# AlfredUg/MiCall-Lite

Measured on AMD Instinct MI355X. Metric: paired 2×251 nt reads/sec mapped+realigned; fraction of HBM roofline, higher is better.
Workload: dtype int32; 1 GPU; C2: synthetic 2x251 nt HIV-1 pol read pairs (10% divergent sample genome, 0.5% errors), prelim_map end-to-end vs 74 seeds + 1 remap iteration(s) (--local vs consensus) + pileups, default projects.json; pairs_per_gpu=1000000, read_len=251, parallelism=dp1 (one GPU, no collective), dist_world=1

## Files before the change

### include/micall_hip.h

```cpp
#ifndef MICALL_HIP_H
#define MICALL_HIP_H

#include <stddef.h>
#include <stdint.h>

#ifdef __cplusplus
extern "C" {
#endif

#define MH_MAXOPS 128

enum { MH_E2E = 0, MH_LOCAL = 1 };
enum { MH_OP_M = 0, MH_OP_I = 1, MH_OP_D = 2, MH_OP_S = 4 };

typedef struct {
    int mode;
    int rdg_open, rdg_ext;
    int rfg_open, rfg_ext;
    int maxins;
} mh_params;

typedef struct {
    int32_t ref, pos, rev, score, secbest, flag, mapq, rnext, pnext, tlen;
    int32_t sam_ref, sam_pos, xm, xo, xg, nm, ys, yt, yf, n_cigar;
// ... 1 lines not shown
} mh_aln;

typedef struct mh_ctx mh_ctx;

int mh_version(void);
int mh_last_error(char *buf, size_t cap);
int mh_device_count(int *n);

int mh_ctx_create(int device, mh_ctx **out);
int mh_ctx_destroy(mh_ctx *ctx);
int mh_ctx_sync(mh_ctx *ctx);
int mh_ctx_stream(mh_ctx *ctx, void **stream);

int mh_index_build(mh_ctx *ctx, int n_refs, const char *const *seqs, int seedlen);

int mh_reads_load(mh_ctx *ctx, int64_t n_reads, int paired, const uint8_t *seq,
                  const uint8_t *qual, const int64_t *offsets, const int32_t *lens);
int mh_reads_load_fastq(mh_ctx *ctx, const char *path1, const char *path2, int64_t *n_reads);
int mh_reads_load_fastq_part(mh_ctx *ctx, const char *path1, const char *path2, int part, int parts,
                             int64_t *n_reads, int64_t *first_unit);
int mh_reads_count(mh_ctx *ctx, int64_t *n_reads, int *paired);

typedef struct mh_fastq mh_fastq;
int mh_fastq_open_part(const char *path, int fd, int part, int parts, mh_fastq **out, int64_t *info);
int mh_fastq_scan_part(const char *path, int fd, int part, int parts, int64_t *info);
int mh_fastq_member_open(const char *path, int fd, int part, int parts, mh_fastq **out, int64_t *info);
int mh_fastq_member_decode(mh_fastq *fq, int64_t end_bit, int64_t *info);
int mh_fastq_member_tail(mh_fastq *fq, const char *window, char *tail);
int mh_fastq_member_finish(mh_fastq *fq, const char *window, int64_t c0, int64_t c1, int64_t *info);
int mh_fastq_frame(mh_fastq *fq, int64_t line0, int starts_line, int64_t *out5);
int mh_fastq_record_offset(mh_fastq *fq, int64_t k, int64_t *off);
int mh_fastq_splice(mh_fastq *fq, int64_t lo, int64_t hi, const char *front, int64_t flen,
                    const char *back, int64_t blen);
int mh_fastq_view(mh_fastq *fq, const char **data, int64_t *len);
int mh_fastq_close(mh_fastq *fq);
int mh_fastq_parse(mh_fastq *fq1, mh_fastq *fq2, char *names, size_t names_cap, uint8_t *seq,
                   uint8_t *qual, size_t bases_cap, int32_t *lens, int64_t reads_cap, int64_t *n_reads,
                   int64_t *n_bases, size_t *names_used);
int mh_reads_load_staged(mh_ctx *ctx, mh_fastq *fq1, mh_fastq *fq2, const int64_t *range4,
                         int64_t fastq_lines1, int64_t *n_reads);
int mh_reads_fastq_lines(mh_ctx *ctx, int64_t *lines1);

int mh_map(mh_ctx *ctx, const mh_params *par);
int mh_alns_fetch(mh_ctx *ctx, int64_t first, int64_t n, mh_aln *out);
int mh_map_counts(mh_ctx *ctx, int64_t *lines, int64_t *filtered, int64_t *mapped,
                  int64_t *first_row, int64_t *first_mapped, int64_t *unmapped,
                  int64_t *star_lines, int64_t *star_first);
int mh_map_stats(mh_ctx *ctx, int64_t *out5);
int mh_test_set_capacities(mh_ctx *ctx, int64_t cigar_pool_words, int64_t pileup_events,
                           int64_t pileup_event_bytes, int64_t token_bytes);
int mh_test_pileup_info(mh_ctx *ctx, int64_t *out16, int n_refs, int32_t *win_len);
int mh_test_force_index_collision(mh_ctx *ctx, int on);
int mh_retry_counts(mh_ctx *ctx, int64_t *out4);
int mh_test_set_gotoh_wait(mh_ctx *ctx, int64_t ticks);
int mh_recs_fetch(mh_ctx *ctx, int64_t first, int64_t n, int32_t *out20);
int mh_recs_fetch_fields(mh_ctx *ctx, int64_t first, int64_t n, int field0, int nfields, int32_t *out);
int mh_reads_set_names(mh_ctx *ctx, int64_t n, const char *const *names);
int mh_format_rows(mh_ctx *ctx, int style, const int64_t *order, int64_t first, int64_t n,
                   const char *const *refnames, char *buf, size_t cap, size_t *used);
int mh_format_segments(mh_ctx *ctx, int style, const int64_t *order, int64_t n,
                       const char *const *refnames, int n_seg, const int64_t *seg_rows,
                       int64_t *seg_bytes);
int mh_write_segments(mh_ctx *ctx, int fd, const int64_t *seg_off, uint32_t *crc);
uint32_t mh_crc32_combine(uint32_t a, uint32_t b, int64_t len_b);
int mh_file_crc32(int fd, int64_t *size, uint32_t *crc);
enum { MH_PHASE_INFLATE = 0, MH_PHASE_PARSE = 1, MH_PHASE_UPLOAD = 2, MH_PHASE_FORMAT = 3,
       MH_PHASE_WRITE = 4, MH_PHASES = 5 };
int mh_phase_times(mh_ctx *ctx, double *ms, int reset);
int mh_write_rows_crc(mh_ctx *ctx, int style, const int64_t *order, int64_t first, int64_t n,
                      const char *const *refnames, int fd, int64_t offset, int64_t *written,
                      uint32_t *crc);

int mh_rows_load(mh_ctx *ctx, int64_t n_rows, const int32_t *flag, const int32_t *ref,
                 const int32_t *pos, const int32_t *cigar_off, const int32_t *n_cigar,
                 const uint32_t *cigar, const uint8_t *seq, const uint8_t *qual,
                 const int64_t *offsets, const int32_t *lens, int64_t n_units,
                 const int64_t *unit_rows);
int mh_rows_load_csv(mh_ctx *ctx, const char *text, int64_t len, int n_refs,
                     const char *const *refnames, int64_t *n_rows, int64_t *n_units,
                     int32_t *n_present);
int mh_rows_info(mh_ctx *ctx, int32_t *out4, int32_t *present, char *unknown, size_t cap);
#define MH_PILEUP_SLACK 2048
int mh_pileup(mh_ctx *ctx, int source, int q_cutoff, int n_refs, const int32_t *ref_lens);
int mh_pileup_only(mh_ctx *ctx, int source, int q_cutoff, int n_refs, const int32_t *ref_lens, int n_sel,
                   const int32_t *sel);
#define MH_WATCH_MAXKEYS 1024
#define MH_WATCH_QBINS 95
int mh_pileup_watch(mh_ctx *ctx, int n_keys, const int32_t *refs, const int32_t *poss);
int mh_pileup_watch_fetch(mh_ctx *ctx, uint32_t *counts, int64_t *first_unit);
int mh_rows_load_sam(mh_ctx *ctx, const char *text, int64_t len, int64_t *n_rows,
                     int64_t *n_units, int32_t *n_refs, size_t *names_bytes);
int mh_sam_info(mh_ctx *ctx, char *names, size_t cap, int32_t *ends);
typedef struct {
    int64_t n_rows, n_units, n_cigar, n_bases;
    int32_t n_refs;
    size_t names_bytes;
} mh_sam_sizes;
int mh_sam_parse(const char *text, int64_t len, mh_sam_sizes *sizes, int32_t *flag, int32_t *ref,
                 int32_t *pos, int32_t *cigar_off, int32_t *n_cigar, uint32_t *cigar,
                 int64_t *seq_off, int32_t *seq_len, uint8_t *seq, uint8_t *qual, int64_t *units,
                 char *names, int32_t *ends);
typedef struct {
    int64_t n_rows, n_units, n_cigar, n_bases;
    int32_t n_present;
    size_t unknown_bytes;
} mh_prelim_sizes;
// ... 147 lines not shown
```

### micall-lite_amd/csrc/mh_api.cpp

```cpp
#include <errno.h>
#include <fcntl.h>
#include <sys/mman.h>
#include <sys/stat.h>
#include <unistd.h>
#include <zlib.h>

#include <algorithm>
#include <atomic>
#include <chrono>
#include <cmath>
#include <cstdarg>
#include <cstdio>
#include <cstring>
#include <memory>
#include <new>
#include <string>
#include <condition_variable>
#include <deque>
#include <exception>
#include <mutex>
#include <functional>
#include <string_view>
#include <thread>
#include <unordered_map>
#include <vector>

#include "mh_fastq.h"
#include "mh_gunzip.h"
#include "mh_internal.h"
#include "mh_prelim.h"
#include "mh_sam.h"
#include "mh_text.h"

#include <map>
#include <tuple>

namespace mh {

static thread_local char g_err[1024];

void set_error(const char *fmt, ...)
{
    va_list ap;
    va_start(ap, fmt);
    vsnprintf(g_err, sizeof(g_err), fmt, ap);
    va_end(ap);
}

static std::string last_error_text() { return std::string(g_err); }

int hip_fail(hipError_t e, const char *what)
{
    set_error("HIP error %d (%s) in %s", (int)e, hipGetErrorString(e), what);
    return -4;
}

hipError_t copy_sync(Ctx &c, void *dst, const void *src, size_t bytes, hipMemcpyKind kind)
{
    hipError_t e = hipMemcpyAsync(dst, src, bytes, kind, c.stream);
    return e == hipSuccess ? hipStreamSynchronize(c.stream) : e;
}

int prof_begin(Ctx &c, const char *name)
{
    if (!c.prof) return -1;
    ProfPending p{name, nullptr, nullptr};
    if (hipEventCreate(&p.a) != hipSuccess || hipEventCreate(&p.b) != hipSuccess) return -1;
    hipEventRecord(p.a, c.stream);
    c.prof_pending.push_back(p);
    return (int)c.prof_pending.size() - 1;
}

void prof_end(Ctx &c, int slot)
{
    if (slot < 0 || slot >= (int)c.prof_pending.size()) return;
    hipEventRecord(c.prof_pending[slot].b, c.stream);
}

void prof_flush(Ctx &c)
{
    for (auto &p : c.prof_pending) {
        float ms = 0.f;
        if (hipEventSynchronize(p.b) == hipSuccess && hipEventElapsedTime(&ms, p.a, p.b) == hipSuccess) {
            ProfEntry &e = c.prof_acc[p.name];
            e.ms += ms;
            e.launches += 1;
        }
        hipEventDestroy(p.a);
        hipEventDestroy(p.b);
    }
    c.prof_pending.clear();
}

static int seed_interval(int mode, int len)
{
    const double f = mode == MH_LOCAL ? 0.75 : 1.15;
    int iv = (int)(1.0 + f * std::sqrt((double)len) + 0.5);
    return iv < 1 ? 1 : iv;
}

static int min_score(int mode, int len)
{
    if (mode == MH_LOCAL) {
        double v = 20.0 + 8.0 * std::log((double)(len > 0 ? len : 1));
        long s = (long)v;
        return (int)(s < 0 ? 0 : s);
    }
    long s = (long)(-0.6 + -0.6 * (double)len);
    return (int)(s > 0 ? 0 : s);
}

static int n_ceil(int len) { return (int)(0.0 + 0.15 * (double)len); }

// ... 27 lines not shown
        c.len_tab = hit->second;
        c.len_tab_key = key;
        return 0;
    }
    std::vector<int32_t> t(4 * (MAXLEN + 1));
    for (int l = 0; l <= MAXLEN; ++l) {
        t[l] = seed_interval(par.mode, l);
        t[(MAXLEN + 1) + l] = min_score(par.mode, l);
        t[2 * (MAXLEN + 1) + l] = n_ceil(l);
        t[3 * (MAXLEN + 1) + l] = band_half(par, l);
    }
    int32_t *d = nullptr;
    MH_HIP(hipMalloc(&d, sizeof(int32_t) * t.size()));
    c.len_tabs[key] = d;
    MH_HIP(copy_sync(c, d, t.data(), sizeof(int32_t) * t.size(), hipMemcpyHostToDevice));
    c.len_tab = d;
    c.len_tab_key = key;
    return 0;
}

struct Bytes {
    std::unique_ptr<char[], BigDeleter> p{nullptr, BigDeleter{}};
    size_t n = 0;
    void alloc(size_t k)
    {
        p = std::unique_ptr<char[], BigDeleter>(big_alloc(k > 0 ? k : 1), BigDeleter{k > 0 ? k : 1});
        n = k;
    }
    void assign(const uint8_t *a, const uint8_t *b) { alloc((size_t)(b - a)); if (b > a) std::memcpy(p.get(), a, n); }
    uint8_t *data() { return (uint8_t *)p.get(); }
    const uint8_t *data() const { return (const uint8_t *)p.get(); }
    size_t size() const { return n; }
};

struct HostReads {
    Bytes seq, qual;
    std::vector<int64_t> off;
    std::vector<int32_t> len;
};

struct CtxEx : Ctx {
    HostReads host;
    std::vector<DevIndex> cache;
    std::vector<std::string> cache_text;
    bool force_index_collision = false;
    std::vector<Rec> rec_cache;
    std::vector<int32_t> csv_rows_info;
    std::vector<int32_t> csv_present;
    std::vector<std::string> csv_unknown;
    std::vector<std::string> sam_names;
    std::vector<int32_t> sam_ends;
    int64_t fastq_lines1 = -1;
    DevIndex small;
    int64_t tok_gen = -1;
    std::vector<int32_t> tok_ref, tok_pos, tok_off, tok_len;
    std::vector<int64_t> tok_count;
    std::string tok_pool;
    void *pin = nullptr;
    size_t pin_cap = 0;
    int64_t map_gen = 0;
    uint64_t fmt_key = 0;
    bool fmt_valid = false;
    std::vector<TextBuf> fmt_chunks;
    double phase_ms[MH_PHASES] = {};
    std::vector<TextBuf> seg_chunks;
    std::vector<int64_t> seg_at;
    std::unordered_map<const void *, size_t> rcap;
    uint8_t *stage_seq = nullptr, *stage_qual = nullptr;
    int64_t *stage_off = nullptr;
};

template <class T>
static hipError_t grow_dev(CtxEx &c, T *&p, size_t need)
{
    if (need == 0) need = 1;
    if (p) {
        auto it = c.rcap.find((const void *)p);
        if (it != c.rcap.end() && it->second >= need) return hipSuccess;
        if (it != c.rcap.end()) c.rcap.erase(it);
        hipFree(p);
        p = nullptr;
    }
    void *q = nullptr;
    const hipError_t e = hipMalloc(&q, need);
    if (e != hipSuccess) return e;
    p = (T *)q;
    c.rcap[(const void *)q] = need;
    return hipSuccess;
}

static void free_index(DevIndex &ix)
{
    hipFree(ix.blob);
    ix = DevIndex{};
}

static void free_reads(DevReads &r)
{
    hipFree(r.seq2); hipFree(r.nmask); hipFree(r.qual); hipFree(r.off); hipFree(r.len);
    r = DevReads{};
}

static uint8_t code_of(char ch)
{
    switch (ch) {
    case 'A': case 'a': return 0;
    case 'C': case 'c': return 1;
    case 'G': case 'g': return 2;
    case 'T': case 't': return 3;
    default: return 4;
    }
}

static inline uint64_t mix64(uint64_t h, uint64_t w)
{
    h = (h ^ w) * 0x9E3779B97F4A7C15ull;
    return h ^ (h >> 29);
}

static uint64_t signature(int n, const char *const *seqs, int seedlen)
{
    uint64_t h = 1469598103934665603ull ^ (uint64_t)seedlen;
    for (int r = 0; r < n; ++r) {
        const size_t len = std::strlen(seqs[r]);
        h = mix64(h, (uint64_t)len);
        uint64_t q[4] = {h, h ^ 1, h ^ 2, h ^ 3};
        size_t i = 0;
        for (; i + 32 <= len; i += 32)
            for (int k = 0; k < 4; ++k) {
                uint64_t w;
                std::memcpy(&w, seqs[r] + i + 8 * k, 8);
                q[k] = mix64(q[k], w);
            }
        h = mix64(mix64(mix64(mix64(h, q[0]), q[1]), q[2]), q[3]);
        for (; i + 8 <= len; i += 8) {
            uint64_t w;
            std::memcpy(&w, seqs[r] + i, 8);
            h = mix64(h, w);
        }
        uint64_t tail = 0;
        std::memcpy(&tail, seqs[r] + i, len - i);
        h = mix64(h, tail ^ 0xffull << 56);
    }
    return mix64(h, (uint64_t)n);
}

static int build_index(DevIndex &ix, int n_refs, const char *const *seqs, int seedlen)
{
    static const bool trace = getenv("MH_INDEX_TRACE") && *getenv("MH_INDEX_TRACE") == '1';
    const auto tb = std::chrono::steady_clock::now();
    auto mark = [&](const char *what) {
        if (trace)
            fprintf(stderr, "index %s %.2f ms\n", what,
                    std::chrono::duration<double, std::milli>(std::chrono::steady_clock::now() - tb).count());
    };
    struct E { uint64_t key; int32_t ref, pos; };
    std::vector<int64_t> ref_off(n_refs);
    std::vector<int32_t> ref_len(n_refs);
    int64_t total_len = 0;
    for (int r = 0; r < n_refs; ++r) {
        ref_len[r] = (int)std::strlen(seqs[r]);
        ref_off[r] = total_len;
        total_len += ref_len[r];
    }
    std::vector<uint8_t> codes((size_t)total_len);
    const int nt = std::max(1, std::min<int>(s2a_threads(), n_refs));
    std::vector<std::vector<E>> per(n_refs);
    mark("pre");
    std::vector<double> t_start((size_t)nt, 0.0);
    {
        std::atomic<int> next(0);
        par_for(nt, [&](int t) {
            t_start[(size_t)t] = std::chrono::duration<double, std::milli>(std::chrono::steady_clock::now() - tb).count();
            for (int r; (r = next.fetch_add(1)) < n_refs;) {
                const int L = ref_len[r];
                uint8_t *cr = codes.data() + ref_off[r];
                std::vector<E> &v = per[r];
                v.reserve(L > seedlen ? (size_t)(L - seedlen + 1) : 0);
                uint64_t key = 0;
                int last_n = -1;
                for (int p = 0; p < L; ++p) {
                    const uint8_t c = code_of(seqs[r][p]);
                    cr[p] = c;
                    if (c > 3) last_n = p;
                    key = (key >> 2) | ((uint64_t)(c & 3) << (2 * (seedlen - 1)));
                    if (p >= seedlen - 1 && last_n <= p - seedlen) v.push_back({key, r, p - seedlen + 1});
                }
            }
        });
    }
    if (trace) {
        double mx = 0;
        for (double x : t_start) mx = std::max(mx, x);
        fprintf(stderr, "index thread starts: last at %.2f ms\n", mx);
    }
    mark("seeds");
    std::vector<E> ent;
    {
        size_t n = 0;
        for (auto &v : per) n += v.size();
        ent.reserve(n);
        for (auto &v : per) { ent.insert(ent.end(), v.begin(), v.end()); std::vector<E>().swap(v); }
    }
    auto less = [](const E &a, const E &b) {
        return a.key != b.key ? a.key < b.key : a.ref != b.ref ? a.ref < b.ref : a.pos < b.pos;
    };
    {
        const int ns = ent.size() < 65536 ? 1 : s2a_threads();
        std::vector<size_t> b((size_t)ns + 1);
        for (int t = 0; t <= ns; ++t) b[(size_t)t] = ent.size() * (size_t)t / (size_t)ns;
        par_for(ns, [&](int t) { std::sort(ent.begin() + b[(size_t)t], ent.begin() + b[(size_t)t + 1], less); });
        for (int w = 1; w < ns; w *= 2) {
            std::vector<std::pair<int, int>> jobs;
            for (int t = 0; t + w < ns; t += 2 * w) jobs.push_back({t, std::min(t + 2 * w, ns)});
            par_for((int)jobs.size(), [&](int j) {
                const int a = jobs[(size_t)j].first, m = a + w, z = jobs[(size_t)j].second;
                std::inplace_merge(ent.begin() + b[(size_t)a], ent.begin() + b[(size_t)m], ent.begin() + b[(size_t)z], less);
            });
        }
    }
    mark("sort");
    size_t nkeys = 0;
    for (size_t i = 0; i < ent.size(); ++i) if (i == 0 || ent[i].key != ent[i - 1].key) ++nkeys;
    uint64_t cap = 1024;
    while (cap < 2 * nkeys) cap <<= 1;
    std::vector<uint4> hent(cap, make_uint4(~0u, ~0u, 0u, 0u));
    std::vector<int2> hits(ent.size() ? ent.size() : 1);
    for (size_t i = 0; i < ent.size();) {
        size_t j = i + 1;
        while (j < ent.size() && ent[j].key == ent[i].key) ++j;
        uint64_t h = hash_key(ent[i].key) & (cap - 1);
        while (((uint64_t)hent[h].x | ((uint64_t)hent[h].y << 32)) != HEMPTY) h = (h + 1) & (cap - 1);
        hent[h] = make_uint4((uint32_t)ent[i].key, (uint32_t)(ent[i].key >> 32), (uint32_t)i, (uint32_t)(j - i));
        i = j;
    }
    for (size_t i = 0; i < ent.size(); ++i) hits[i] = make_int2(ent[i].ref, ent[i].pos);
    mark("hash");
    ix.n_refs = n_refs;
    ix.seedlen = seedlen;
    ix.total = (int64_t)codes.size();
    ix.hmask = cap - 1;
    codes.resize(codes.size() + 64, 4);
    std::vector<uint32_t> code2((codes.size() + 15) / 16 + 2, 0), ncode((codes.size() + 31) / 32 + 2, 0);
    for (size_t j = 0; j < codes.size(); ++j) {
        if (codes[j] > 3) ncode[j >> 5] |= 1u << (j & 31);
        else code2[j >> 4] |= (uint32_t)codes[j] << (2 * (j & 15));
    }
    std::vector<uint32_t> cplane(2 * ((codes.size() + 31) / 32 + 2), 0);
    for (size_t j = 0; j < codes.size(); ++j) {
        const uint32_t c = codes[j] > 3 ? 0u : codes[j];
        cplane[2 * (j >> 5)] |= (c & 1u) << (j & 31);
        cplane[2 * (j >> 5) + 1] |= (c >> 1) << (j & 31);
    }
    auto al = [](size_t x) { return (x + 255) & ~(size_t)255; };
    constexpr int NP = 8;
    const size_t sz[NP] = {codes.size(), sizeof(int64_t) * (size_t)n_refs, sizeof(int32_t) * (size_t)n_refs,
                           sizeof(uint4) * cap, sizeof(int2) * hits.size(), sizeof(uint32_t) * code2.size(),
                           sizeof(uint32_t) * ncode.size(), sizeof(uint32_t) * cplane.size()};
    const void *src[NP] = {codes.data(), ref_off.data(), ref_len.data(), hent.data(), hits.data(),
                           code2.data(), ncode.data(), cplane.data()};
    size_t at[NP], total = 0;
    for (int x = 0; x < NP; ++x) { at[x] = total; total += al(sz[x]); }
    if ((int64_t)total > ix.cap_blob) {
        hipFree(ix.blob);
        ix.blob = nullptr;
        ix.cap_blob = 0;
        MH_HIP(hipMalloc(&ix.blob, total));
        ix.cap_blob = (int64_t)total;
    }
    mark("planes+alloc");
    std::vector<uint8_t> stage(total);
    for (int x = 0; x < NP; ++x) if (sz[x]) std::memcpy(stage.data() + at[x], src[x], sz[x]);
    mark("stage");
    uint8_t *d = (uint8_t *)ix.blob;
    ix.codes = d + at[0];
    ix.ref_off = (int64_t *)(d + at[1]);
    ix.ref_len = (int32_t *)(d + at[2]);
    ix.hent = (uint4 *)(d + at[3]);
    ix.hits = (int2 *)(d + at[4]);
    ix.code2 = (uint32_t *)(d + at[5]);
    ix.ncode = (uint32_t *)(d + at[6]);
    ix.cplane = (uint32_t *)(d + at[7]);
    MH_HIP(hipMemcpy(ix.blob, stage.data(), total, hipMemcpyHostToDevice));
    mark("upload");
    return 0;
}

static int load_reads(CtxEx &c, DevReads &dst, HostReads &host, int64_t n, int paired,
                      const uint8_t *seq, const uint8_t *qual, const int64_t *offsets,
                      const int32_t *lens, bool keep_host, HostReads *adopt = nullptr)
{
    if (n < 0 || (paired && (n & 1))) { set_error("reads: bad count"); return -3; }
    int max_len = 0;
    int64_t src_total = 0;
    for (int64_t r = 0; r < n; ++r) {
        if (lens[r] < 0 || lens[r] > MAXLEN) {
            set_error("reads: read %lld has length %d (max %d)", (long long)r, lens[r], MAXLEN);
            return -3;
        }
        max_len = std::max(max_len, (int)lens[r]);
        src_total = std::max(src_total, offsets[r] + lens[r]);
    }
    std::vector<int64_t> off(n > 0 ? n : 1);
    int64_t total = 0;
    for (int64_t r = 0; r < n; ++r) {
        off[r] = total;
        total += ((int64_t)lens[r] + 31) / 32 * 32;
    }
    MH_HIP(hipStreamSynchronize(c.stream));
    dst.n = n;
    dst.paired = paired;
    dst.max_len = max_len;
    dst.total_bases = total;
    MH_HIP(grow_dev(c, dst.seq2, sizeof(uint32_t) * (total / 16 + 8)));
    MH_HIP(grow_dev(c, dst.nmask, sizeof(uint32_t) * (total / 32 + 8)));
    MH_HIP(grow_dev(c, dst.qual, (size_t)total + 64));
    MH_HIP(grow_dev(c, dst.off, sizeof(int64_t) * (n > 0 ? n : 1)));
    MH_HIP(grow_dev(c, dst.len, sizeof(int32_t) * (n > 0 ? n : 1)));
    MH_HIP(hipMemsetAsync(dst.seq2, 0, sizeof(uint32_t) * (total / 16 + 8), c.stream));
    MH_HIP(hipMemsetAsync(dst.nmask, 0, sizeof(uint32_t) * (total / 32 + 8), c.stream));
    if (n > 0) {
        MH_HIP(hipMemcpyAsync(dst.off, off.data(), sizeof(int64_t) * n, hipMemcpyHostToDevice, c.stream));
        MH_HIP(hipMemcpyAsync(dst.len, lens, sizeof(int32_t) * n, hipMemcpyHostToDevice, c.stream));
        MH_HIP(grow_dev(c, c.stage_seq, (size_t)src_total + 1));
        MH_HIP(grow_dev(c, c.stage_qual, (size_t)src_total + 1));
        MH_HIP(grow_dev(c, c.stage_off, sizeof(int64_t) * (size_t)n));
        MH_HIP(hipMemcpyAsync(c.stage_seq, seq, src_total, hipMemcpyHostToDevice, c.stream));
        MH_HIP(hipMemcpyAsync(c.stage_qual, qual, src_total, hipMemcpyHostToDevice, c.stream));
        MH_HIP(hipMemcpyAsync(c.stage_off, offsets, sizeof(int64_t) * n, hipMemcpyHostToDevice, c.stream));
        MH_HIP(launch_pack_reads(dst, c.stage_seq, c.stage_qual, c.stage_off, c.stream));
        MH_HIP(hipStreamSynchronize(c.stream));
    }
    if (adopt) {
        host = std::move(*adopt);
    } else if (keep_host) {
        host.seq.assign(seq, seq + src_total);
        host.qual.assign(qual, qual + src_total);
// ... 175 lines not shown
    if (!buf || cap == 0) return -3;
    snprintf(buf, cap, "%s", g_err);
    return 0;
}

int mh_device_count(int *n)
{
    int k = 0;
    hipError_t e = hipGetDeviceCount(&k);
    if (e != hipSuccess) { *n = 0; return hip_fail(e, "hipGetDeviceCount") == -4 ? -5 : -5; }
    *n = k;
    return 0;
}

int mh_ctx_create(int device, mh_ctx **out)
{
    if (!out) return -3;
    *out = nullptr;
    int n = 0;
    if (hipGetDeviceCount(&n) != hipSuccess || n == 0) {
        set_error("no HIP device available (the MI355X path has no CPU fallback)");
        return -5;
    }
    if (device < 0 || device >= n) { set_error("bad device %d", device); return -3; }
    MH_HIP(hipSetDevice(device));
    hipDeviceProp_t prop;
    MH_HIP(hipGetDeviceProperties(&prop, device));
    if (std::strncmp(prop.gcnArchName, "gfx950", 6) != 0) {
        set_error("device %d is %s, libmicall_hip is built for gfx950 only", device, prop.gcnArchName);
        return -5;
    }
    CtxEx *c = new (std::nothrow) CtxEx();
    if (!c) return -2;
    c->device = device;
    hipError_t e = hipStreamCreateWithFlags(&c->stream, hipStreamNonBlocking);
    if (e != hipSuccess) { delete c; return hip_fail(e, "hipStreamCreate"); }
    *out = reinterpret_cast<mh_ctx *>(c);
    return 0;
}

int mh_ctx_destroy(mh_ctx *ctx)
{
    if (!ctx) return 0;
    CtxEx *c = X(ctx);
    hipSetDevice(c->device);
    hipStreamSynchronize(c->stream);
    free_reads(c->reads);
    free_reads(c->rows.reads);
    hipFree(c->stage_seq); hipFree(c->stage_qual); hipFree(c->stage_off);
    for (auto &ix : c->cache) free_index(ix);
    free_index(c->small);
    MapState &M = c->map;
    hipFree(M.cand); hipFree(M.n_cand); hipFree(M.yf); hipFree(M.work); hipFree(M.rwork); hipFree(M.skey); hipFree(M.sinfo);
    hipFree(M.pool); hipFree(M.pool_used); hipFree(M.rec); hipFree(M.counters); hipFree(M.ref_stats);
    if (M.stats_pin) hipHostFree(M.stats_pin);
    M.stats_pin = nullptr;
    M.stats_pin_cap = 0;
    RowState &R = c->rows;
    hipFree(R.flag); hipFree(R.ref); hipFree(R.pos); hipFree(R.cig_off); hipFree(R.n_cigar);
    hipFree(R.cigar); hipFree(R.units);
    PileState &P = c->pile;
    hipFree(c->gotoh_buf);
    hipFree(P.dense); hipFree(P.nflag); hipFree(P.dflag); hipFree(P.read_counts);
    hipFree(P.first_unit); hipFree(P.max_pos); hipFree(P.ev); hipFree(P.ev_pool);
    hipFree(P.tok_slot); hipFree(P.tok_cnt); hipFree(P.tok_used); hipFree(P.tok_meta);
    hipFree(P.tok_bytes);
    hipFree(P.ev_counters);
    if (P.land) hipHostFree(P.land);
    P.land = nullptr;
    if (P.tok_pin) hipHostFree(P.tok_pin);
    P.tok_pin = nullptr;
    P.tok_pin_cap = 0;
    P.land_cap = 0;
    P.land_ok = false;
    hipFree(P.ins_scratch);
    hipFree(P.watch_dpos); hipFree(P.watch_range); hipFree(P.watch_count); hipFree(P.watch_first);
    hipFree(P.sel);
    hipFree(P.win_map);
    for (auto &kv : c->len_tabs) hipFree(kv.second);
    if (c->pin) hipHostFree(c->pin);
    s2a_free(*c);
    censor_free(*c);
    a2c_free(*c);
    hipStreamDestroy(c->stream);
    delete c;
    return 0;
}

int mh_ctx_sync(mh_ctx *ctx)
{
    if (!ctx) return -3;
    MH_HIP(hipSetDevice(X(ctx)->device));
    MH_HIP(hipStreamSynchronize(X(ctx)->stream));
    return 0;
}

int mh_ctx_stream(mh_ctx *ctx, void **stream)
{
    if (!ctx || !stream) return -3;
    *stream = (void *)X(ctx)->stream;
    return 0;
}

int mh_index_build(mh_ctx *ctx, int n_refs, const char *const *seqs, int seedlen)
{
    if (!ctx || n_refs < 0 || (n_refs > 0 && !seqs) || seedlen < 8 || seedlen > 32) {
        set_error("mh_index_build: bad arguments");
        return -3;
    }
    CtxEx *c = X(ctx);
    MH_HIP(hipSetDevice(c->device));
    MH_HIP(hipStreamSynchronize(c->stream));
    int64_t total = 0;
    for (int r = 0; r < n_refs; ++r) total += (int64_t)std::strlen(seqs[r]);
    const uint64_t sig = c->force_index_collision ? 0x5eedull : signature(n_refs, seqs, seedlen);
    const bool cacheable = total > 65536;
    c->index = DevIndex{};
    for (size_t e = 0; e < c->cache.size(); ++e) {
        const DevIndex &ix = c->cache[e];
        if (ix.sig != sig || ix.n_refs != n_refs || ix.seedlen != seedlen) continue;
        const std::string &t = c->cache_text[e];
        bool same = t.size() == (size_t)(total + n_refs);
        size_t at = 0;
        for (int r = 0; same && r < n_refs; ++r) {
            const size_t len = std::strlen(seqs[r]);
            same = std::memcmp(t.data() + at, seqs[r], len + 1) == 0;
            at += len + 1;
        }
        if (same) {
            c->index = ix;
            return 0;
        }
    }
    if (!cacheable) {
        if (int st = build_index(c->small, n_refs, seqs, seedlen)) return st;
        c->small.sig = sig;
        c->index = c->small;
        return 0;
    }
    DevIndex ix;
    if (int st = build_index(ix, n_refs, seqs, seedlen)) { free_index(ix); return st; }
    ix.sig = sig;
    if (c->cache.size() >= 2) {
        free_index(c->cache.front());
        c->cache.erase(c->cache.begin());
        c->cache_text.erase(c->cache_text.begin());
    }
    std::string text;
    text.reserve((size_t)(total + n_refs));
    for (int r = 0; r < n_refs; ++r) text.append(seqs[r], std::strlen(seqs[r]) + 1);
    c->cache.push_back(ix);
    c->cache_text.push_back(std::move(text));
    c->index = ix;
    return 0;
}

int mh_reads_load(mh_ctx *ctx, int64_t n_reads, int paired, const uint8_t *seq,
                  const uint8_t *qual, const int64_t *offsets, const int32_t *lens)
{
    if (!ctx || (n_reads > 0 && (!seq || !qual || !offsets || !lens))) return -3;
    CtxEx *c = X(ctx);
    MH_HIP(hipSetDevice(c->device));
    c->names.clear();
    c->map.valid = false;
    return load_reads(*c, c->reads, c->host, n_reads, paired, seq, qual, offsets, lens, true);
}

int mh_reads_load_fastq(mh_ctx *ctx, const char *path1, const char *path2, int64_t *n_reads)
{
    return mh_reads_load_fastq_part(ctx, path1, path2, 0, 1, n_reads, nullptr);
}

static int host_reads_from(Fastq &a, Fastq *b, int64_t a0, int64_t a1, int64_t b0, int64_t b1,
                           HostReads &h, NameTable &names, double *names_ms, double *copy_ms)
{
    const bool paired = b != nullptr;
    if (a0 < 0 || a1 < a0 || a1 > (int64_t)a.size() ||
        (paired && (b0 < 0 || b1 < b0 || b1 > (int64_t)b->size() || b1 - b0 != a1 - a0))) {
        set_error("paired FASTQ blocks hold %lld and %lld reads", (long long)(a1 - a0),
                  (long long)(paired ? b1 - b0 : a1 - a0));
        return -3;
    }
    const int per = paired ? 2 : 1;
    const int64_t n = per * (a1 - a0);
    h.off.resize((size_t)n);
    h.len.resize((size_t)n);
    int64_t total = 0;
    for (int64_t i = 0; i < n; ++i) {
        const bool mate2 = paired && (i & 1);
        const Fastq &f = mate2 ? *b : a;
        h.off[i] = total;
        h.len[i] = f.len[(mate2 ? b0 : a0) + i / per];
        total += h.len[i];
    }
// ... 209 lines not shown
            return st;
        const int64_t n = (int64_t)h.len.size();
        const int64_t bases = n ? h.off[n - 1] + h.len[n - 1] : 0;
        *n_reads = n;
        *n_bases = bases;
        *names_used = nt.pool.size() + (size_t)n;
        if (!names || !seq || !qual || !lens) return 0;
        if (reads_cap < n || bases_cap < (size_t)bases || names_cap < *names_used) {
            set_error("mh_fastq_parse: buffers too small");
            return -2;
        }
        size_t at = 0;
        for (int64_t r = 0; r < n; ++r) {
            const std::string_view v = nt[(size_t)r];
            memcpy(names + at, v.data(), v.size());
            at += v.size();
            names[at++] = '\n';
            lens[r] = h.len[r];
        }
        if (bases) {
            memcpy(seq, h.seq.data(), (size_t)bases);
            memcpy(qual, h.qual.data(), (size_t)bases);
        }
        return 0;
    } catch (const std::bad_alloc &) {
        set_error("mh_fastq_parse: out of memory");
        return -2;
    }
}

int mh_reads_count(mh_ctx *ctx, int64_t *n_reads, int *paired)
{
    if (!ctx) return -3;
    if (n_reads) *n_reads = X(ctx)->reads.n;
    if (paired) *paired = X(ctx)->reads.paired;
    return 0;
}

int mh_reads_set_names(mh_ctx *ctx, int64_t n, const char *const *names)
{
    if (!ctx || n != X(ctx)->reads.n) { set_error("mh_reads_set_names: count mismatch"); return -3; }
    CtxEx *c = X(ctx);
    c->names.assign(names, n);
    return 0;
}

int mh_map(mh_ctx *ctx, const mh_params *par)
{
    if (!ctx || !par) return -3;
    CtxEx *c = X(ctx);
    MH_HIP(hipSetDevice(c->device));
    if (int st = prepare_len_tab(*c, *par)) return st;
    int st = run_map(*c, *par);
    if (st == 0) MH_HIP(hipStreamSynchronize(c->stream));
    prof_flush(*c);
    c->rec_cache.clear();
    ++c->map_gen;
    c->fmt_valid = false;
    c->fmt_chunks.clear();
    return st;
}

int mh_probe_extend(mh_ctx *ctx, const mh_params *par, int n, const int32_t *items, int32_t *out)
{
    if (!ctx || !par || n < 0 || (n > 0 && (!items || !out))) return -3;
    CtxEx *c = X(ctx);
    MH_HIP(hipSetDevice(c->device));
    if (int st = prepare_len_tab(*c, *par)) return st;
    return run_probe_ext(*c, *par, n, items, out);
}

int mh_profile(mh_ctx *ctx, int enable)
{
    if (!ctx) return -3;
    CtxEx *c = X(ctx);
    c->prof = enable != 0;
    c->prof_acc.clear();
    return 0;
}

int mh_profile_get(mh_ctx *ctx, const char *kernel, double *total_ms, int64_t *launches)
{
    if (!ctx || !kernel) return -3;
    CtxEx *c = X(ctx);
    prof_flush(*c);
    auto it = c->prof_acc.find(kernel);
    if (total_ms) *total_ms = it == c->prof_acc.end() ? 0.0 : it->second.ms;
    if (launches) *launches = it == c->prof_acc.end() ? 0 : it->second.launches;
    return 0;
}

static int fetch_recs(CtxEx *c, int64_t first, int64_t n, std::vector<Rec> &rec,
                      std::vector<uint32_t> &pool)
{
    MapState &M = c->map;
    if (!M.valid) { set_error("no mapping results (call mh_map)"); return -3; }
    if (first < 0 || n < 0 || first + n > M.n_reads) { set_error("record range out of bounds"); return -3; }
    rec.resize(n > 0 ? n : 1);
    if (n > 0)
        MH_HIP(copy_sync(*c, rec.data(), M.rec + first, sizeof(Rec) * n, hipMemcpyDeviceToHost));
    int64_t used = M.last_cigar < M.pool_cap ? M.last_cigar : M.pool_cap;
    pool.resize(used > 0 ? used : 1);
    if (used > 0)
        MH_HIP(copy_sync(*c, pool.data(), M.pool, sizeof(uint32_t) * used, hipMemcpyDeviceToHost));
    return 0;
}

// ... 40 lines not shown

int mh_map_stats(mh_ctx *ctx, int64_t *out5)
{
    if (!ctx || !out5) return -3;
    int64_t *out4 = out5;
    CtxEx *c = X(ctx);
    MapState &M = c->map;
    if (!M.valid) { set_error("no mapping results (call mh_map)"); return -3; }
    out4[0] = M.n_reads;
    out4[1] = M.last_work;
    out4[2] = M.last_cigar;
    out4[3] = M.last_fast;
    out5[4] = M.last_rescue;
    return 0;
}

int mh_test_force_index_collision(mh_ctx *ctx, int on)
{
    if (!ctx) return -3;
    X(ctx)->force_index_collision = on != 0;
    return 0;
}

int mh_test_set_capacities(mh_ctx *ctx, int64_t cigar_pool_words, int64_t pileup_events,
                           int64_t pileup_event_bytes, int64_t token_bytes)
{
    if (!ctx || cigar_pool_words < 0 || pileup_events < 0 || pileup_event_bytes < 0 || token_bytes < 0) {
        set_error("mh_test_set_capacities: bad arguments");
        return -3;
    }
    CtxEx *c = X(ctx);
    MH_HIP(hipSetDevice(c->device));
    MH_HIP(hipStreamSynchronize(c->stream));
    MapState &M = c->map;
    PileState &P = c->pile;
    hipFree(M.pool); M.pool = nullptr; M.pool_cap = 0;
    hipFree(P.ev); P.ev = nullptr; P.ev_cap = 0;
    hipFree(P.ev_pool); P.ev_pool = nullptr; P.pool_cap = 0;
    hipFree(P.tok_bytes); P.tok_bytes = nullptr; P.tok_bytes_cap = 0;
    M.valid = false;
    TestCaps &t = c->test_caps;
    t.cigar_pool_words = cigar_pool_words;
    t.pile_events = pileup_events;
    t.pile_event_bytes = pileup_event_bytes;
    t.token_bytes = token_bytes;
    return 0;
}

int mh_retry_counts(mh_ctx *ctx, int64_t *out4)
{
    if (!ctx || !out4) return -3;
    for (int k = 0; k < RETRY_KINDS; ++k) out4[k] = X(ctx)->retries[k];
    return 0;
}

int mh_test_set_gotoh_wait(mh_ctx *ctx, int64_t ticks)
{
    if (!ctx || ticks < 0) { set_error("mh_test_set_gotoh_wait: bad arguments"); return -3; }
    X(ctx)->test_caps.gotoh_wait_ticks = ticks;
    return 0;
}

int mh_recs_fetch(mh_ctx *ctx, int64_t first, int64_t n, int32_t *out20)
{
    if (!ctx || (n > 0 && !out20)) return -3;
    CtxEx *c = X(ctx);
    MapState &M = c->map;
    if (!M.valid) { set_error("no mapping results (call mh_map)"); return -3; }
    if (first < 0 || n < 0 || first + n > M.n_reads) { set_error("record range out of bounds"); return -3; }
    MH_HIP(hipSetDevice(c->device));
    if (n == 0) return 0;
    MH_HIP(hipMemcpy2DAsync(out20, sizeof(int32_t) * 20, M.rec + first, sizeof(Rec), sizeof(int32_t) * 20,
                            (size_t)n, hipMemcpyDeviceToHost, c->stream));
    MH_HIP(hipStreamSynchronize(c->stream));
    return 0;
}

int mh_recs_fetch_fields(mh_ctx *ctx, int64_t first, int64_t n, int field0, int nfields, int32_t *out)
{
    if (!ctx || (n > 0 && !out) || field0 < 0 || nfields < 1 || field0 + nfields > 20) return -3;
    CtxEx *c = X(ctx);
    MapState &M = c->map;
    if (!M.valid) { set_error("no mapping results (call mh_map)"); return -3; }
    if (first < 0 || n < 0 || first + n > M.n_reads) { set_error("record range out of bounds"); return -3; }
    MH_HIP(hipSetDevice(c->device));
    if (n == 0) return 0;
    MH_HIP(hipMemcpy2DAsync(out, sizeof(int32_t) * nfields, (const int32_t *)(M.rec + first) + field0, sizeof(Rec),
                            sizeof(int32_t) * nfields, (size_t)n, hipMemcpyDeviceToHost, c->stream));
    MH_HIP(hipStreamSynchronize(c->stream));
    return 0;
}

static inline char *put_int(char *o, int64_t v)
{
    char t[24];
    int n = 0;
    uint64_t u = v < 0 ? (uint64_t)(-(v + 1)) + 1 : (uint64_t)v;
    do { t[n++] = (char)('0' + u % 10); u /= 10; } while (u);
    if (v < 0) *o++ = '-';
    while (n) *o++ = t[--n];
    return o;
}

static inline char *put_str(char *o, const char *s, size_t n)
{
    std::memcpy(o, s, n);
// ... 723 lines not shown
    }
    P.watch_order.swap(order);
    return 0;
}

extern "C" int mh_pileup_watch_fetch(mh_ctx *ctx, uint32_t *counts, int64_t *first_unit)
{
    if (!ctx) return -3;
    CtxEx *c = X(ctx);
    PileState &P = c->pile;
    const size_t nk = P.watch_order.size(), cells = 4 * (size_t)MH_WATCH_QBINS;
    if (!nk) return 0;
    if (!counts || !first_unit) return -3;
    if (!P.watch_count || !P.watch_first) { set_error("no watched pileup (call mh_pileup)"); return -3; }
    MH_HIP(hipSetDevice(c->device));
    std::vector<uint32_t> cnt(nk * cells);
    std::vector<uint64_t> fst(nk * cells);
    MH_HIP(copy_sync(*c, cnt.data(), P.watch_count, sizeof(uint32_t) * cnt.size(), hipMemcpyDeviceToHost));
    MH_HIP(copy_sync(*c, fst.data(), P.watch_first, sizeof(uint64_t) * fst.size(), hipMemcpyDeviceToHost));
    for (size_t z = 0; z < nk; ++z) {
        const size_t k = (size_t)P.watch_order[z];
        for (size_t x = 0; x < cells; ++x) {
            counts[k * cells + x] = cnt[z * cells + x];
            const uint64_t f = fst[z * cells + x];
            first_unit[k * cells + x] = f > (uint64_t)INT64_MAX ? INT64_MAX : (int64_t)f;
        }
    }
    return 0;
}

extern "C" int mh_rows_info(mh_ctx *ctx, int32_t *out4, int32_t *present, char *unknown,
                            size_t cap)
{
    if (!ctx) return -3;
    CtxEx *c = X(ctx);
    if (out4) std::memcpy(out4, c->csv_rows_info.data(), sizeof(int32_t) * c->csv_rows_info.size());
    if (present) std::memcpy(present, c->csv_present.data(), sizeof(int32_t) * c->csv_present.size());
    if (unknown) {
        std::string all;
        for (auto &u : c->csv_unknown) { all += u; all.push_back('\n'); }
        if (all.size() + 1 > cap) { set_error("mh_rows_info: name buffer too small"); return -2; }
        std::memcpy(unknown, all.c_str(), all.size() + 1);
    }
    return 0;
}

extern "C" int mh_reads_fastq_lines(mh_ctx *ctx, int64_t *lines1)
{
    if (!ctx || !lines1) return -3;
    *lines1 = X(ctx)->fastq_lines1;
    return 0;
}

struct Landing {
    int64_t *read_counts, *first_unit;
    int32_t *max_pos;
    int64_t *ev_counters;
    size_t bytes;
};

static Landing landing_of(const PileState &P)
{
    const size_t nr = (size_t)P.n_refs, ev_at = (20 * nr + 7) & ~(size_t)7;
    return Landing{(int64_t *)P.land, (int64_t *)(P.land + 8 * nr), (int32_t *)(P.land + 16 * nr),
                   (int64_t *)(P.land + ev_at), 20 * nr + 64};
}

int mh_pileup(mh_ctx *ctx, int source, int q_cutoff, int n_refs, const int32_t *ref_lens)
{
    return mh_pileup_only(ctx, source, q_cutoff, n_refs, ref_lens, -1, nullptr);
}

int mh_pileup_only(mh_ctx *ctx, int source, int q_cutoff, int n_refs, const int32_t *ref_lens, int n_sel,
                   const int32_t *sel)
{
    if (!ctx || n_refs < 0 || (n_refs > 0 && !ref_lens) || (source != 0 && source != 1) ||
        (n_sel > 0 && !sel))
        return -3;
    CtxEx *c = X(ctx);
    MH_HIP(hipSetDevice(c->device));
    c->pile.only.clear();
    if (n_sel >= 0) {
        c->pile.only.assign((size_t)n_refs, 0);
        for (int k = 0; k < n_sel; ++k) {
            if (sel[k] < 0 || sel[k] >= n_refs) { set_error("mh_pileup_only: reference %d out of range", sel[k]); return -3; }
            c->pile.only[(size_t)sel[k]] = 1;
        }
        if (!c->pile.watch_order.empty()) {
            set_error("mh_pileup_only: watched positions are set (mh_pileup_watch); a watched pileup "
                      "counts every reference");
            return -3;
        }
    }
    int32_t cap = 1;
    for (int r = 0; r < n_refs; ++r) cap = std::max(cap, ref_lens[r] + MH_PILEUP_SLACK);
    c->pile.n_refs = n_refs;
    c->pile.cap = cap;
    c->pile.ref_lens.assign(ref_lens, ref_lens + n_refs);
    c->pile.land_ok = false;
    int st = run_pileup(*c, source, q_cutoff);
    if (st == 0) {
        PileState &P = c->pile;
        const size_t nr = (size_t)P.n_refs, need = landing_of(P).bytes;
        if (P.land_cap < need) {
            if (P.land) hipHostFree(P.land);
            P.land = nullptr;
            P.land_cap = 0;
            if (hipHostMalloc((void **)&P.land, need, hipHostMallocDefault) == hipSuccess) P.land_cap = need;
            else P.land = nullptr;
        }
        if (P.land && P.read_counts && P.first_unit && P.max_pos) {
            const Landing L = landing_of(P);
            bool ok = hipMemcpyAsync(L.read_counts, P.read_counts, 8 * nr, hipMemcpyDeviceToHost, c->stream) == hipSuccess &&
                      hipMemcpyAsync(L.first_unit, P.first_unit, 8 * nr, hipMemcpyDeviceToHost, c->stream) == hipSuccess &&
                      hipMemcpyAsync(L.max_pos, P.max_pos, 4 * nr, hipMemcpyDeviceToHost, c->stream) == hipSuccess;
            if (ok && P.ev_counters)
                ok = hipMemcpyAsync(L.ev_counters, P.ev_counters, 32, hipMemcpyDeviceToHost, c->stream) == hipSuccess;
            P.land_ok = ok;
        }
        MH_HIP(hipStreamSynchronize(c->stream));
    }
    prof_flush(*c);
    return st;
}

static int aggregate_tokens(CtxEx &c)
{
    PileState &P = c.pile;
    if (c.tok_gen == P.gen) return 0;
    c.tok_ref.clear(); c.tok_pos.clear(); c.tok_off.clear(); c.tok_len.clear();
    c.tok_count.clear(); c.tok_pool.clear();
    int64_t ctr[4] = {0, 0, 0, 0};
    if (P.ev_counters && P.land_ok)
        std::memcpy(ctr, landing_of(P).ev_counters, sizeof(ctr));
    else if (P.ev_counters)
        MH_HIP(copy_sync(c, ctr, P.ev_counters, sizeof(ctr), hipMemcpyDeviceToHost));
    const int64_t ne = ctr[0];
    if (ne > 0) {
        std::vector<int32_t> meta;
        std::string bytes;
        if (int st = run_token_aggregate(c, ne, ctr[1], meta, bytes)) return st;
        struct Key { int32_t ref, pos, off, len; int64_t count; };
        const size_t nd = meta.size() / 5;
        std::vector<Key> uniq(nd);
        for (size_t d = 0; d < nd; ++d)
            uniq[d] = Key{meta[5 * d], meta[5 * d + 1], meta[5 * d + 2], meta[5 * d + 3], meta[5 * d + 4]};
        const char *pb = bytes.data();
        std::sort(uniq.begin(), uniq.end(), [pb](const Key &a, const Key &b) {
            if (a.ref != b.ref) return a.ref < b.ref;
            if (a.pos != b.pos) return a.pos < b.pos;
            const int cmp = std::memcmp(pb + a.off, pb + b.off, (size_t)std::min(a.len, b.len));
            if (cmp != 0) return cmp < 0;
            return a.len < b.len;
        });
        for (const Key &k : uniq) {
            c.tok_ref.push_back(k.ref);
            c.tok_pos.push_back(k.pos);
            c.tok_off.push_back((int32_t)c.tok_pool.size());
            c.tok_len.push_back(k.len);
            c.tok_count.push_back(k.count);
            c.tok_pool.append(pb + k.off, (size_t)k.len);
        }
    }
    c.tok_gen = P.gen;
    return 0;
}

int mh_pileup_dims(mh_ctx *ctx, int *n_refs, int32_t *cap, int64_t *n_events, int64_t *event_bytes)
{
    if (!ctx) return -3;
    CtxEx *c = X(ctx);
    PileState &P = c->pile;
    if (n_refs) *n_refs = P.n_refs;
    if (cap) *cap = P.cap;
    MH_HIP(hipSetDevice(c->device));
    if (int st = aggregate_tokens(*c)) return st;
    if (n_events) *n_events = (int64_t)c->tok_ref.size();
    if (event_bytes) *event_bytes = (int64_t)c->tok_pool.size();
    return 0;
}

struct FetchPart {
    const void *src;
    size_t bytes;
    void *dst;
};

static int fetch_parts(CtxEx &c, const FetchPart *parts, int n)
{
    size_t total = 0;
    for (int i = 0; i < n; ++i) if (parts[i].dst) total += (parts[i].bytes + 255) & ~(size_t)255;
    if (total > ((size_t)64 << 20)) {
        for (int i = 0; i < n; ++i)
            if (parts[i].dst && parts[i].bytes)
                MH_HIP(copy_sync(c, parts[i].dst, parts[i].src, parts[i].bytes, hipMemcpyDeviceToHost));
        return 0;
    }
    if (c.pin_cap < total) {
        if (c.pin) hipHostFree(c.pin);
        c.pin = nullptr;
        c.pin_cap = 0;
        const size_t cap = total > ((size_t)1 << 20) ? total : ((size_t)1 << 20);
        MH_HIP(hipHostMalloc(&c.pin, cap, hipHostMallocDefault));
        c.pin_cap = cap;
    }
    size_t at = 0;
    for (int i = 0; i < n; ++i) {
        if (!parts[i].dst) continue;
        if (parts[i].bytes)
            MH_HIP(hipMemcpyAsync((char *)c.pin + at, parts[i].src, parts[i].bytes, hipMemcpyDeviceToHost,
                                  c.stream));
        at += (parts[i].bytes + 255) & ~(size_t)255;
    }
    MH_HIP(hipStreamSynchronize(c.stream));
    at = 0;
    for (int i = 0; i < n; ++i) {
        if (!parts[i].dst) continue;
        if (parts[i].bytes) std::memcpy(parts[i].dst, (const char *)c.pin + at, parts[i].bytes);
        at += (parts[i].bytes + 255) & ~(size_t)255;
    }
    return 0;
}

int mh_pileup_fetch(mh_ctx *ctx, int32_t *dense, uint8_t *nflag, uint8_t *dflag,
                    int64_t *read_counts, int64_t *first_unit, int32_t *max_pos)
{
    if (!ctx) return -3;
    CtxEx *c = X(ctx);
    PileState &P = c->pile;
    if (!P.dense) { set_error("no pileup (call mh_pileup)"); return -3; }
    MH_HIP(hipSetDevice(c->device));
    const size_t cells = (size_t)P.n_refs * P.cap, nr = (size_t)P.n_refs;
    if (!dense && !nflag && !dflag && P.land_ok) {
        const Landing L = landing_of(P);
        if (read_counts) std::memcpy(read_counts, L.read_counts, 8 * nr);
        if (first_unit) std::memcpy(first_unit, L.first_unit, 8 * nr);
        if (max_pos) std::memcpy(max_pos, L.max_pos, 4 * nr);
        return 0;
    }
    const FetchPart parts[6] = {{P.dense, sizeof(int32_t) * 4 * cells, dense},
                                {P.nflag, cells, nflag},
                                {P.dflag, cells, dflag},
                                {P.read_counts, sizeof(int64_t) * nr, read_counts},
                                {P.first_unit, sizeof(int64_t) * nr, first_unit},
                                {P.max_pos, sizeof(int32_t) * nr, max_pos}};
    return fetch_parts(*c, parts, 6);
}

int mh_pileup_fetch_refs(mh_ctx *ctx, int n_sel, const int32_t *refs, int32_t *dense, uint8_t *nflag,
                         uint8_t *dflag)
{
    if (!ctx || n_sel < 0 || (n_sel > 0 && (!refs || !dense || !nflag || !dflag))) return -3;
    CtxEx *c = X(ctx);
    PileState &P = c->pile;
    if (!P.dense) { set_error("no pileup (call mh_pileup)"); return -3; }
    MH_HIP(hipSetDevice(c->device));
    std::vector<int32_t> mx((size_t)std::max(P.n_refs, 1));
    if (P.land_ok && P.land)
        std::memcpy(mx.data(), landing_of(P).max_pos, sizeof(int32_t) * (size_t)P.n_refs);
    else
        MH_HIP(copy_sync(*c, mx.data(), P.max_pos, sizeof(int32_t) * (size_t)P.n_refs, hipMemcpyDeviceToHost));
    std::vector<FetchPart> parts;
    parts.reserve(3 * (size_t)n_sel);
    for (int k = 0; k < n_sel; ++k) {
        const int r = refs[k];
        if (r < 0 || r >= P.n_refs) { set_error("mh_pileup_fetch_refs: ref %d out of range", r); return -3; }
        const int64_t rows = std::min<int64_t>(P.cap, std::max(mx[(size_t)r], 0));
        if (rows == 0) continue;
        const int64_t base = (int64_t)r * P.cap;
        parts.push_back({P.dense + 4 * base, sizeof(int32_t) * 4 * (size_t)rows, dense + 4 * base});
        parts.push_back({P.nflag + base, (size_t)rows, nflag + base});
        parts.push_back({P.dflag + base, (size_t)rows, dflag + base});
    }
    return parts.empty() ? 0 : fetch_parts(*c, parts.data(), (int)parts.size());
}

int mh_pileup_events(mh_ctx *ctx, int32_t *ref, int32_t *pos, int32_t *tok_off, int32_t *tok_len,
                     int64_t *count, char *pool)
{
    if (!ctx) return -3;
    CtxEx *c = X(ctx);
    MH_HIP(hipSetDevice(c->device));
    if (int st = aggregate_tokens(*c)) return st;
    const size_t n = c->tok_ref.size();
    if (ref) std::memcpy(ref, c->tok_ref.data(), sizeof(int32_t) * n);
    if (pos) std::memcpy(pos, c->tok_pos.data(), sizeof(int32_t) * n);
    if (tok_off) std::memcpy(tok_off, c->tok_off.data(), sizeof(int32_t) * n);
    if (tok_len) std::memcpy(tok_len, c->tok_len.data(), sizeof(int32_t) * n);
    if (count) std::memcpy(count, c->tok_count.data(), sizeof(int64_t) * n);
    if (pool) std::memcpy(pool, c->tok_pool.data(), c->tok_pool.size());
    return 0;
}

static int gotoh_threw(const char *entry, const std::exception &e)
{
    set_error("%s: out of memory (%s)", entry, e.what());
    return -2;
}

int mh_gotoh_align(mh_ctx *ctx, const char *seq1, const char *seq2, int gop, int gep,
                   int is_global, const char *alphabet, const int *matrix, char *out1, char *out2,
                   int cap, int *score)
{
    if (!ctx || !seq1 || !seq2 || !alphabet || !matrix || !out1 || !out2 || !score) return -3;
    CtxEx *c = X(ctx);
    MH_HIP(hipSetDevice(c->device));
    try {
        return run_gotoh(*c, seq1, seq2, gop, gep, is_global, alphabet, matrix, out1, out2, cap, score);
    } catch (const std::exception &e) {
        return gotoh_threw("mh_gotoh_align", e);
    }
}

int mh_gotoh_align_batch(mh_ctx *ctx, int count, const char *const *seq1,
                         const char *const *seq2, int gop, int gep, int is_global,
                         const char *alphabet, const int *matrix, char *const *out1,
                         char *const *out2, const int *cap, int *score, int *status)
{
    if (!ctx || count < 0 || (count > 0 && (!seq1 || !seq2 || !out1 || !out2 || !cap || !score ||
// ... 268 lines not shown
```

### micall-lite_amd/csrc/mh_internal.h

```cpp
#pragma once
#include <hip/hip_runtime.h>
#include <stdint.h>
#include <string.h>

#include <map>
#include <mutex>
#include <string>
#include <string_view>
#include <tuple>
#include <vector>

#include "micall_hip.h"
#include "mh_gunzip.h"

namespace mh {

constexpr int BAND = 64;
constexpr int MAXCAND = 4;
constexpr int MAXHITS_SEED = 64;
constexpr int MAXHITS_MATE = 512;
constexpr int CLUSTER_GAP = 8;
constexpr int MAXSEEDS = 32;
constexpr int MAXLEN = 1024;
constexpr int GBAR = 4;
// ... 32 lines not shown
    int32_t *ref_len = nullptr;
    uint4 *hent = nullptr;
    uint64_t hmask = 0;
    int2 *hits = nullptr;
    uint64_t sig = 0;
    void *blob = nullptr;
    int64_t cap_blob = 0;
};

constexpr uint64_t HEMPTY = ~0ull;

__host__ __device__ inline uint64_t hash_key(uint64_t k)
{
    k ^= k >> 33;
    k *= 0xff51afd7ed558ccdull;
    k ^= k >> 33;
    k *= 0xc4ceb9fe1a85ec53ull;
    k ^= k >> 33;
    return k;
}

struct Cand {
    int32_t strand, ref, center, support;
};

struct Slot {
    int32_t valid, strand, ref, pos, end, score, xm, xo, xg, nm, n_cigar, cig_off;
    int32_t maxm;
};

struct alignas(16) SlotKey {
    int32_t rs;
    int32_t pos, end, score;
};
struct alignas(16) SlotInfo {
    int32_t cig_off;
    uint32_t xm_xo;
    uint32_t xg_nc;
    int32_t maxm;
};
static_assert(sizeof(SlotInfo) == 16, "a read's MAXCAND statistics fill half a 128-B line");

struct Rec {
    int32_t ref, pos, rev, score, secbest, flag, mapq, rnext, pnext, tlen;
    int32_t sam_ref, sam_pos, xm, xo, xg, nm, ys, yt, yf, n_cigar;
    int32_t cig_off, maxm;
};

__host__ __device__ inline int64_t slot_at(int32_t sid, int64_t plane)
{
    const uint32_t u = (uint32_t)sid;
    return (int64_t)(u % MAXCAND) * plane + (int64_t)(u / MAXCAND);
}

struct MapState {
    int64_t n_reads = 0;
    int n_refs = 0;
    mh_params par{};
    Cand *cand = nullptr;
    int32_t *n_cand = nullptr;
    int32_t *yf = nullptr;
    int32_t *work = nullptr;
    int32_t *rwork = nullptr;
    SlotKey *skey = nullptr;
    SlotInfo *sinfo = nullptr;
    uint32_t *pool = nullptr;
    int64_t pool_cap = 0;
    unsigned long long *pool_used = nullptr;
    Rec *rec = nullptr;
    int32_t *counters = nullptr;
    int64_t *ref_stats = nullptr;
    int64_t cap_reads = 0;
    int cap_refs = 0;
    int64_t last_work = 0;
    int64_t last_cigar = 0;
    int64_t last_fast = 0;
    int64_t last_rescue = 0;
    bool valid = false;
    std::vector<int64_t> stats_host;
    int64_t *stats_pin = nullptr;
    size_t stats_pin_cap = 0;
    bool stats_pin_ready = false;
    std::map<std::pair<const void *, int>, int> dp_occ;
    bool stats_host_valid = false;
};

struct RowState {
    int64_t n_rows = 0, n_units = 0;
    int32_t *flag = nullptr, *ref = nullptr, *pos = nullptr, *cig_off = nullptr,
            *n_cigar = nullptr;
    uint32_t *cigar = nullptr;
    int64_t *units = nullptr;
    DevReads reads;
    int hot_ref = -1;
    std::vector<int64_t> ref_rows;
    int max_span = 0;
};

struct PileState {
    int n_refs = 0;
    int32_t cap = 0;
    int32_t *dense = nullptr;
    uint8_t *nflag = nullptr;
    uint8_t *dflag = nullptr;
    int64_t *read_counts = nullptr;
    int64_t *first_unit = nullptr;
    int32_t *max_pos = nullptr;
    int32_t *ev = nullptr;
    char *ev_pool = nullptr;
    int64_t ev_cap = 0, pool_cap = 0;
    int64_t *ev_counters = nullptr;
    int64_t alloc_cells = 0;
    int alloc_refs = 0;
    int64_t gen = 0;
    char *land = nullptr;
    size_t land_cap = 0;
    bool land_ok = false;
    std::vector<int32_t> ref_lens;
    std::vector<uint8_t> only;
    std::vector<int32_t> watch_ref, watch_pos, watch_order;
    int32_t *watch_dpos = nullptr, *watch_range = nullptr;
    int watch_range_cap = 0;
    uint32_t *watch_count = nullptr;
    unsigned long long *watch_first = nullptr;
    int32_t *sel = nullptr;
    int sel_cap = 0;
    int32_t *win_map = nullptr;
    int win_map_cap = 0;
    char *ins_scratch = nullptr;
    int64_t ins_scratch_bytes = 0;
    std::map<std::tuple<int, int64_t, int>, std::pair<int, int>> shapes;
    int32_t *tok_slot = nullptr;
    uint32_t *tok_cnt = nullptr;
    int32_t *tok_used = nullptr;
    int64_t tok_cap = 0;
    int32_t *tok_meta = nullptr;
    char *tok_bytes = nullptr;
    int64_t tok_meta_cap = 0, tok_bytes_cap = 0;
    char *tok_pin = nullptr;
    size_t tok_pin_cap = 0;
    struct Info {
        int64_t blocks = 0, n_units = 0;
        int wpb = 0, win_words = 0;
        std::vector<int32_t> win_map;
        int64_t tok_insert_blocks = 0, tok_count_blocks = 0, tok_ne = 0, tok_nd = 0;
    } info;
};

hipError_t launch_pack_reads(DevReads &r, const uint8_t *d_seq, const uint8_t *d_qual,
                             const int64_t *d_src_off, hipStream_t s);
int run_map(struct Ctx &c, const mh_params &par);
int run_probe_ext(struct Ctx &c, const mh_params &par, int n, const int32_t *items, int32_t *out);
const int64_t *map_stats_host(struct Ctx &c);
int run_pileup(struct Ctx &c, int source, int q_cutoff);
int run_token_aggregate(struct Ctx &c, int64_t n_events, int64_t pool_used,
                        std::vector<int32_t> &meta, std::string &bytes);
int run_gotoh(struct Ctx &c, const char *s1, const char *s2, int gop, int gep, int is_global,
              const char *alphabet, const int *matrix, char *out1, char *out2, int cap,
              int *score);
int run_gotoh_batch(struct Ctx &c, int count, const char *const *s1, const char *const *s2,
                    int gop, int gep, int is_global, const char *alphabet, const int *matrix,
                    char *const *out1, char *const *out2, const int *cap, int *score,
                    int *status);
int run_gotoh_distance_batch(struct Ctx &c, int count, const char *const *s1, const char *const *s2,
                             const char *const *text, int gop, int gep, int is_global,
                             const char *alphabet, const int *matrix, int *dist, int *score,
                             int *status);

struct NameTable {
    TextBuf pool;
    std::vector<int64_t> off{0};
    size_t size() const { return off.size() - 1; }
    std::string_view operator[](size_t r) const
    {
        return std::string_view(pool.data() + off[r], (size_t)(off[r + 1] - off[r]));
    }
    void clear() { pool.clear(); off.assign(1, 0); }
    void assign(const char *const *names, int64_t n)
    {
        clear();
        off.resize((size_t)n + 1);
        for (int64_t r = 0; r < n; ++r) off[r + 1] = off[r] + (int64_t)strlen(names[r]);
        pool.resize((size_t)off[n]);
        for (int64_t r = 0; r < n; ++r) memcpy(&pool[off[r]], names[r], (size_t)(off[r + 1] - off[r]));
    }
    void swap(NameTable &o) { pool.swap(o.pool); off.swap(o.off); }
};

struct ProfEntry {
    double ms = 0.0;
    int64_t launches = 0;
};

struct ProfPending {
    const char *name;
    hipEvent_t a, b;
};

struct S2AState;
struct CensorState;
struct A2CState;

struct TestCaps {
    int64_t cigar_pool_words = 0;
    int64_t pile_events = 0;
    int64_t pile_event_bytes = 0;
    int64_t token_bytes = 0;
    int64_t gotoh_wait_ticks = 0;
};

enum { RETRY_CIGAR_POOL = 0, RETRY_PILE_EVENTS = 1, RETRY_TOKEN_BYTES = 2, RETRY_GOTOH_WAIT = 3,
       RETRY_KINDS = 4 };

struct Ctx {
    int device = 0;
    TestCaps test_caps;
    int64_t retries[RETRY_KINDS] = {0, 0, 0, 0};
    int n_cu = 0;
    bool prof = false;
    std::map<std::string, ProfEntry> prof_acc;
    std::vector<ProfPending> prof_pending;
    hipStream_t stream = nullptr;
    DevReads reads;
    NameTable names;
    std::vector<std::string> host_seq, host_qual;
    DevIndex index;
    MapState map;
    RowState rows;
    PileState pile;
    int32_t *len_tab = nullptr;
    S2AState *s2a = nullptr;
    int64_t s2a_serial = 0;
    CensorState *censor = nullptr;
    A2CState **a2c = nullptr;
    int64_t len_tab_key = -1;
    std::map<int64_t, int32_t *> len_tabs;
    char *gotoh_buf = nullptr;
    size_t gotoh_cap = 0;
    std::mutex gotoh_mutex;
};

void set_error(const char *fmt, ...);
int host_read_text(Ctx &c, int64_t r, bool rev, char *seq, char *qual);
Ctx *ctx_of(mh_ctx *ctx);
void s2a_free(Ctx &c);
void censor_free(Ctx &c);
void a2c_free(Ctx &c);
int prof_begin(Ctx &c, const char *name);
void prof_end(Ctx &c, int slot);
void prof_flush(Ctx &c);
int hip_fail(hipError_t e, const char *what);
hipError_t copy_sync(Ctx &c, void *dst, const void *src, size_t bytes, hipMemcpyKind kind);

}

#define MH_HIP(call)                                                  \
    do {                                                              \
        hipError_t e_ = (call);                                       \
        if (e_ != hipSuccess) return ::mh::hip_fail(e_, #call);       \
    } while (0)
```

### micall-lite_amd/csrc/mh_map.hip

```cpp
#include <cstring>

#include "mh_internal.h"

namespace mh {

template <int CTRL, int ROWMASK = 0xF>
__device__ __forceinline__ int dpp(int old, int v)
{
    return __builtin_amdgcn_update_dpp(old, v, CTRL, ROWMASK, 0xF, false);
}
constexpr int DPP_ROW_SHR1 = 0x111, DPP_ROW_SHR2 = 0x112, DPP_ROW_SHR4 = 0x114,
              DPP_ROW_SHR8 = 0x118, DPP_WAVE_SHL1 = 0x130, DPP_WAVE_SHR1 = 0x138;

__device__ __forceinline__ int wave_uniform(int v) { return __builtin_amdgcn_readfirstlane(v); }

__device__ __forceinline__ void wave_sync()
{
    __builtin_amdgcn_fence(__ATOMIC_RELEASE, "wavefront");
    __builtin_amdgcn_wave_barrier();
    __builtin_amdgcn_fence(__ATOMIC_ACQUIRE, "wavefront");
}

template <class Op>
__device__ __forceinline__ int wave_scan_dpp(int v, int identity, Op op)
// ... 2204 lines not shown
                o1.tlen = first1 ? t : -t;
                o2.tlen = first1 ? -t : t;
            } else {
                o1.rnext = o2.ref;
                o2.rnext = o1.ref;
            }
            o1.pnext = o2.sam_pos;
            o2.pnext = o1.sam_pos;
        } else if (al1 || al2) {
            const int sref = al1 ? o1.sam_ref : o2.sam_ref;
            const int spos = al1 ? o1.sam_pos : o2.sam_pos;
            const int ascore = al1 ? o1.score : o2.score;
            o1.sam_ref = o2.sam_ref = sref;
            o1.sam_pos = o2.sam_pos = spos;
            o1.rnext = o2.rnext = -1;
            o1.pnext = o2.pnext = spos;
            if (al1) o2.ys = ascore;
            else o1.ys = ascore;
        }
        A.rec[r1] = o1;
        A.rec[r2] = o2;
        tally(A, T, o1, r1);
        tally(A, T, o2, r2);
    }
    if (T) {
        __syncthreads();
        tally_flush(A, T);
    }
}

static int64_t pool_words_for(int64_t n)
{
    return (n > 0 ? n : 1) * 8 + 4096 + 2 * (int64_t)DP_MAX_BLOCKS * DP_WAVES_PER_BLOCK * POOL_CHUNK;
}

static int ensure_map_buffers(Ctx &c)
{
    MapState &M = c.map;
    const int64_t n = c.reads.n;
    if (M.cap_reads < n || M.cand == nullptr) {
        hipFree(M.cand); hipFree(M.n_cand); hipFree(M.yf); hipFree(M.work);
        hipFree(M.rwork); hipFree(M.skey); hipFree(M.sinfo); hipFree(M.rec);
        const int64_t cap = n > 0 ? n : 1;
        MH_HIP(hipMalloc(&M.cand, sizeof(Cand) * cap * MAXCAND));
        MH_HIP(hipMalloc(&M.n_cand, sizeof(int32_t) * cap));
        MH_HIP(hipMalloc(&M.yf, sizeof(int32_t) * cap));
        MH_HIP(hipMalloc(&M.work, sizeof(int32_t) * cap * MAXCAND));
        MH_HIP(hipMalloc(&M.rwork, sizeof(int32_t) * (cap / 2 + 1)));
        MH_HIP(hipMalloc(&M.skey, sizeof(SlotKey) * cap * MAXCAND));
        MH_HIP(hipMalloc(&M.sinfo, sizeof(SlotInfo) * cap * MAXCAND));
        MH_HIP(hipMalloc(&M.rec, sizeof(Rec) * cap));
        M.cap_reads = cap;
    }
    if (M.counters == nullptr) MH_HIP(hipMalloc(&M.counters, sizeof(int32_t) * 8));
    if (M.cap_refs < c.index.n_refs || M.ref_stats == nullptr) {
        hipFree(M.ref_stats);
        const int cr = c.index.n_refs > 0 ? c.index.n_refs : 1;
        MH_HIP(hipMalloc(&M.ref_stats, sizeof(int64_t) * (5 * cr + 3)));
        M.cap_refs = cr;
    }
    if (M.pool_used == nullptr) MH_HIP(hipMalloc(&M.pool_used, sizeof(unsigned long long)));
    const int64_t test_cap = c.test_caps.cigar_pool_words;
    const int64_t need = test_cap > 0 ? test_cap : pool_words_for(n);
    if (need > (int64_t)INT32_MAX) {
        set_error("mh_map: %lld reads need a CIGAR pool past 2^31 words; map them in batches",
                  (long long)n);
        return -3;
    }
    if (M.pool == nullptr || (test_cap > 0 ? M.pool_cap != need : M.pool_cap < need)) {
        hipFree(M.pool);
        M.pool = nullptr;
        M.pool_cap = 0;
        MH_HIP(hipMalloc(&M.pool, sizeof(uint32_t) * need));
        M.pool_cap = need;
    }
    return 0;
}

__global__ void k_init_stats(int64_t *s, int n_refs)
{
    for (int i = blockIdx.x * blockDim.x + threadIdx.x; i < 5 * n_refs + 3; i += gridDim.x * blockDim.x)
        s[i] = ((i >= 3 * n_refs && i < 5 * n_refs) || i == 5 * n_refs + 2) ? INT64_MAX : 0;
}

__global__ void k_fix_first(int64_t *s, int n_refs)
{
    for (int i = blockIdx.x * blockDim.x + threadIdx.x; i < 2 * n_refs; i += gridDim.x * blockDim.x)
        if (s[3 * n_refs + i] == INT64_MAX) s[3 * n_refs + i] = -1;
    if (blockIdx.x == 0 && threadIdx.x == 0 && s[5 * n_refs + 2] == INT64_MAX) s[5 * n_refs + 2] = -1;
}

const int64_t *map_stats_host(Ctx &c)
{
    MapState &M = c.map;
    if (!M.stats_host_valid) {
        M.stats_host.resize(5 * (size_t)M.n_refs + 3);
        const size_t bytes = sizeof(int64_t) * M.stats_host.size();
        if (M.stats_pin_ready) {
            if (hipStreamSynchronize(c.stream) != hipSuccess) {
                set_error("map_stats_host: copy failed");
                return nullptr;
            }
            std::memcpy(M.stats_host.data(), M.stats_pin, bytes);
        } else if (hipMemcpyAsync(M.stats_host.data(), M.ref_stats, bytes, hipMemcpyDeviceToHost,
                                  c.stream) != hipSuccess ||
                   hipStreamSynchronize(c.stream) != hipSuccess) {
            set_error("map_stats_host: copy failed");
            return nullptr;
        }
        M.stats_host_valid = true;
    }
    return M.stats_host.data();
}

template <int LOCAL>
__global__ __launch_bounds__(64) void k_probe_ext(DpArgs A, const int32_t *items, int32_t *out, int n)
{
    extern __shared__ __attribute__((aligned(16))) unsigned char smem[];
    const int lane = threadIdx.x & 63;
    const int e = blockIdx.x;
    if (e >= n) return;
    uint32_t *bits = (uint32_t *)smem;
    unsigned char *xbase = smem + (size_t)32 * A.rows_pad;
    const XView X0 = xview(xbase, A.rows_pad, 0);
    const int gmin = A.oeI < A.oeD ? A.oeI : A.oeD;
    const int r = items[4 * e];
    XItem it;
    it.sid = 0;
    it.m = A.R.len[r];
    it.roff = A.R.off[r];
    it.strand = items[4 * e + 1];
    it.ref = items[4 * e + 2];
    it.d0 = items[4 * e + 3] - XCENTER;
    it.reflen = A.I.ref_len[it.ref];
    it.gref = A.I.ref_off[it.ref];
    it.hb = A.len_tab[3 * (MAXLEN + 1) + it.m];
    stage_ext<LOCAL>(A, it, X0, lane);
    wave_sync();
    int best = 0, bi = 0, bl = 0, low = -1;
    const bool fast = it.m > 2 * GBAR + 8 && it.m <= 512 &&
                      dp_ungapped<LOCAL>(X0, it.m, lane, gmin, it.hb, best, bi, bl, low, A.oeI, A.exI,
                                        A.oeD, A.exD);
    wave_sync();
    int b0, i0, l0, b1, i1, l1;
    dp_pair<LOCAL>(A, X0, X0, it.m, it.m, it.hb, it.hb, bits, lane, b0, i0, l0, b1, i1, l1);
    if (lane == 0) {
        int32_t *o = out + 8 * e;
        o[0] = fast;
        o[1] = fast ? best : 0;
        o[2] = fast ? bi : 0;
        o[3] = fast ? bl : 0;
        o[4] = it.hb;
        o[5] = b0;
        o[6] = i0;
        o[7] = l0;
    }
}

int run_probe_ext(Ctx &c, const mh_params &par, int n, const int32_t *items, int32_t *out)
{
    if (c.index.n_refs <= 0 || c.reads.n <= 0 || n < 0) { set_error("mh_probe_extend: no index / reads"); return -3; }
    if (par.mode != MH_E2E && par.mode != MH_LOCAL) { set_error("mh_probe_extend: bad mode"); return -3; }
    if (c.len_tab == nullptr || c.len_tab_key != len_tab_key(par)) { set_error("mh_probe_extend: length tables"); return -3; }
    for (int e = 0; e < n; ++e) {
        if (items[4 * e] < 0 || items[4 * e] >= c.reads.n || (items[4 * e + 1] & ~1) ||
            items[4 * e + 2] < 0 || items[4 * e + 2] >= c.index.n_refs) {
            set_error("mh_probe_extend: item %d out of range", e);
            return -3;
        }
    }
    if (n == 0) return 0;
    const int rows_pad = ((c.reads.max_len + 7) / 8) * 8;
    const int lds = 32 * rows_pad + 2 * xview_bytes(rows_pad);
    if (lds > 160 * 1024) { set_error("mh_probe_extend: reads too long"); return -3; }
    hipStream_t s = c.stream;
    int32_t *d_items = nullptr, *d_out = nullptr;
    MH_HIP(hipMalloc(&d_items, sizeof(int32_t) * 4 * (size_t)n));
    MH_HIP(hipMalloc(&d_out, sizeof(int32_t) * 8 * (size_t)n));
    MH_HIP(hipMemcpyAsync(d_items, items, sizeof(int32_t) * 4 * (size_t)n, hipMemcpyHostToDevice, s));
    DpArgs da{c.reads, c.index, c.len_tab, nullptr, nullptr, nullptr, nullptr, nullptr, nullptr,
              nullptr, nullptr, nullptr, 0, rows_pad, lds,
              par.rfg_open + par.rfg_ext, par.rfg_ext, par.rdg_open + par.rdg_ext, par.rdg_ext};
    const void *kf = par.mode == MH_LOCAL ? (const void *)k_probe_ext<1> : (const void *)k_probe_ext<0>;
    MH_HIP(hipFuncSetAttribute(kf, hipFuncAttributeMaxDynamicSharedMemorySize, 160 * 1024));
    if (par.mode == MH_LOCAL) hipLaunchKernelGGL((k_probe_ext<1>), dim3(n), dim3(64), lds, s, da, d_items, d_out, n);
    else hipLaunchKernelGGL((k_probe_ext<0>), dim3(n), dim3(64), lds, s, da, d_items, d_out, n);
    MH_HIP(hipGetLastError());
    MH_HIP(hipMemcpyAsync(out, d_out, sizeof(int32_t) * 8 * (size_t)n, hipMemcpyDeviceToHost, s));
    MH_HIP(hipStreamSynchronize(s));
    hipFree(d_items);
    hipFree(d_out);
    return 0;
}

int run_map(Ctx &c, const mh_params &par)
{
    c.map.stats_host_valid = false;
    c.map.stats_pin_ready = false;
    if (c.index.n_refs <= 0 || c.index.hent == nullptr) {
        set_error("mh_map: no reference index (call mh_index_build first)");
        return -3;
    }
    if (par.mode != MH_E2E && par.mode != MH_LOCAL) { set_error("mh_map: bad mode"); return -3; }
    const int SL = par.mode == MH_LOCAL ? 20 : 22;
    if (c.index.seedlen != SL) {
        set_error("mh_map: index seed length %d does not match mode (%d)", c.index.seedlen, SL);
        return -3;
    }
    if (c.len_tab == nullptr || c.len_tab_key != len_tab_key(par)) {
        set_error("mh_map: length tables not prepared");
        return -3;
    }
    if (int st = ensure_map_buffers(c)) return st;
    MapState &M = c.map;
    const int64_t n = c.reads.n;
    M.n_reads = n;
    M.n_refs = c.index.n_refs;
    M.par = par;
    hipStream_t s = c.stream;
    M.last_work = M.last_cigar = 0;
    if (n == 0) hipLaunchKernelGGL(k_init_stats, dim3(64), dim3(256), 0, s, M.ref_stats, M.n_refs);
    if (n > 0) {
        auto launch_seed = [&]() -> int {
            SeedArgs sa{c.reads, c.index, par.mode, c.len_tab, M.cand, M.n_cand, M.yf, M.work, M.counters, M.cap_reads};
            int64_t blocks = ((n + SEED_CHUNK - 1) / SEED_CHUNK + 3) / 4;
            if (blocks > 1 << 16) blocks = 1 << 16;
            const int pk = prof_begin(c, "k_seed");
            hipLaunchKernelGGL(k_seed, dim3((unsigned)blocks), dim3(256), 0, s, sa);
            prof_end(c, pk);
            MH_HIP(hipGetLastError());
            return 0;
        };

        const int rows_pad = ((c.reads.max_len + 7) / 8) * 8;
        const int wave_lds = 32 * rows_pad + 2 * xview_bytes(rows_pad) + raw_bytes(rows_pad);
        if (wave_lds > 160 * 1024) { set_error("mh_map: reads too long for LDS"); return -3; }
        int wpb = 1;
        for (int w = DP_WAVES_PER_BLOCK; w >= 1; --w)
            if ((160 * 1024 / (w * wave_lds)) * w > (160 * 1024 / (wpb * wave_lds)) * wpb ||
                ((160 * 1024 / (w * wave_lds)) * w == (160 * 1024 / (wpb * wave_lds)) * wpb && w > wpb))
                wpb = w;
        auto launch_dp = [&](const int32_t *work, const int32_t *count, int32_t *queue,
                             int64_t max_items, const char *name) -> int {
            DpArgs da{c.reads, c.index, c.len_tab, M.cand, work, count, M.skey, M.sinfo, M.pool,
                      M.pool_used, M.counters + 1, queue, M.pool_cap, rows_pad, wave_lds,
                      par.rfg_open + par.rfg_ext, par.rfg_ext, par.rdg_open + par.rdg_ext,
                      par.rdg_ext, M.cap_reads};
            const int round = rows_pad <= 256 ? 256 : rows_pad <= 320 ? 320 : 0;
            const void *kf =
                par.mode == MH_LOCAL
                    ? (round == 256 ? (const void *)k_dp<1, 256> : round ? (const void *)k_dp<1, 320> : (const void *)k_dp<1, 0>)
                    : (round == 256 ? (const void *)k_dp<0, 256> : round ? (const void *)k_dp<0, 320> : (const void *)k_dp<0, 0>);
            const auto okey = std::make_pair(kf, wpb * wave_lds);
            auto occ = M.dp_occ.find(okey);
            if (occ == M.dp_occ.end()) {
                MH_HIP(hipFuncSetAttribute(kf, hipFuncAttributeMaxDynamicSharedMemorySize, 160 * 1024));
                if (!c.n_cu) MH_HIP(hipDeviceGetAttribute(&c.n_cu, hipDeviceAttributeMultiprocessorCount, c.device));
                int nb = 0;
                MH_HIP(hipOccupancyMaxActiveBlocksPerMultiprocessor(&nb, kf, 64 * wpb, (size_t)wpb * wave_lds));
                occ = M.dp_occ.emplace(okey, nb).first;
            }
            const int per_cu = occ->second;
            int64_t dblocks = (int64_t)(c.n_cu > 0 ? c.n_cu : 256) * (per_cu > 0 ? per_cu : 1);
            const int64_t need = (max_items + (int64_t)wpb * DP_QUEUE_CHUNK - 1) / ((int64_t)wpb * DP_QUEUE_CHUNK);
            if (dblocks > need) dblocks = need;
            if (dblocks > DP_MAX_BLOCKS) dblocks = DP_MAX_BLOCKS;
            if (dblocks < 1) dblocks = 1;
            const int pd = prof_begin(c, name);
            const dim3 grid((unsigned)dblocks), block(64 * wpb);
            const size_t lds = (size_t)wpb * wave_lds;
            if (par.mode == MH_LOCAL) {
                if (round == 256) hipLaunchKernelGGL((k_dp<1, 256>), grid, block, lds, s, da);
                else if (round) hipLaunchKernelGGL((k_dp<1, 320>), grid, block, lds, s, da);
                else hipLaunchKernelGGL((k_dp<1, 0>), grid, block, lds, s, da);
            } else {
                if (round == 256) hipLaunchKernelGGL((k_dp<0, 256>), grid, block, lds, s, da);
                else if (round) hipLaunchKernelGGL((k_dp<0, 320>), grid, block, lds, s, da);
                else hipLaunchKernelGGL((k_dp<0, 0>), grid, block, lds, s, da);
            }
            prof_end(c, pd);
            MH_HIP(hipGetLastError());
            return 0;
        };
        const int64_t units = c.reads.paired ? n / 2 : n;
        PairArgs pa{c.reads, c.len_tab, M.skey, M.sinfo, M.n_cand, M.yf, M.pool, M.rec, M.ref_stats,
                    M.n_refs, par.mode == MH_LOCAL, par.maxins, c.reads.paired, M.cap_reads};
        int64_t pblocks = (units + 255) / 256;
        if (pblocks > 1 << 16) pblocks = 1 << 16;
        if (pblocks < 1) pblocks = 1;
        for (int attempt = 0; attempt < 2; ++attempt) {
            hipLaunchKernelGGL(k_init_stats, dim3(64), dim3(256), 0, s, M.ref_stats, M.n_refs);
            MH_HIP(hipMemsetAsync(M.counters, 0, sizeof(int32_t) * 8, s));
            MH_HIP(hipMemsetAsync(M.pool_used, 0, sizeof(unsigned long long), s));
            if (int st = launch_seed()) return st;
            if (int st = launch_dp(M.work, M.counters, M.counters + 5, n * 2, "k_dp")) return st;
            if (c.reads.paired && units > 0) {
                RescueArgs ra{c.reads, c.index, M.skey, M.n_cand, M.yf, M.cand, M.rwork,
                              M.counters + 4, par.maxins, M.cap_reads};
                int64_t rblocks = (units + 255) / 256;
                if (rblocks > 4096) rblocks = 4096;
                const int pr = prof_begin(c, "k_rescue");
                hipLaunchKernelGGL(k_rescue, dim3((unsigned)rblocks), dim3(256), 0, s, ra);
                prof_end(c, pr);
                MH_HIP(hipGetLastError());
                if (int st = launch_dp(M.rwork, M.counters + 4, M.counters + 6, units, "k_dp_rescue")) return st;
            }
            pa.pool = M.pool;
            const int pp = prof_begin(c, "k_pair");
            hipLaunchKernelGGL(k_pair, dim3((unsigned)pblocks), dim3(256), 0, s, pa);
            prof_end(c, pp);
            MH_HIP(hipGetLastError());
            int32_t ctr[5];
            unsigned long long used = 0;
            MH_HIP(hipMemcpyAsync(ctr, M.counters, sizeof(ctr), hipMemcpyDeviceToHost, s));
            MH_HIP(hipMemcpyAsync(&used, M.pool_used, sizeof(used), hipMemcpyDeviceToHost, s));
            MH_HIP(hipStreamSynchronize(s));
            M.last_work = ctr[0] + ctr[4];
            M.last_rescue = ctr[4];
            M.last_cigar = (int64_t)used;
            M.last_fast = ctr[3];
            if (!ctr[2]) break;
            if (attempt == 1) { set_error("mh_map: CIGAR pool overflow after a retry"); return -2; }
            ++c.retries[RETRY_CIGAR_POOL];
            hipFree(M.pool);
            M.pool = nullptr;
            M.pool_cap = 0;
            int64_t grown = (int64_t)used * 2 + pool_words_for(0);
            if (grown > (int64_t)INT32_MAX) grown = INT32_MAX;
            if ((int64_t)used > grown) {
                set_error("mh_map: CIGAR pool demand %llu words passes the int32 offsets",
                          (unsigned long long)used);
                return -2;
            }
            MH_HIP(hipMalloc(&M.pool, sizeof(uint32_t) * grown));
            M.pool_cap = grown;
        }
    }
    hipLaunchKernelGGL(k_fix_first, dim3(8), dim3(256), 0, s, M.ref_stats, M.n_refs);
    MH_HIP(hipGetLastError());
    {
        const size_t bytes = sizeof(int64_t) * (5 * (size_t)M.n_refs + 3);
        if (M.stats_pin_cap < bytes) {
            if (M.stats_pin) hipHostFree(M.stats_pin);
            M.stats_pin = nullptr;
            M.stats_pin_cap = 0;
            if (hipHostMalloc(&M.stats_pin, bytes, hipHostMallocDefault) == hipSuccess)
                M.stats_pin_cap = bytes;
            else
                M.stats_pin = nullptr;
        }
        if (M.stats_pin && hipMemcpyAsync(M.stats_pin, M.ref_stats, bytes, hipMemcpyDeviceToHost, s) == hipSuccess)
            M.stats_pin_ready = true;
    }
    M.valid = true;
    return 0;
}

}
```

### micall-lite_amd/csrc/mh_pileup.hip

```cpp
#include <cstring>

#include "mh_internal.h"

namespace mh {

constexpr int PU_INSBUF = 3 * 1024;
constexpr int PU_MAXINS = 2 * MH_MAXOPS;
constexpr int PU_LDS = 160 * 1024 - 64;
constexpr int PU_XCH = 5;
constexpr unsigned long long PILE_ERR_ROW = 1, PILE_ERR_INSBUF = 2;
constexpr int PW_QBINS = MH_WATCH_QBINS, PW_Q0 = 32;

struct RowV {
    int present, flag, ref, pos, n_cigar, rev, m;
    const uint32_t *cig;
    int64_t roff;
    uint32_t op0;
};

__device__ __forceinline__ void fetch_ops(RowV &v, int lane)
{
    v.op0 = 0;
    if (v.present && lane < v.n_cigar) v.op0 = v.cig[lane];
}
// ... 693 lines not shown
                    const unsigned long long p = atomicAdd(&A.ev_ctr[1], (unsigned long long)tl);
                    if ((long long)e < A.ev_cap && (long long)(p + tl) <= A.pool_cap) {
                        A.ev[4 * e] = ref;
                        A.ev[4 * e + 1] = P;
                        A.ev[4 * e + 2] = (int32_t)p;
                        A.ev[4 * e + 3] = tl;
                        A.ev_pool[p] = mc;
                        for (int x = 0; x < tl - 1; ++x) A.ev_pool[p + 1 + x] = I.buf[I.off[hit] + x];
                    } else {
                        atomicExch(&A.ev_ctr[2], 1ull);
                    }
                }
            }
            if (base) {
                const int code = (((int)mc >> 1) ^ ((int)mc >> 2)) & 3;
                if (wo >= 0 && P <= wl) atomicAdd(&win[wo + (code >> 1) * wl + (P - 1)], 1u << (16 * (code & 1)));
                else atomicAdd(&A.dense[cell * 4 + code], 1);
            }
        };
        for (int i0 = begin; i0 < len2; i0 += 128) {
            const int ia = i0 + lane, ib = ia + 64;
            const char ma = merged(ia), mb = merged(ib);
            count(ia, ma);
            count(ib, mb);
        }
        mxp = wave_max_all(mxp);
        err = wave_max_all(err);
        if (lane == 0) {
            atomicAdd(&rl[ref].read_count, 1u);
            atomicMin(&rl[ref].first_unit, (long long)u);
            if (mxp > 0) atomicMax(&rl[ref].max_pos, mxp);
            if (err) atomicExch(&A.ev_ctr[3], PILE_ERR_ROW);
        }
        __builtin_amdgcn_wave_barrier();
    }
    __syncthreads();
    for (int r = 0; r < NR; ++r) {
        const int wo = wmap[2 * r], wl = wmap[2 * r + 1];
        if (wo < 0) continue;
        int32_t *dst = A.dense + (int64_t)r * A.cap * 4;
        for (int x = threadIdx.x; x < 4 * wl; x += blockDim.x) {
            const unsigned int v = (win[wo + ((x & 3) >> 1) * wl + (x >> 2)] >> (16 * (x & 1))) & 0xffffu;
            if (v) atomicAdd(&dst[x], (int)v);
        }
    }
    for (int r = threadIdx.x; r < NR; r += blockDim.x) {
        if (!rl[r].read_count) continue;
        atomicAdd(&A.read_counts[r], (unsigned long long)rl[r].read_count);
        atomicMin(&A.first_unit[r], rl[r].first_unit);
        if (rl[r].max_pos > 0) atomicMax(&A.max_pos[r], rl[r].max_pos);
    }
}

__global__ void k_pile_init(long long *first_unit, int32_t *max_pos, int n)
{
    for (int i = blockIdx.x * blockDim.x + threadIdx.x; i < n; i += gridDim.x * blockDim.x) {
        first_unit[i] = INT64_MAX;
        max_pos[i] = 0;
    }
}

__global__ void k_pile_fix(long long *first_unit, int n)
{
    for (int i = blockIdx.x * blockDim.x + threadIdx.x; i < n; i += gridDim.x * blockDim.x)
        if (first_unit[i] == INT64_MAX) first_unit[i] = -1;
}

static int ensure_pile(Ctx &c)
{
    PileState &P = c.pile;
    const int64_t cells = (int64_t)(P.n_refs > 0 ? P.n_refs : 1) * P.cap;
    if (P.alloc_cells < cells) {
        hipFree(P.dense); hipFree(P.nflag); hipFree(P.dflag);
        MH_HIP(hipMalloc(&P.dense, sizeof(int32_t) * 4 * cells));
        MH_HIP(hipMalloc(&P.nflag, cells));
        MH_HIP(hipMalloc(&P.dflag, cells));
        P.alloc_cells = cells;
    }
    if (P.alloc_refs < (P.n_refs > 0 ? P.n_refs : 1)) {
        hipFree(P.read_counts); hipFree(P.first_unit); hipFree(P.max_pos);
        const int nr = P.n_refs > 0 ? P.n_refs : 1;
        MH_HIP(hipMalloc(&P.read_counts, sizeof(int64_t) * nr));
        MH_HIP(hipMalloc(&P.first_unit, sizeof(int64_t) * nr));
        MH_HIP(hipMalloc(&P.max_pos, sizeof(int32_t) * nr));
        P.alloc_refs = nr;
    }
    if (!P.ev_counters) MH_HIP(hipMalloc(&P.ev_counters, sizeof(int64_t) * 4));
    const int64_t t_ev = c.test_caps.pile_events, t_pool = c.test_caps.pile_event_bytes;
    if (!P.ev || (t_ev > 0 && P.ev_cap != t_ev)) {
        hipFree(P.ev);
        P.ev = nullptr;
        P.ev_cap = t_ev > 0 ? t_ev : 1 << 16;
        MH_HIP(hipMalloc(&P.ev, sizeof(int32_t) * 4 * P.ev_cap));
    }
    if (!P.ev_pool || (t_pool > 0 && P.pool_cap != t_pool)) {
        hipFree(P.ev_pool);
        P.ev_pool = nullptr;
        P.pool_cap = t_pool > 0 ? t_pool : 1 << 20;
        MH_HIP(hipMalloc(&P.ev_pool, P.pool_cap));
    }
    return 0;
}

struct PileGeometry {
    int span = 0, unit_bytes = 0, wpb = 1, win_words = 0;
    std::vector<int32_t> win_map;
    int64_t blocks = 1;
    size_t lds = 0;
};

constexpr int64_t PU_UNITS_PER_BLOCK = 60000;

static int pile_geometry(Ctx &c, int source, int64_t n_units, PileGeometry &g)
{
    PileState &P = c.pile;
    const int NR = P.n_refs;
    std::vector<int64_t> hits((size_t)NR, 0);
    int span = 0;
    if (source == 0) {
        span = c.reads.max_len + BAND;
        const int n = c.map.n_refs;
        const int64_t *st = map_stats_host(c);
        if (!st) return -1;
        for (int r = 0; r < n && r < NR; ++r) hits[(size_t)r] = st[2 * (size_t)n + r];
    } else {
        span = c.rows.max_span;
        for (int r = 0; r < NR && r < (int)c.rows.ref_rows.size(); ++r) hits[(size_t)r] = c.rows.ref_rows[(size_t)r];
    }
    g.span = ((span > 16 ? span : 16) + 15) & ~15;
    g.unit_bytes = (unit_bytes_for(g.span) + 15) & ~15;
    const size_t base = (sizeof(RefLds) + 2 * sizeof(int32_t)) * (size_t)NR;
    if (base + (size_t)g.unit_bytes > (size_t)PU_LDS) {
        set_error("mh_pileup: reference span %d / %d references do not fit in LDS", span, NR);
        return -3;
    }
    const int64_t room = (int64_t)PU_LDS - (int64_t)base - 8 * (int64_t)g.unit_bytes;
    std::vector<int> order((size_t)NR);
    for (int r = 0; r < NR; ++r) order[(size_t)r] = r;
    std::stable_sort(order.begin(), order.end(), [&](int x, int y) { return hits[(size_t)x] > hits[(size_t)y]; });
    const bool some = P.only.size() == (size_t)NR;
// ... 31 lines not shown
        hit = P.shapes.emplace(key, std::make_pair(best_wpb, best_nb > 0 ? best_nb : 1)).first;
    }
    g.wpb = hit->second.first;
    g.lds = (size_t)lds0 + (size_t)g.wpb * g.unit_bytes;
    g.blocks = (n_units + g.wpb - 1) / g.wpb;
    const int64_t n_cu = c.n_cu > 0 ? c.n_cu : 256;
    const int64_t max_blocks = words > 0 ? n_cu * hit->second.second : n_cu * 8;
    if (g.blocks > max_blocks) g.blocks = max_blocks;
    if (words > 0 && g.blocks < (n_units + PU_UNITS_PER_BLOCK - 1) / PU_UNITS_PER_BLOCK)
        g.blocks = (n_units + PU_UNITS_PER_BLOCK - 1) / PU_UNITS_PER_BLOCK;
    if (g.blocks < 1) g.blocks = 1;
    return 0;
}

int run_pileup(Ctx &c, int source, int q_cutoff)
{
    PileState &P = c.pile;
    ++P.gen;
    int64_t n_units;
    const DevReads *R;
    if (source == 0) {
        if (!c.map.valid) { set_error("mh_pileup: no mapping results"); return -3; }
        R = &c.reads;
        n_units = c.reads.paired ? c.reads.n / 2 : c.reads.n;
    } else {
        R = &c.rows.reads;
        n_units = c.rows.n_units;
    }
    if (int st = ensure_pile(c)) return st;
    hipStream_t s = c.stream;
    PileGeometry geo;
    if (int st = pile_geometry(c, source, n_units, geo)) return st;
    P.info.blocks = geo.blocks;
    P.info.wpb = geo.wpb;
    P.info.win_words = geo.win_words;
    P.info.n_units = n_units;
    P.info.win_map = geo.win_map;
    P.info.tok_insert_blocks = P.info.tok_count_blocks = P.info.tok_ne = P.info.tok_nd = 0;
    {
        const int64_t need = geo.blocks * geo.wpb * (int64_t)PU_INS_BYTES;
        if (P.ins_scratch_bytes < need) {
            hipFree(P.ins_scratch);
            P.ins_scratch = nullptr;
            MH_HIP(hipMalloc(&P.ins_scratch, need));
            P.ins_scratch_bytes = need;
        }
    }
    if (P.win_map_cap < 2 * P.n_refs || !P.win_map) {
        hipFree(P.win_map);
        P.win_map = nullptr;
        P.win_map_cap = 2 * (P.n_refs > 16 ? P.n_refs : 16);
        MH_HIP(hipMalloc(&P.win_map, sizeof(int32_t) * P.win_map_cap));
    }
    if (P.n_refs > 0)
        MH_HIP(hipMemcpyAsync(P.win_map, geo.win_map.data(), sizeof(int32_t) * 2 * P.n_refs,
                              hipMemcpyHostToDevice, s));
    const int n_watch = (int)P.watch_order.size();
    const size_t watch_cells = (size_t)n_watch * 4 * PW_QBINS;
    if (n_watch > 0) {
        if (P.only.size() == (size_t)P.n_refs && P.n_refs > 0) {
            set_error("mh_pileup: watched positions with a reference selection");
            return -3;
        }
        if (!P.watch_dpos) {
            MH_HIP(hipMalloc(&P.watch_dpos, sizeof(int32_t) * MH_WATCH_MAXKEYS));
            MH_HIP(hipMalloc(&P.watch_count, sizeof(uint32_t) * MH_WATCH_MAXKEYS * 4 * PW_QBINS));
            MH_HIP(hipMalloc(&P.watch_first, sizeof(unsigned long long) * MH_WATCH_MAXKEYS * 4 * PW_QBINS));
        }
        const int nr = P.n_refs > 0 ? P.n_refs : 1;
        if (P.watch_range_cap < nr) {
            hipFree(P.watch_range);
            P.watch_range = nullptr;
            P.watch_range_cap = 0;
            MH_HIP(hipMalloc(&P.watch_range, sizeof(int32_t) * 2 * nr));
            P.watch_range_cap = nr;
        }
        std::vector<int32_t> range(2 * (size_t)nr, 0);
        for (int z = 0; z < n_watch; ++z) {
            const int32_t r = P.watch_ref[(size_t)z];
            if (r < 0 || r >= P.n_refs) continue;
            if (range[2 * (size_t)r + 1] == 0) range[2 * (size_t)r] = z;
            range[2 * (size_t)r + 1] = z + 1;
        }
        MH_HIP(copy_sync(c, P.watch_dpos, P.watch_pos.data(), sizeof(int32_t) * n_watch, hipMemcpyHostToDevice));
        MH_HIP(copy_sync(c, P.watch_range, range.data(), sizeof(int32_t) * range.size(), hipMemcpyHostToDevice));
    }
    const int64_t cells = (int64_t)P.n_refs * P.cap;
    for (int attempt = 0; attempt < 3; ++attempt) {
        if (n_watch > 0) {
            MH_HIP(hipMemsetAsync(P.watch_count, 0, sizeof(uint32_t) * watch_cells, s));
            MH_HIP(hipMemsetAsync(P.watch_first, 0xff, sizeof(unsigned long long) * watch_cells, s));
        }
        MH_HIP(hipMemsetAsync(P.dense, 0, sizeof(int32_t) * 4 * (cells > 0 ? cells : 1), s));
        MH_HIP(hipMemsetAsync(P.nflag, 0, cells > 0 ? cells : 1, s));
        MH_HIP(hipMemsetAsync(P.dflag, 0, cells > 0 ? cells : 1, s));
        MH_HIP(hipMemsetAsync(P.read_counts, 0, sizeof(int64_t) * (P.n_refs > 0 ? P.n_refs : 1), s));
        MH_HIP(hipMemsetAsync(P.ev_counters, 0, sizeof(int64_t) * 4, s));
        hipLaunchKernelGGL(k_pile_init, dim3(8), dim3(256), 0, s, (long long *)P.first_unit,
                           P.max_pos, P.n_refs);
        PileArgs A{};
        A.rec = c.map.rec;
        A.pool = c.map.pool;
        A.R = *R;
        A.paired = source == 0 ? c.reads.paired : 0;
        A.flag = c.rows.flag; A.ref = c.rows.ref; A.pos = c.rows.pos; A.cig_off = c.rows.cig_off;
        A.n_cigar = c.rows.n_cigar; A.cigar = c.rows.cigar; A.units = c.rows.units;
        A.n_units = n_units;
        A.n_refs = P.n_refs;
        A.cap = P.cap;
        A.dense = P.dense; A.nflag = P.nflag; A.dflag = P.dflag;
        A.read_counts = (unsigned long long *)P.read_counts;
        A.first_unit = (long long *)P.first_unit;
        A.max_pos = P.max_pos;
        A.ev = P.ev; A.ev_pool = P.ev_pool; A.ev_cap = P.ev_cap; A.pool_cap = P.pool_cap;
        A.ev_ctr = (unsigned long long *)P.ev_counters;
        A.q_cutoff = q_cutoff;
        A.win_map = P.win_map;
        A.win_words = geo.win_words;
        A.span_cap = geo.span;
        A.unit_bytes = geo.unit_bytes;
        A.ins_scratch = P.ins_scratch;
        A.watch_pos = P.watch_dpos;
        A.watch_range = P.watch_range;
        A.watch_count = P.watch_count;
        A.watch_first = P.watch_first;
        if (n_units > 0) {
            const int pk = prof_begin(c, "k_pileup");
            const bool skip = P.only.size() == (size_t)P.n_refs &&
                              std::find(P.only.begin(), P.only.end(), (uint8_t)0) != P.only.end();
            const void *kern = source == 0 ? (skip ? (const void *)k_pileup<0, true, false> : (const void *)k_pileup<0, false, false>)
                                           : (skip ? (const void *)k_pileup<1, true, false> : (const void *)k_pileup<1, false, false>);
            if (n_watch > 0)
                kern = source == 0 ? (const void *)k_pileup<0, false, true> : (const void *)k_pileup<1, false, true>;
            MH_HIP(hipFuncSetAttribute(kern, hipFuncAttributeMaxDynamicSharedMemorySize, (int)geo.lds));
            void *kargs[] = {&A};
            MH_HIP(hipLaunchKernel(kern, dim3((unsigned)geo.blocks), dim3(64 * geo.wpb), kargs, geo.lds, s));
            prof_end(c, pk);
            MH_HIP(hipGetLastError());
        }
        hipLaunchKernelGGL(k_pile_fix, dim3(8), dim3(256), 0, s, (long long *)P.first_unit, P.n_refs);
        int64_t ctr[4];
        MH_HIP(hipMemcpyAsync(ctr, P.ev_counters, sizeof(ctr), hipMemcpyDeviceToHost, s));
        MH_HIP(hipStreamSynchronize(s));
        if (ctr[3] == (int64_t)PILE_ERR_INSBUF) {
            set_error("mh_pileup: the merged insertions of one read pair exceed PU_INSBUF (%d bytes)",
                      PU_INSBUF);
            return -3;
        }
        if (ctr[3]) {
            set_error("mh_pileup: malformed alignment row (CIGAR/position)");
            return -3;
        }
        if (!ctr[2]) return 0;
        ++c.retries[RETRY_PILE_EVENTS];
        hipFree(P.ev); hipFree(P.ev_pool);
        P.ev = nullptr; P.ev_pool = nullptr;
        P.ev_cap = ctr[0] * 2 + 1024;
        P.pool_cap = ctr[1] * 2 + 4096;
        MH_HIP(hipMalloc(&P.ev, sizeof(int32_t) * 4 * P.ev_cap));
        MH_HIP(hipMalloc(&P.ev_pool, P.pool_cap));
    }
    set_error("mh_pileup: event buffer overflow");
    return -2;
}

__device__ __forceinline__ uint64_t token_hash(int32_t ref, int32_t pos, const char *b, int32_t len)
{
    uint64_t h = 1469598103934665603ull;
    for (int32_t x = 0; x < len; ++x) h = (h ^ (unsigned char)b[x]) * 1099511628211ull;
    h ^= ((uint64_t)(uint32_t)ref << 32) | (uint32_t)pos;
    h ^= h >> 33; h *= 0xff51afd7ed558ccdull; h ^= h >> 33;
    return h;
}

__device__ __forceinline__ bool same_event(const int32_t *ev, const char *pool, int64_t u, int32_t r,
                                           int32_t ps, int32_t of, int32_t ln)
{
    bool same = ev[4 * u] == r && ev[4 * u + 1] == ps && ev[4 * u + 3] == ln;
    for (int32_t x = 0; same && x < ln; ++x) same = pool[ev[4 * u + 2] + x] == pool[of + x];
    return same;
}

constexpr int TOK_LDS_SLOTS = 4096;
constexpr int TOK_LDS_PROBES = 32;
__global__ __launch_bounds__(1024) void k_tok_insert(const int32_t *ev, const char *pool, int64_t ne,
                                                     int32_t *slot, int32_t *used, int32_t *eslot,
                                                     int64_t mask)
{
    __shared__ int32_t lrep[TOK_LDS_SLOTS];
    __shared__ int32_t lglob[TOK_LDS_SLOTS];
    for (int x = threadIdx.x; x < TOK_LDS_SLOTS; x += blockDim.x) lrep[x] = 0;
    __syncthreads();
    const int64_t per = (ne + gridDim.x - 1) / gridDim.x;
    const int64_t a = (int64_t)blockIdx.x * per, b = a + per < ne ? a + per : ne;
    for (int64_t e0 = a; e0 < b; e0 += blockDim.x) {
        const int64_t e = e0 + threadIdx.x;
        const bool live = e < b;
        int32_t r = 0, ps = 0, of = 0, ln = 0;
        uint64_t h = 0;
        int li = -1;
        bool lead = false;
        if (live) {
            r = ev[4 * e]; ps = ev[4 * e + 1]; of = ev[4 * e + 2]; ln = ev[4 * e + 3];
            h = token_hash(r, ps, pool + of, ln);
            int x = (int)((h >> 40) & (TOK_LDS_SLOTS - 1));
            for (int p = 0; p < TOK_LDS_PROBES; ++p, x = (x + 1) & (TOK_LDS_SLOTS - 1)) {
// ... 42 lines not shown
{
    __shared__ uint32_t hist[TOK_LDS_KEYS];
    const int nd = used[0];
    const bool lds = nd <= TOK_LDS_KEYS;
    if (lds)
        for (int d = threadIdx.x; d < nd; d += blockDim.x) hist[d] = 0;
    __syncthreads();
    const int64_t per = (ne + gridDim.x - 1) / gridDim.x;
    const int64_t a = (int64_t)blockIdx.x * per, b = a + per < ne ? a + per : ne;
    for (int64_t e = a + threadIdx.x; e < b; e += blockDim.x) {
        const int d = slotid[eslot[e]];
        if (lds) atomicAdd(&hist[d], 1u);
        else atomicAdd(&cnt[d], 1u);
    }
    __syncthreads();
    if (lds)
        for (int d = threadIdx.x; d < nd; d += blockDim.x)
            if (hist[d]) atomicAdd(&cnt[d], hist[d]);
}

__global__ void k_tok_gather(const int32_t *ev, const char *pool, const int32_t *slot,
                             const uint32_t *cnt, const int32_t *used, int32_t *meta,
                             char *bytes, int64_t bytes_cap, int32_t *overflow)
{
    const int lane = threadIdx.x;
    const int nd = used[0];
    int base = 0;
    for (int d0 = 0; d0 < nd; d0 += 64) {
        const int d = d0 + lane;
        int32_t ln = 0, u = 0, i = 0;
        if (d < nd) {
            i = used[1 + d];
            u = slot[i] - 1;
            ln = ev[4 * u + 3];
        }
        const int incl = wave_incl_scan(ln, lane);
        const int off = base + incl - ln;
        if (d < nd) {
            meta[5 * d] = ev[4 * u];
            meta[5 * d + 1] = ev[4 * u + 1];
            meta[5 * d + 2] = off;
            meta[5 * d + 3] = ln;
            meta[5 * d + 4] = (int32_t)cnt[d];
            if (off + ln <= bytes_cap) {
                for (int32_t x = 0; x < ln; ++x) bytes[off + x] = pool[ev[4 * u + 2] + x];
            } else {
                *overflow = 1;
            }
        }
        base += __builtin_amdgcn_readlane(incl, 63);
    }
}

int run_token_aggregate(Ctx &c, int64_t ne, int64_t pool_used, std::vector<int32_t> &meta,
                        std::string &bytes)
{
    PileState &P = c.pile;
    hipStream_t s = c.stream;
    meta.clear();
    bytes.clear();
    if (ne <= 0) return 0;
    int64_t cap = 1024;
    while (cap < 2 * ne) cap <<= 1;
    if (P.tok_cap < cap) {
        hipFree(P.tok_slot); hipFree(P.tok_cnt); hipFree(P.tok_used);
        P.tok_slot = nullptr; P.tok_cnt = nullptr; P.tok_used = nullptr; P.tok_cap = 0;
        MH_HIP(hipMalloc(&P.tok_slot, sizeof(int32_t) * 2 * cap + sizeof(int32_t) * (cap / 2 + 1)));
        MH_HIP(hipMalloc(&P.tok_cnt, sizeof(uint32_t) * cap));
        MH_HIP(hipMalloc(&P.tok_used, sizeof(int32_t) * (cap + 1)));
        P.tok_cap = cap;
    }
    if (P.tok_meta_cap < ne) {
        hipFree(P.tok_meta);
        P.tok_meta = nullptr;
        P.tok_meta_cap = 0;
        MH_HIP(hipMalloc(&P.tok_meta, sizeof(int32_t) * (5 * (size_t)ne + 1)));
        P.tok_meta_cap = ne;
    }
    int32_t *ovf = P.tok_meta + 5 * (size_t)P.tok_meta_cap;
    const int64_t want = c.test_caps.token_bytes > 0 ? c.test_caps.token_bytes
                                                     : std::max<int64_t>(pool_used, 64);
    if (P.tok_bytes_cap < want || (c.test_caps.token_bytes > 0 && P.tok_bytes_cap != want)) {
        hipFree(P.tok_bytes);
        P.tok_bytes = nullptr;
        P.tok_bytes_cap = 0;
        MH_HIP(hipMalloc(&P.tok_bytes, (size_t)want));
        P.tok_bytes_cap = want;
    }
    int32_t *slotid = P.tok_slot + cap, *eslot = P.tok_slot + 2 * cap;
    MH_HIP(hipMemsetAsync(P.tok_slot, 0, sizeof(int32_t) * cap, s));
    MH_HIP(hipMemsetAsync(P.tok_cnt, 0, sizeof(uint32_t) * cap, s));
    MH_HIP(hipMemsetAsync(P.tok_used, 0, sizeof(int32_t), s));
    int64_t blocks = (ne + 1023) / 1024;
    if (blocks > 256) blocks = 256;
    hipLaunchKernelGGL(k_tok_insert, dim3((unsigned)blocks), dim3(1024), 0, s, P.ev, P.ev_pool, ne,
                       P.tok_slot, P.tok_used, eslot, cap - 1);
    hipLaunchKernelGGL(k_tok_number, dim3(64), dim3(256), 0, s, P.tok_used, slotid);
    int64_t cblocks = (ne + 4095) / 4096;
    if (cblocks > 256) cblocks = 256;
    hipLaunchKernelGGL(k_tok_count, dim3((unsigned)cblocks), dim3(1024), 0, s, eslot, ne, slotid,
                       P.tok_used, P.tok_cnt);
    MH_HIP(hipGetLastError());
    const int64_t K = std::min<int64_t>(ne, 4096), B = std::min<int64_t>(P.tok_bytes_cap, 64 << 10);
    const size_t pin_need = 16 + 20 * (size_t)K + (size_t)B;
    if (P.tok_pin_cap < pin_need) {
        if (P.tok_pin) hipHostFree(P.tok_pin);
        P.tok_pin = nullptr;
        P.tok_pin_cap = 0;
        MH_HIP(hipHostMalloc((void **)&P.tok_pin, pin_need, hipHostMallocDefault));
        P.tok_pin_cap = pin_need;
    }
    for (int attempt = 0; attempt < 2; ++attempt) {
        MH_HIP(hipMemsetAsync(ovf, 0, sizeof(int32_t), s));
        hipLaunchKernelGGL(k_tok_gather, dim3(1), dim3(64), 0, s, P.ev, P.ev_pool, P.tok_slot,
                           P.tok_cnt, P.tok_used, P.tok_meta, P.tok_bytes, P.tok_bytes_cap, ovf);
        MH_HIP(hipGetLastError());
        MH_HIP(hipMemcpyAsync(P.tok_pin, P.tok_used, sizeof(int32_t), hipMemcpyDeviceToHost, s));
        MH_HIP(hipMemcpyAsync(P.tok_pin + 4, ovf, sizeof(int32_t), hipMemcpyDeviceToHost, s));
        MH_HIP(hipMemcpyAsync(P.tok_pin + 16, P.tok_meta, 20 * (size_t)K, hipMemcpyDeviceToHost, s));
        MH_HIP(hipMemcpyAsync(P.tok_pin + 16 + 20 * (size_t)K, P.tok_bytes, (size_t)B, hipMemcpyDeviceToHost, s));
        MH_HIP(hipStreamSynchronize(s));
        int32_t nd = 0, of = 0;
        std::memcpy(&nd, P.tok_pin, 4);
        std::memcpy(&of, P.tok_pin + 4, 4);
        P.info.tok_insert_blocks = blocks;
        P.info.tok_count_blocks = cblocks;
        P.info.tok_ne = ne;
        P.info.tok_nd = nd;
        if (nd <= 0) return 0;
        meta.resize(5 * (size_t)nd);
        std::memcpy(meta.data(), P.tok_pin + 16, 20 * (size_t)std::min<int64_t>(nd, K));
        if (nd > K)
            MH_HIP(copy_sync(c, meta.data() + 5 * (size_t)K, P.tok_meta + 5 * (size_t)K,
                             20 * (size_t)(nd - K), hipMemcpyDeviceToHost));
        const int64_t total = (int64_t)meta[5 * (size_t)(nd - 1) + 2] + meta[5 * (size_t)(nd - 1) + 3];
        if (!of) {
            bytes.resize((size_t)total);
            if (total > 0) std::memcpy(&bytes[0], P.tok_pin + 16 + 20 * (size_t)K, (size_t)std::min(total, B));
            if (total > B)
                MH_HIP(copy_sync(c, &bytes[(size_t)B], P.tok_bytes + B, (size_t)(total - B), hipMemcpyDeviceToHost));
            return 0;
        }
        ++c.retries[RETRY_TOKEN_BYTES];
        hipFree(P.tok_bytes);
        P.tok_bytes = nullptr;
        P.tok_bytes_cap = 0;
        MH_HIP(hipMalloc(&P.tok_bytes, (size_t)total));
        P.tok_bytes_cap = total;
    }
    set_error("mh_pileup_events: token gather overflow");
    return -2;
}

__global__ void k_pile_export(const int32_t *dense, const uint8_t *nflag, const uint8_t *dflag,
                              const int64_t *read_counts, const int64_t *first_unit,
                              const int32_t *max_pos, int32_t cap, int n_refs, const int32_t *sel,
                              int n_sel, int64_t unit_base, int32_t *sum, int32_t *mx,
                              uint8_t *flags)
{
    const int sidx = blockIdx.y;
    const int64_t stride = (int64_t)gridDim.x * blockDim.x;
    const int64_t t0 = (int64_t)blockIdx.x * blockDim.x + threadIdx.x;
    if (sidx < n_sel) {
        const int64_t src = (int64_t)sel[sidx] * cap, dst = (int64_t)sidx * cap;
        for (int64_t i = t0; i < 4 * (int64_t)cap; i += stride) sum[4 * dst + i] = dense[4 * src + i];
        for (int64_t i = t0; i < cap; i += stride) {
            flags[dst + i] = nflag[src + i];
            flags[(int64_t)n_sel * cap + dst + i] = dflag[src + i];
        }
    }
    if (sidx == 0) {
        for (int64_t i = t0; i < n_refs; i += stride) {
            sum[4 * (int64_t)n_sel * cap + i] = (int32_t)read_counts[i];
            mx[i] = max_pos[i];
// ... 63 lines not shown
    out16[14] = I.tok_nd;
    out16[15] = (int64_t)I.win_map.size() / 2;
    for (int r = 0; r < n_refs && 2 * (size_t)r + 1 < I.win_map.size(); ++r) {
        const int32_t wo = I.win_map[2 * (size_t)r];
        win_len[r] = wo >= 0 ? I.win_map[2 * (size_t)r + 1] : (wo == -2 ? -1 : 0);
    }
    return 0;
}

static int upload_sel(Ctx &c, int n_sel, const int32_t *sel, int32_t **dsel)
{
    PileState &P = c.pile;
    for (int i = 0; i < n_sel; ++i)
        if (sel[i] < 0 || sel[i] >= P.n_refs) { set_error("pileup exchange: ref %d out of range", sel[i]); return -3; }
    if (P.sel_cap < n_sel || !P.sel) {
        hipFree(P.sel);
        P.sel = nullptr;
        P.sel_cap = n_sel > 64 ? n_sel : 64;
        MH_HIP(hipMalloc(&P.sel, sizeof(int32_t) * P.sel_cap));
    }
    if (n_sel) MH_HIP(copy_sync(c, P.sel, sel, sizeof(int32_t) * n_sel, hipMemcpyHostToDevice));
    *dsel = P.sel;
    return 0;
}

extern "C" int mh_pileup_export(mh_ctx *ctx, int n_sel, const int32_t *sel, int64_t unit_base,
                                void *dev_sum, void *dev_max, void *dev_flags)
{
    if (!ctx || !dev_sum || !dev_max || (n_sel > 0 && (!sel || !dev_flags))) return -3;
    Ctx &c = *reinterpret_cast<Ctx *>(ctx);
    PileState &P = c.pile;
    if (!P.dense) { set_error("no pileup to export"); return -3; }
    MH_HIP(hipSetDevice(c.device));
    int32_t *dsel = nullptr;
    if (int st = upload_sel(c, n_sel, sel, &dsel)) return st;
    hipLaunchKernelGGL(k_pile_export, dim3(64, n_sel > 0 ? n_sel : 1), dim3(256), 0, c.stream,
                       P.dense, P.nflag, P.dflag, P.read_counts, P.first_unit, P.max_pos, P.cap,
                       P.n_refs, n_sel > 0 ? dsel : nullptr, n_sel, unit_base, (int32_t *)dev_sum,
                       (int32_t *)dev_max, (uint8_t *)dev_flags);
    MH_HIP(hipGetLastError());
    MH_HIP(hipStreamSynchronize(c.stream));
    return 0;
}

extern "C" int mh_pileup_import(mh_ctx *ctx, int n_sel, const int32_t *sel, const void *dev_sum,
                                const void *dev_max, const void *dev_flags)
{
    if (!ctx || !dev_sum || !dev_max || (n_sel > 0 && (!sel || !dev_flags))) return -3;
    Ctx &c = *reinterpret_cast<Ctx *>(ctx);
    PileState &P = c.pile;
    if (!P.dense) { set_error("no pileup to import into"); return -3; }
    MH_HIP(hipSetDevice(c.device));
    P.land_ok = false;
    int32_t *dsel = nullptr;
    if (int st = upload_sel(c, n_sel, sel, &dsel)) return st;
    hipLaunchKernelGGL(k_pile_import, dim3(64, n_sel > 0 ? n_sel : 1), dim3(256), 0, c.stream,
                       P.dense, P.nflag, P.dflag, P.read_counts, P.first_unit, P.max_pos, P.cap,
                       P.n_refs, n_sel > 0 ? dsel : nullptr, n_sel, (const int32_t *)dev_sum,
                       (const int32_t *)dev_max, (const uint8_t *)dev_flags);
    MH_HIP(hipGetLastError());
    MH_HIP(hipStreamSynchronize(c.stream));
    return 0;
}

namespace mh {

__global__ void k_ev_rebase(int32_t *ev, int64_t first, int64_t n, int32_t pool_base)
{
    for (int64_t e = (int64_t)blockIdx.x * blockDim.x + threadIdx.x; e < n;
         e += (int64_t)gridDim.x * blockDim.x)
        ev[4 * (first + e) + 2] += pool_base;
}

}

extern "C" int mh_pileup_event_bytes(mh_ctx *ctx, int64_t *n_events, int64_t *pool_bytes)
{
    if (!ctx) return -3;
    Ctx &c = *reinterpret_cast<Ctx *>(ctx);
    PileState &P = c.pile;
    int64_t ctr[4] = {0, 0, 0, 0};
    MH_HIP(hipSetDevice(c.device));
    if (P.ev_counters) MH_HIP(copy_sync(c, ctr, P.ev_counters, sizeof(ctr), hipMemcpyDeviceToHost));
    if (n_events) *n_events = ctr[0];
    if (pool_bytes) *pool_bytes = ctr[1];
    return 0;
}

extern "C" int mh_pileup_events_export(mh_ctx *ctx, void *dev_events, void *dev_pool)
{
    if (!ctx) return -3;
    Ctx &c = *reinterpret_cast<Ctx *>(ctx);
    PileState &P = c.pile;
    int64_t n = 0, bytes = 0;
    if (int st = mh_pileup_event_bytes(ctx, &n, &bytes)) return st;
    if ((n > 0 && !dev_events) || (bytes > 0 && !dev_pool)) return -3;
    if (n > 0) MH_HIP(hipMemcpyAsync(dev_events, P.ev, sizeof(int32_t) * 4 * n,
                                     hipMemcpyDeviceToDevice, c.stream));
    if (bytes > 0) MH_HIP(hipMemcpyAsync(dev_pool, P.ev_pool, bytes, hipMemcpyDeviceToDevice, c.stream));
    MH_HIP(hipStreamSynchronize(c.stream));
    return 0;
}

extern "C" int mh_pileup_events_import(mh_ctx *ctx, int parts, const int64_t *n_events,
                                       const int64_t *pool_bytes, const void *dev_events,
                                       int64_t events_stride, const void *dev_pool,
// ... 55 lines not shown
```

### micall-lite_amd/micall_amd/_native.py

```python
import ctypes
import os

import numpy as np

HERE = os.path.dirname(os.path.abspath(__file__))
LIB_PATH = os.environ.get('MICALL_HIP_LIB', os.path.join(HERE, 'libmicall_hip.so'))

E2E, LOCAL = 0, 1
MAXOPS = 128
INT32_MIN = -2 ** 31
OP_CHARS = 'MIDxS'
PILEUP_SLACK = 2048


class NativeUnavailable(RuntimeError):
    pass


class NativeError(RuntimeError):
    pass


class Params(ctypes.Structure):
    _fields_ = [('mode', ctypes.c_int), ('rdg_open', ctypes.c_int), ('rdg_ext', ctypes.c_int),
# ... 2 lines not shown

ALN_FIELDS = ('ref', 'pos', 'rev', 'score', 'secbest', 'flag', 'mapq', 'rnext', 'pnext', 'tlen',
              'sam_ref', 'sam_pos', 'xm', 'xo', 'xg', 'nm', 'ys', 'yt', 'yf', 'n_cigar')


class Aln(ctypes.Structure):
    _fields_ = [(name, ctypes.c_int32) for name in ALN_FIELDS] + [('cigar', ctypes.c_uint32 * MAXOPS)]


ALN_DTYPE = np.dtype([(name, np.int32) for name in ALN_FIELDS] + [('cigar', np.uint32, MAXOPS)])
assert ALN_DTYPE.itemsize == ctypes.sizeof(Aln)

_lib = None

_P = ctypes.c_void_p
_I64P = ctypes.POINTER(ctypes.c_int64)
_I32P = ctypes.POINTER(ctypes.c_int32)


def _declare(L):
    sig = {
        'mh_version': ([], ctypes.c_int),
        'mh_last_error': ([ctypes.c_char_p, ctypes.c_size_t], ctypes.c_int),
        'mh_device_count': ([ctypes.POINTER(ctypes.c_int)], ctypes.c_int),
        'mh_ctx_create': ([ctypes.c_int, ctypes.POINTER(_P)], ctypes.c_int),
        'mh_ctx_destroy': ([_P], ctypes.c_int),
        'mh_ctx_sync': ([_P], ctypes.c_int),
        'mh_ctx_stream': ([_P, ctypes.POINTER(_P)], ctypes.c_int),
        'mh_index_build': ([_P, ctypes.c_int, ctypes.POINTER(ctypes.c_char_p), ctypes.c_int], ctypes.c_int),
        'mh_reads_load': ([_P, ctypes.c_int64, ctypes.c_int, _P, _P, _P, _P], ctypes.c_int),
        'mh_reads_load_fastq': ([_P, ctypes.c_char_p, ctypes.c_char_p, _I64P], ctypes.c_int),
        'mh_reads_load_fastq_part': ([_P, ctypes.c_char_p, ctypes.c_char_p, ctypes.c_int,
                                      ctypes.c_int, _I64P, _I64P], ctypes.c_int),
        'mh_reads_count': ([_P, _I64P, ctypes.POINTER(ctypes.c_int)], ctypes.c_int),
        'mh_reads_set_names': ([_P, ctypes.c_int64, ctypes.POINTER(ctypes.c_char_p)], ctypes.c_int),
        'mh_map': ([_P, ctypes.POINTER(Params)], ctypes.c_int),
        'mh_probe_extend': ([_P, ctypes.POINTER(Params), ctypes.c_int, _P, _P], ctypes.c_int),
        'mh_conseqs_build': ([ctypes.c_int, _P, _P, _P, _P, ctypes.c_int32, _P, _P, _P, ctypes.c_int64,
                              _P, _P, _P, _P, _P, ctypes.c_char_p, _P, ctypes.c_int64, _P, _P],
                             ctypes.c_int),
        'mh_top_tokens': ([ctypes.c_int32, ctypes.c_int32, _P, _P, _P, ctypes.c_char_p, ctypes.c_int32, _P,
                           _P], ctypes.c_int),
        'mh_alns_fetch': ([_P, ctypes.c_int64, ctypes.c_int64, _P], ctypes.c_int),
        'mh_map_counts': ([_P, _P, _P, _P, _P, _P, _I64P, _I64P, _I64P], ctypes.c_int),
        'mh_map_stats': ([_P, _P], ctypes.c_int),
        'mh_recs_fetch_fields': ([_P, ctypes.c_int64, ctypes.c_int64, ctypes.c_int, ctypes.c_int, _P],
                                 ctypes.c_int),
        'mh_recs_fetch': ([_P, ctypes.c_int64, ctypes.c_int64, _P], ctypes.c_int),
        'mh_test_set_capacities': ([_P, ctypes.c_int64, ctypes.c_int64, ctypes.c_int64,
                                    ctypes.c_int64], ctypes.c_int),
        'mh_test_pileup_info': ([_P, _P, ctypes.c_int, _P], ctypes.c_int),
        'mh_test_force_index_collision': ([_P, ctypes.c_int], ctypes.c_int),
        'mh_retry_counts': ([_P, _P], ctypes.c_int),
        'mh_test_set_gotoh_wait': ([_P, ctypes.c_int64], ctypes.c_int),
        'mh_format_rows': ([_P, ctypes.c_int, _P, ctypes.c_int64, ctypes.c_int64,
                            ctypes.POINTER(ctypes.c_char_p), _P, ctypes.c_size_t,
                            ctypes.POINTER(ctypes.c_size_t)], ctypes.c_int),
        'mh_write_rows_crc': ([_P, ctypes.c_int, _P, ctypes.c_int64, ctypes.c_int64,
                               ctypes.POINTER(ctypes.c_char_p), ctypes.c_int, ctypes.c_int64, _I64P,
                               ctypes.POINTER(ctypes.c_uint32)], ctypes.c_int),
        'mh_rows_load': ([_P, ctypes.c_int64, _P, _P, _P, _P, _P, _P, _P, _P, _P, _P,
                          ctypes.c_int64, _P], ctypes.c_int),
        'mh_rows_load_csv': ([_P, ctypes.c_char_p, ctypes.c_int64, ctypes.c_int,
                              ctypes.POINTER(ctypes.c_char_p), _I64P, _I64P, _I32P], ctypes.c_int),
        'mh_rows_info': ([_P, _P, _P, ctypes.c_char_p, ctypes.c_size_t], ctypes.c_int),
        'mh_reads_fastq_lines': ([_P, _I64P], ctypes.c_int),
        'mh_rows_load_sam': ([_P, ctypes.c_char_p, ctypes.c_int64, _I64P, _I64P, _I32P,
                              ctypes.POINTER(ctypes.c_size_t)], ctypes.c_int),
        'mh_sam_info': ([_P, ctypes.c_char_p, ctypes.c_size_t, _P], ctypes.c_int),
        'mh_sam_parse': ([ctypes.c_char_p, ctypes.c_int64, _P, _P, _P, _P, _P, _P, _P, _P, _P, _P,
                          _P, _P, ctypes.c_char_p, _P], ctypes.c_int),
        'mh_prelim_parse': ([ctypes.c_char_p, ctypes.c_int64, ctypes.c_int, ctypes.POINTER(ctypes.c_char_p),
                             ctypes.c_int, _P, _P, _P, _P, _P, _P, _P, _P, _P, _P, _P, _P, _P, _P,
                             ctypes.c_char_p], ctypes.c_int),
        'mh_pileup_watch': ([_P, ctypes.c_int, _P, _P], ctypes.c_int),
        'mh_pileup_watch_fetch': ([_P, _P, _P], ctypes.c_int),
        'mh_pileup': ([_P, ctypes.c_int, ctypes.c_int, ctypes.c_int, _P], ctypes.c_int),
        'mh_pileup_only': ([_P, ctypes.c_int, ctypes.c_int, ctypes.c_int, _P, ctypes.c_int, _P], ctypes.c_int),
        'mh_pileup_dims': ([_P, ctypes.POINTER(ctypes.c_int), _I32P, _I64P, _I64P], ctypes.c_int),
        'mh_pileup_fetch': ([_P, _P, _P, _P, _P, _P, _P], ctypes.c_int),
        'mh_pileup_fetch_refs': ([_P, ctypes.c_int, _P, _P, _P, _P], ctypes.c_int),
        'mh_pileup_events': ([_P, _P, _P, _P, _P, _P, _P], ctypes.c_int),
        'mh_pileup_exchange_bytes': ([_P, ctypes.c_int, _I64P, _I64P, _I64P], ctypes.c_int),
        'mh_pileup_export': ([_P, ctypes.c_int, _P, ctypes.c_int64, _P, _P, _P], ctypes.c_int),
        'mh_pileup_import': ([_P, ctypes.c_int, _P, _P, _P, _P], ctypes.c_int),
        'mh_gotoh_align': ([_P, ctypes.c_char_p, ctypes.c_char_p, ctypes.c_int, ctypes.c_int,
                            ctypes.c_int, ctypes.c_char_p, _P, ctypes.c_char_p, ctypes.c_char_p,
                            ctypes.c_int, ctypes.POINTER(ctypes.c_int)], ctypes.c_int),
        'mh_levenshtein': ([ctypes.c_char_p, ctypes.c_char_p], ctypes.c_int),
        'mh_gotoh_align_batch': ([_P, ctypes.c_int, _P, _P, ctypes.c_int, ctypes.c_int,
                                  ctypes.c_int, ctypes.c_char_p, _P, _P, _P, _P, _P, _P],
                                 ctypes.c_int),
        'mh_gotoh_distance_batch': ([_P, ctypes.c_int, _P, _P, _P, ctypes.c_int, ctypes.c_int,
                                     ctypes.c_int, ctypes.c_char_p, _P, _P, _P, _P], ctypes.c_int),
        'mh_levenshtein_batch': ([ctypes.c_int, _P, _P, _P], ctypes.c_int),
        'mh_pileup_event_bytes': ([_P, _P, _P], ctypes.c_int),
        'mh_pileup_events_export': ([_P, _P, _P], ctypes.c_int),
        'mh_pileup_events_import': ([_P, ctypes.c_int, _P, _P, _P, ctypes.c_int64, _P,
                                     ctypes.c_int64], ctypes.c_int),
        'mh_sam2aln_csv': ([_P, ctypes.c_char_p, ctypes.c_int64, ctypes.c_int, ctypes.c_double,
                            _I64P], ctypes.c_int),
        'mh_sam2aln_csv_q': ([_P, ctypes.c_char_p, ctypes.c_int64, ctypes.c_int, _P, ctypes.c_double,
                              _I64P], ctypes.c_int),
        'mh_sam2aln_file_q': ([_P, ctypes.c_int, ctypes.c_int, _P, ctypes.c_double, _I64P], ctypes.c_int),
        'mh_sam2aln_resident': ([_P, ctypes.c_int, ctypes.POINTER(ctypes.c_char_p), ctypes.c_int, _P,
                                 ctypes.c_double, _I64P], ctypes.c_int),
# ... 68 lines not shown
                             _P], ctypes.c_int),
        'mh_a2c_variant_entries': ([_P, ctypes.c_int, _P, _P, _P, ctypes.c_char_p, ctypes.c_size_t,
                                    ctypes.POINTER(ctypes.c_size_t)], ctypes.c_int),
        'mh_a2c_variant_stats': ([_P, ctypes.c_int, _P, ctypes.POINTER(ctypes.c_double)], ctypes.c_int),
        'mh_fastq_open_part': ([ctypes.c_char_p, ctypes.c_int, ctypes.c_int, ctypes.c_int,
                                ctypes.POINTER(_P), _I64P], ctypes.c_int),
        'mh_fastq_scan_part': ([ctypes.c_char_p, ctypes.c_int, ctypes.c_int, ctypes.c_int, _I64P],
                               ctypes.c_int),
        'mh_fastq_member_open': ([ctypes.c_char_p, ctypes.c_int, ctypes.c_int, ctypes.c_int,
                                  ctypes.POINTER(_P), _I64P], ctypes.c_int),
        'mh_fastq_member_decode': ([_P, ctypes.c_int64, _I64P], ctypes.c_int),
        'mh_fastq_member_tail': ([_P, _P, _P], ctypes.c_int),
        'mh_fastq_member_finish': ([_P, _P, ctypes.c_int64, ctypes.c_int64, _I64P], ctypes.c_int),
        'mh_fastq_frame': ([_P, ctypes.c_int64, ctypes.c_int, _I64P], ctypes.c_int),
        'mh_fastq_record_offset': ([_P, ctypes.c_int64, _I64P], ctypes.c_int),
        'mh_fastq_splice': ([_P, ctypes.c_int64, ctypes.c_int64, _P, ctypes.c_int64, _P,
                             ctypes.c_int64], ctypes.c_int),
        'mh_fastq_view': ([_P, ctypes.POINTER(_P), _I64P], ctypes.c_int),
        'mh_fastq_close': ([_P], ctypes.c_int),
        'mh_fastq_parse': ([_P, _P, ctypes.c_char_p, ctypes.c_size_t, _P, _P, ctypes.c_size_t, _P,
                            ctypes.c_int64, _I64P, _I64P, ctypes.POINTER(ctypes.c_size_t)], ctypes.c_int),
        'mh_reads_load_staged': ([_P, _P, _P, _I64P, ctypes.c_int64, _I64P], ctypes.c_int),
        'mh_format_segments': ([_P, ctypes.c_int, _P, ctypes.c_int64, ctypes.POINTER(ctypes.c_char_p),
                                ctypes.c_int, _P, _P], ctypes.c_int),
        'mh_write_segments': ([_P, ctypes.c_int, _P, _P], ctypes.c_int),
        'mh_crc32_combine': ([ctypes.c_uint32, ctypes.c_uint32, ctypes.c_int64], ctypes.c_uint32),
        'mh_file_crc32': ([ctypes.c_int, _I64P, ctypes.POINTER(ctypes.c_uint32)], ctypes.c_int),
        'mh_phase_times': ([_P, _P, ctypes.c_int], ctypes.c_int),
        'mh_profile': ([_P, ctypes.c_int], ctypes.c_int),
        'mh_profile_get': ([_P, ctypes.c_char_p, ctypes.POINTER(ctypes.c_double), _I64P],
                           ctypes.c_int),
    }
    for name, (args, res) in sig.items():
        fn = getattr(L, name)
        fn.argtypes = args
        fn.restype = res
    return sig


EXPORTED = None


def lib():
    global _lib, EXPORTED
    if _lib is None:
        if not os.path.exists(LIB_PATH):
            raise NativeUnavailable('libmicall_hip.so not built at {} (run __graft_entry__.build() '
                                    'or make -C micall-lite_amd/csrc)'.format(LIB_PATH))
        _lib = ctypes.CDLL(LIB_PATH)
        EXPORTED = sorted(_declare(_lib))
    return _lib


def last_error():
    buf = ctypes.create_string_buffer(1024)
    lib().mh_last_error(buf, len(buf))
    return buf.value.decode(errors='replace')


def check(status, what):
    if status == 0:
        return
    msg = last_error()
    if status == -5:
        raise NativeUnavailable('{}: {}'.format(what, msg))
    if status == -1:
        raise RuntimeError(msg or 'Traceback failed, try local alignment')
    raise NativeError('{} failed ({}): {}'.format(what, status, msg))


def top_tokens(length, rows, dense, nflag, dflag, seed, tok):
    pos = ctypes.c_int32()
    check(lib().mh_top_tokens(length, rows, _ptr(dense), _ptr(nflag), _ptr(dflag), seed, len(seed),
                              _ptr(tok), ctypes.byref(pos)), 'mh_top_tokens')
    return bool(pos.value)


def conseqs_build(rows_of, lengths, seeds, dense, nflag, dflag, ev_row, ev_pos, ev_off, ev_len, ev_cnt,
                  pool):
    n = len(rows_of)
    cap = dense.shape[1] if dense.ndim == 3 else 0
    rows_of = np.ascontiguousarray(rows_of, dtype=np.int32)
    lengths = np.ascontiguousarray(lengths, dtype=np.int32)
    seed_bufs = [ctypes.create_string_buffer(sd, len(sd) + 1) for sd in seeds]
    seed_ptrs = (ctypes.c_char_p * max(n, 1))(*[ctypes.cast(b, ctypes.c_char_p) for b in seed_bufs])
    seed_lens = np.ascontiguousarray([len(sd) for sd in seeds], dtype=np.int32)
    n_ev = len(ev_row)
    ev_row = np.ascontiguousarray(ev_row, dtype=np.int32)
    ev_pos = np.ascontiguousarray(ev_pos, dtype=np.int32)
    ev_off = np.ascontiguousarray(ev_off, dtype=np.int64)
    ev_len = np.ascontiguousarray(ev_len, dtype=np.int32)
    ev_cnt = np.ascontiguousarray(ev_cnt, dtype=np.int64)
    out_cap = int(lengths.sum()) + int(ev_len.sum()) + 1
    out = np.zeros(out_cap, dtype=np.uint8)
    off = np.zeros(n + 1, dtype=np.int64)
    present = np.zeros(max(n, 1), dtype=np.int32)
    check(lib().mh_conseqs_build(n, _ptr(rows_of), _ptr(lengths), seed_ptrs, _ptr(seed_lens), cap,
                                 _ptr(dense), _ptr(nflag), _ptr(dflag), n_ev, _ptr(ev_row),
                                 _ptr(ev_pos), _ptr(ev_off), _ptr(ev_len), _ptr(ev_cnt), bytes(pool) or b'\0',
                                 _ptr(out), out_cap, _ptr(off), _ptr(present)), 'mh_conseqs_build')
    raw = out.tobytes()
    return [(raw[off[k]:off[k + 1]], bool(present[k])) for k in range(n)]


def device_count():
    n = ctypes.c_int()
# ... 578 lines not shown
        offsets = np.ascontiguousarray(offsets, dtype=np.int64)
        lens = np.ascontiguousarray(lens, dtype=np.int32)
        check(lib().mh_reads_load(self.h, len(lens), int(paired), _ptr(seq), _ptr(qual),
                                  _ptr(offsets), _ptr(lens)), 'mh_reads_load')
        self.map_serial += 1

    def reads_load(self, seqs, quals, paired, names=None):
        lens = np.array([len(s) for s in seqs], dtype=np.int32)
        offsets = np.zeros(len(seqs), dtype=np.int64)
        if len(seqs):
            offsets[1:] = np.cumsum(lens[:-1])
        seq = np.frombuffer(''.join(seqs).encode(), dtype=np.uint8)
        qual = np.frombuffer(''.join(quals).encode(), dtype=np.uint8)
        self.reads_load_arrays(seq, qual, offsets, lens, paired)
        if names is not None:
            self.set_names(names)

    def reads_load_fixed(self, reads, quals, paired):
        n, L = reads.shape
        lens = np.full(n, L, dtype=np.int32)
        offsets = np.arange(n, dtype=np.int64) * L
        self.reads_load_arrays(reads.reshape(-1), quals.reshape(-1), offsets, lens, paired)

    def reads_load_fastq(self, path1, path2=None):
        n = ctypes.c_int64()
        check(lib().mh_reads_load_fastq(self.h, path1.encode(), path2.encode() if path2 else None,
                                        ctypes.byref(n)), 'mh_reads_load_fastq')
        self.map_serial += 1
        return n.value

    def reads_load_fastq_part(self, path1, path2, part, parts):
        n = ctypes.c_int64()
        u0 = ctypes.c_int64()
        check(lib().mh_reads_load_fastq_part(self.h, path1.encode(),
                                             path2.encode() if path2 else None, part, parts,
                                             ctypes.byref(n), ctypes.byref(u0)),
              'mh_reads_load_fastq_part')
        self.map_serial += 1
        return n.value, u0.value

    def reads_load_staged(self, fq1, fq2, ranges, fastq_lines1):
        r = np.ascontiguousarray(ranges, dtype=np.int64)
        n = ctypes.c_int64()
        check(lib().mh_reads_load_staged(self.h, fq1.h, fq2.h if fq2 is not None else None,
                                         r.ctypes.data_as(_I64P), int(fastq_lines1),
                                         ctypes.byref(n)), 'mh_reads_load_staged')
        self.map_serial += 1
        return n.value

    def phase_times(self, reset=False):
        out = np.zeros(5, dtype=np.float64)
        check(lib().mh_phase_times(self.h, _ptr(out), int(reset)), 'mh_phase_times')
        return dict(zip(('inflate', 'parse', 'upload', 'format', 'write'), (float(x) for x in out)))

    def _row_args(self, first, n, order):
        if order is not None:
            order = np.ascontiguousarray(order, dtype=np.int64)
            if n is None:
                n = len(order) - first
        elif n is None:
            n = self.reads_count()[0] - first
        names = (ctypes.c_char_p * max(self.n_refs, 1))(*[r.encode() for r in self.refnames])
        return order, None if order is None else _ptr(order), n, names

    def format_segments(self, style, order, seg_rows):
        order, optr, n, names = self._row_args(0, None, order)
        seg_rows = np.ascontiguousarray(seg_rows, dtype=np.int64)
        k = len(seg_rows) - 1
        out = np.zeros(max(k, 1), dtype=np.int64)
        check(lib().mh_format_segments(self.h, style, optr, n, names, k, _ptr(seg_rows), _ptr(out)),
              'mh_format_segments')
        return out[:k]

    def write_rows_at(self, fd, offset, style, order=None, first=0, n=None):
        order, optr, n, names = self._row_args(first, n, order)
        written = ctypes.c_int64()
        crc = ctypes.c_uint32()
        check(lib().mh_write_rows_crc(self.h, style, optr, first, n, names, int(fd), int(offset),
                                      ctypes.byref(written), ctypes.byref(crc)), 'mh_write_rows_crc')
        return written.value, crc.value

    def write_segments(self, fd, offsets, crc=True):
        offsets = np.ascontiguousarray(offsets, dtype=np.int64)
        out = np.zeros(max(len(offsets), 1), dtype=np.uint32)
        check(lib().mh_write_segments(self.h, int(fd), _ptr(offsets), _ptr(out) if crc else None),
              'mh_write_segments')
        return out[:len(offsets)]

    def reads_count(self):
        n = ctypes.c_int64()
        p = ctypes.c_int()
        check(lib().mh_reads_count(self.h, ctypes.byref(n), ctypes.byref(p)), 'mh_reads_count')
        return n.value, bool(p.value)

    def set_names(self, names):
        arr = (ctypes.c_char_p * max(len(names), 1))(*[n.encode() for n in names])
        check(lib().mh_reads_set_names(self.h, len(names), arr), 'mh_reads_set_names')

    def map(self, par):
        check(lib().mh_map(self.h, ctypes.byref(par)), 'mh_map')
        self.map_serial += 1

    def fetch(self, first=0, n=None):
        if n is None:
            n = self.reads_count()[0] - first
        out = np.zeros(max(n, 1), dtype=ALN_DTYPE)
# ... 515 lines not shown
```

Baseline: 64.86 million reads/s.

## Cut host-device syncs across index, map and pileup; stage pileup results in one image

```diff
diff --git a/include/micall_hip.h b/include/micall_hip.h
--- a/include/micall_hip.h
+++ b/include/micall_hip.h
@@ -77,6 +77,10 @@
 int mh_test_pileup_info(mh_ctx *ctx, int64_t *out16, int n_refs, int32_t *win_len);
 int mh_test_force_index_collision(mh_ctx *ctx, int on);
 int mh_retry_counts(mh_ctx *ctx, int64_t *out4);
+int mh_wait_counts(mh_ctx *ctx, int64_t *out5, int reset);
+int mh_test_pileup_staging(mh_ctx *ctx, int on);
+int mh_test_index_tables(int n_refs, const char *const *seqs, int seedlen, int method, int64_t *cap,
+                         int64_t *n_hits, uint32_t *hent, int32_t *hits);
 int mh_test_set_gotoh_wait(mh_ctx *ctx, int64_t ticks);
 int mh_recs_fetch(mh_ctx *ctx, int64_t first, int64_t n, int32_t *out20);
 int mh_recs_fetch_fields(mh_ctx *ctx, int64_t first, int64_t n, int field0, int nfields, int32_t *out);
diff --git a/micall-lite_amd/csrc/mh_api.cpp b/micall-lite_amd/csrc/mh_api.cpp
--- a/micall-lite_amd/csrc/mh_api.cpp
+++ b/micall-lite_amd/csrc/mh_api.cpp
@@ -58,7 +58,15 @@
 hipError_t copy_sync(Ctx &c, void *dst, const void *src, size_t bytes, hipMemcpyKind kind)
 {
     hipError_t e = hipMemcpyAsync(dst, src, bytes, kind, c.stream);
-    return e == hipSuccess ? hipStreamSynchronize(c.stream) : e;
+    return e == hipSuccess ? wait_stream(c, WAIT_OTHER) : e;
+}
+
+hipError_t wait_stream(Ctx &c, int kind)
+{
+    const hipError_t e = hipStreamSynchronize(c.stream);
+    ++c.waits[kind];
+    if (e == hipSuccess) c.index_busy = false;
+    return e;
 }
 
 int prof_begin(Ctx &c, const char *name)
@@ -192,6 +200,8 @@
     std::vector<int32_t> sam_ends;
     int64_t fastq_lines1 = -1;
     DevIndex small;
+    uint8_t *index_pin = nullptr;
+    size_t index_pin_cap = 0;
     int64_t tok_gen = -1;
     std::vector<int32_t> tok_ref, tok_pos, tok_off, tok_len;
     std::vector<int64_t> tok_count;
@@ -285,7 +295,46 @@
     return mix64(h, (uint64_t)n);
 }
 
-static int build_index(DevIndex &ix, int n_refs, const char *const *seqs, int seedlen)
+constexpr int64_t INDEX_SMALL_TOTAL = 65536;
+
+struct HostIndex {
+    std::vector<int64_t> ref_off;
+    std::vector<int32_t> ref_len;
+    std::vector<uint8_t> codes;
+    std::vector<uint4> hent;
+    std::vector<int2> hits;
+    size_t n_hits = 0;
+    uint64_t cap = 0;
+};
+
+struct IndexEnt { uint64_t key; int32_t ref, pos; };
+
+static void index_counting_sort(std::vector<IndexEnt> &ent, int seedlen)
+{
+    constexpr int DIG = 11;
+    const int passes = (2 * seedlen + DIG - 1) / DIG;
+    const size_t n = ent.size();
+    std::vector<uint32_t> count((size_t)passes << DIG, 0);
+    for (size_t i = 0; i < n; ++i)
+        for (int d = 0; d < passes; ++d) ++count[((size_t)d << DIG) | ((ent[i].key >> (DIG * d)) & ((1u << DIG) - 1))];
+    std::vector<IndexEnt> other(n);
+    for (int d = 0; d < passes; ++d) {
+        uint32_t *cn = count.data() + ((size_t)d << DIG);
+        uint32_t at = 0;
+        bool one = false;
+        for (int b = 0; b < 1 << DIG; ++b) {
+            const uint32_t k = cn[b];
+            one = one || (k == n && n > 0);
+            cn[b] = at;
+            at += k;
+        }
+        if (one) continue;
+        for (size_t i = 0; i < n; ++i) other[cn[(ent[i].key >> (DIG * d)) & ((1u << DIG) - 1)]++] = ent[i];
+        ent.swap(other);
+    }
+}
+
+static void index_tables(int n_refs, const char *const *seqs, int seedlen, bool counting, HostIndex &H)
 {
     static const bool trace = getenv("MH_INDEX_TRACE") && *getenv("MH_INDEX_TRACE") == '1';
     const auto tb = std::chrono::steady_clock::now();
@@ -294,17 +343,20 @@
             fprintf(stderr, "index %s %.2f ms\n", what,
                     std::chrono::duration<double, std::milli>(std::chrono::steady_clock::now() - tb).count());
     };
-    struct E { uint64_t key; int32_t ref, pos; };
-    std::vector<int64_t> ref_off(n_refs);
-    std::vector<int32_t> ref_len(n_refs);
+    using E = IndexEnt;
+    std::vector<int64_t> &ref_off = H.ref_off;
+    std::vector<int32_t> &ref_len = H.ref_len;
+    ref_off.assign((size_t)n_refs, 0);
+    ref_len.assign((size_t)n_refs, 0);
     int64_t total_len = 0;
     for (int r = 0; r < n_refs; ++r) {
         ref_len[r] = (int)std::strlen(seqs[r]);
         ref_off[r] = total_len;
         total_len += ref_len[r];
     }
-    std::vector<uint8_t> codes((size_t)total_len);
-    const int nt = std::max(1, std::min<int>(s2a_threads(), n_refs));
+    std::vector<uint8_t> &codes = H.codes;
+    codes.assign((size_t)total_len, 0);
+    const int nt = counting ? 1 : std::max(1, std::min<int>(s2a_threads(), n_refs));
     std::vector<std::vector<E>> per(n_refs);
     mark("pre");
     std::vector<double> t_start((size_t)nt, 0.0);
@@ -345,7 +397,9 @@
     auto less = [](const E &a, const E &b) {
         return a.key != b.key ? a.key < b.key : a.ref != b.ref ? a.ref < b.ref : a.pos < b.pos;
     };
-    {
+    if (counting) {
+        index_counting_sort(ent, seedlen);
+    } else {
         const int ns = ent.size() < 65536 ? 1 : s2a_threads();
         std::vector<size_t> b((size_t)ns + 1);
         for (int t = 0; t <= ns; ++t) b[(size_t)t] = ent.size() * (size_t)t / (size_t)ns;
@@ -364,8 +418,12 @@
     for (size_t i = 0; i < ent.size(); ++i) if (i == 0 || ent[i].key != ent[i - 1].key) ++nkeys;
     uint64_t cap = 1024;
     while (cap < 2 * nkeys) cap <<= 1;
-    std::vector<uint4> hent(cap, make_uint4(~0u, ~0u, 0u, 0u));
-    std::vector<int2> hits(ent.size() ? ent.size() : 1);
+    std::vector<uint4> &hent = H.hent;
+    std::vector<int2> &hits = H.hits;
+    hent.assign(cap, make_uint4(~0u, ~0u, 0u, 0u));
+    hits.assign(ent.size() ? ent.size() : 1, make_int2(0, 0));
+    H.n_hits = ent.size();
+    H.cap = cap;
     for (size_t i = 0; i < ent.size();) {
         size_t j = i + 1;
         while (j < ent.size() && ent[j].key == ent[i].key) ++j;
@@ -376,6 +434,18 @@
     }
     for (size_t i = 0; i < ent.size(); ++i) hits[i] = make_int2(ent[i].ref, ent[i].pos);
     mark("hash");
+}
+
+static int build_index(CtxEx &c, DevIndex &ix, int n_refs, const char *const *seqs, int seedlen, bool small)
+{
+    HostIndex H;
+    index_tables(n_refs, seqs, seedlen, small, H);
+    std::vector<int64_t> &ref_off = H.ref_off;
+    std::vector<int32_t> &ref_len = H.ref_len;
+    std::vector<uint8_t> &codes = H.codes;
+    std::vector<uint4> &hent = H.hent;
+    std::vector<int2> &hits = H.hits;
+    const uint64_t cap = H.cap;
     ix.n_refs = n_refs;
     ix.seedlen = seedlen;
     ix.total = (int64_t)codes.size();
@@ -408,10 +478,23 @@
         MH_HIP(hipMalloc(&ix.blob, total));
         ix.cap_blob = (int64_t)total;
     }
-    mark("planes+alloc");
-    std::vector<uint8_t> stage(total);
-    for (int x = 0; x < NP; ++x) if (sz[x]) std::memcpy(stage.data() + at[x], src[x], sz[x]);
-    mark("stage");
+    std::vector<uint8_t> pageable;
+    uint8_t *stage;
+    if (small) {
+        if (c.index_pin_cap < total) {
+            if (c.index_pin) hipHostFree(c.index_pin);
+            c.index_pin = nullptr;
+            c.index_pin_cap = 0;
+            const size_t pcap = total > ((size_t)1 << 20) ? total : ((size_t)1 << 20);
+            MH_HIP(hipHostMalloc((void **)&c.index_pin, pcap, hipHostMallocDefault));
+            c.index_pin_cap = pcap;
+        }
+        stage = c.index_pin;
+    } else {
+        pageable.resize(total);
+        stage = pageable.data();
+    }
+    for (int x = 0; x < NP; ++x) if (sz[x]) std::memcpy(stage + at[x], src[x], sz[x]);
     uint8_t *d = (uint8_t *)ix.blob;
     ix.codes = d + at[0];
     ix.ref_off = (int64_t *)(d + at[1]);
@@ -421,8 +504,12 @@
     ix.code2 = (uint32_t *)(d + at[5]);
     ix.ncode = (uint32_t *)(d + at[6]);
     ix.cplane = (uint32_t *)(d + at[7]);
-    MH_HIP(hipMemcpy(ix.blob, stage.data(), total, hipMemcpyHostToDevice));
-    mark("upload");
+    if (small) {
+        MH_HIP(hipMemcpyAsync(ix.blob, stage, total, hipMemcpyHostToDevice, c.stream));
+        c.index_busy = true;
+    } else {
+        MH_HIP(hipMemcpy(ix.blob, stage, total, hipMemcpyHostToDevice));
+    }
     return 0;
 }
 
@@ -704,22 +791,29 @@
     free_index(c->small);
     MapState &M = c->map;
     hipFree(M.cand); hipFree(M.n_cand); hipFree(M.yf); hipFree(M.work); hipFree(M.rwork); hipFree(M.skey); hipFree(M.sinfo);
-    hipFree(M.pool); hipFree(M.pool_used); hipFree(M.rec); hipFree(M.counters); hipFree(M.ref_stats);
-    if (M.stats_pin) hipHostFree(M.stats_pin);
-    M.stats_pin = nullptr;
-    M.stats_pin_cap = 0;
+    hipFree(M.pool); hipFree(M.rec);
+    hipFree(M.counters);
+    if (M.pass_pin) hipHostFree(M.pass_pin);
+    M.pass_pin = nullptr;
+    M.pass_pin_cap = 0;
     RowState &R = c->rows;
     hipFree(R.flag); hipFree(R.ref); hipFree(R.pos); hipFree(R.cig_off); hipFree(R.n_cigar);
     hipFree(R.cigar); hipFree(R.units);
     PileState &P = c->pile;
     hipFree(c->gotoh_buf);
-    hipFree(P.dense); hipFree(P.nflag); hipFree(P.dflag); hipFree(P.read_counts);
-    hipFree(P.first_unit); hipFree(P.max_pos); hipFree(P.ev); hipFree(P.ev_pool);
+    hipFree(P.dense); hipFree(P.nflag); hipFree(P.dflag);
+    hipFree(P.scal);
+    hipFree(P.ev); hipFree(P.ev_pool);
     hipFree(P.tok_slot); hipFree(P.tok_cnt); hipFree(P.tok_used); hipFree(P.tok_meta);
     hipFree(P.tok_bytes);
-    hipFree(P.ev_counters);
     if (P.land) hipHostFree(P.land);
     P.land = nullptr;
+    P.stage = nullptr;
+    P.stage_gen = -1;
+    hipFree(P.pack);
+    if (P.win_pin) hipHostFree(P.win_pin);
+    P.win_pin = nullptr;
+    P.win_pin_cap = 0;
     if (P.tok_pin) hipHostFree(P.tok_pin);
     P.tok_pin = nullptr;
     P.tok_pin_cap = 0;
@@ -731,6 +825,7 @@
     hipFree(P.win_map);
     for (auto &kv : c->len_tabs) hipFree(kv.second);
     if (c->pin) hipHostFree(c->pin);
+    if (c->index_pin) hipHostFree(c->index_pin);
     s2a_free(*c);
     censor_free(*c);
     a2c_free(*c);
@@ -762,11 +857,11 @@
     }
     CtxEx *c = X(ctx);
     MH_HIP(hipSetDevice(c->device));
-    MH_HIP(hipStreamSynchronize(c->stream));
+    if (c->index_busy) MH_HIP(wait_stream(*c, WAIT_INDEX));
     int64_t total = 0;
     for (int r = 0; r < n_refs; ++r) total += (int64_t)std::strlen(seqs[r]);
     const uint64_t sig = c->force_index_collision ? 0x5eedull : signature(n_refs, seqs, seedlen);
-    const bool cacheable = total > 65536;
+    const bool cacheable = total > INDEX_SMALL_TOTAL;
     c->index = DevIndex{};
     for (size_t e = 0; e < c->cache.size(); ++e) {
         const DevIndex &ix = c->cache[e];
@@ -785,13 +880,13 @@
         }
     }
     if (!cacheable) {
-        if (int st = build_index(c->small, n_refs, seqs, seedlen)) return st;
+        if (int st = build_index(*c, c->small, n_refs, seqs, seedlen, true)) return st;
         c->small.sig = sig;
         c->index = c->small;
         return 0;
     }
     DevIndex ix;
-    if (int st = build_index(ix, n_refs, seqs, seedlen)) { free_index(ix); return st; }
+    if (int st = build_index(*c, ix, n_refs, seqs, seedlen, false)) { free_index(ix); return st; }
     ix.sig = sig;
     if (c->cache.size() >= 2) {
         free_index(c->cache.front());
@@ -1107,7 +1202,6 @@
     MH_HIP(hipSetDevice(c->device));
     if (int st = prepare_len_tab(*c, *par)) return st;
     int st = run_map(*c, *par);
-    if (st == 0) MH_HIP(hipStreamSynchronize(c->stream));
     prof_flush(*c);
     c->rec_cache.clear();
     ++c->map_gen;
@@ -1254,6 +1348,54 @@
     if (!ctx || !out4) return -3;
     for (int k = 0; k < RETRY_KINDS; ++k) out4[k] = X(ctx)->retries[k];
     return 0;
+}
+
+int mh_wait_counts(mh_ctx *ctx, int64_t *out5, int reset)
+{
+    if (!ctx || !out5) return -3;
+    Ctx *c = X(ctx);
+    for (int k = 0; k < WAIT_KINDS; ++k) {
+        out5[k] = c->waits[k];
+        if (reset) c->waits[k] = 0;
+    }
+    return 0;
+}
+
+int mh_test_pileup_staging(mh_ctx *ctx, int on)
+{
+    if (!ctx) return -3;
+    X(ctx)->test_caps.no_pile_stage = on == 0;
+    return 0;
+}
+
+int mh_test_index_tables(int n_refs, const char *const *seqs, int seedlen, int method, int64_t *cap,
+                         int64_t *n_hits, uint32_t *hent, int32_t *hits)
+{
+    if (n_refs < 0 || (n_refs > 0 && !seqs) || seedlen < 8 || seedlen > 32 || method < 0 || method > 2 ||
+        !cap || !n_hits) {
+        set_error("mh_test_index_tables: bad arguments");
+        return -3;
+    }
+    try {
+        int64_t total = 0;
+        for (int r = 0; r < n_refs; ++r) total += (int64_t)std::strlen(seqs[r]);
+        HostIndex H;
+        index_tables(n_refs, seqs, seedlen, method == 0 ? total <= INDEX_SMALL_TOTAL : method == 2, H);
+        if (hent && hits) {
+            if (*cap < (int64_t)H.cap || *n_hits < (int64_t)H.n_hits) {
+                set_error("mh_test_index_tables: buffers too small");
+                return -2;
+            }
+            std::memcpy(hent, H.hent.data(), sizeof(uint4) * H.cap);
+            std::memcpy(hits, H.hits.data(), sizeof(int2) * H.n_hits);
+        }
+        *cap = (int64_t)H.cap;
+        *n_hits = (int64_t)H.n_hits;
+        return 0;
+    } catch (const std::exception &e) {
+        set_error("mh_test_index_tables: %s", e.what());
+        return -2;
+    }
 }
 
 int mh_test_set_gotoh_wait(mh_ctx *ctx, int64_t ticks)
@@ -2083,19 +2225,7 @@
     return 0;
 }
 
-struct Landing {
-    int64_t *read_counts, *first_unit;
-    int32_t *max_pos;
-    int64_t *ev_counters;
-    size_t bytes;
-};
-
-static Landing landing_of(const PileState &P)
-{
-    const size_t nr = (size_t)P.n_refs, ev_at = (20 * nr + 7) & ~(size_t)7;
-    return Landing{(int64_t *)P.land, (int64_t *)(P.land + 8 * nr), (int32_t *)(P.land + 16 * nr),
-                   (int64_t *)(P.land + ev_at), 20 * nr + 64};
-}
+static Landing landing_of(const PileState &P) { return landing_at(P.land, (size_t)P.n_refs); }
 
 int mh_pileup(mh_ctx *ctx, int source, int q_cutoff, int n_refs, const int32_t *ref_lens)
 {
@@ -2128,29 +2258,7 @@
     c->pile.n_refs = n_refs;
     c->pile.cap = cap;
     c->pile.ref_lens.assign(ref_lens, ref_lens + n_refs);
-    c->pile.land_ok = false;
     int st = run_pileup(*c, source, q_cutoff);
-    if (st == 0) {
-        PileState &P = c->pile;
-        const size_t nr = (size_t)P.n_refs, need = landing_of(P).bytes;
-        if (P.land_cap < need) {
-            if (P.land) hipHostFree(P.land);
-            P.land = nullptr;
-            P.land_cap = 0;
-            if (hipHostMalloc((void **)&P.land, need, hipHostMallocDefault) == hipSuccess) P.land_cap = need;
-            else P.land = nullptr;
-        }
-        if (P.land && P.read_counts && P.first_unit && P.max_pos) {
-            const Landing L = landing_of(P);
-            bool ok = hipMemcpyAsync(L.read_counts, P.read_counts, 8 * nr, hipMemcpyDeviceToHost, c->stream) == hipSuccess &&
-                      hipMemcpyAsync(L.first_unit, P.first_unit, 8 * nr, hipMemcpyDeviceToHost, c->stream) == hipSuccess &&
-                      hipMemcpyAsync(L.max_pos, P.max_pos, 4 * nr, hipMemcpyDeviceToHost, c->stream) == hipSuccess;
-            if (ok && P.ev_counters)
-                ok = hipMemcpyAsync(L.ev_counters, P.ev_counters, 32, hipMemcpyDeviceToHost, c->stream) == hipSuccess;
-            P.land_ok = ok;
-        }
-        MH_HIP(hipStreamSynchronize(c->stream));
-    }
     prof_flush(*c);
     return st;
 }
@@ -2243,7 +2351,7 @@
                                   c.stream));
         at += (parts[i].bytes + 255) & ~(size_t)255;
     }
-    MH_HIP(hipStreamSynchronize(c.stream));
+    MH_HIP(wait_stream(c, WAIT_FETCH));
     at = 0;
     for (int i = 0; i < n; ++i) {
         if (!parts[i].dst) continue;
@@ -2291,11 +2399,28 @@
         std::memcpy(mx.data(), landing_of(P).max_pos, sizeof(int32_t) * (size_t)P.n_refs);
     else
         MH_HIP(copy_sync(*c, mx.data(), P.max_pos, sizeof(int32_t) * (size_t)P.n_refs, hipMemcpyDeviceToHost));
+    for (int k = 0; k < n_sel; ++k)
+        if (refs[k] < 0 || refs[k] >= P.n_refs) { set_error("mh_pileup_fetch_refs: ref %d out of range", refs[k]); return -3; }
+    bool staged = P.stage && P.stage_gen == P.gen && P.stage_at.size() == (size_t)P.n_refs;
+    for (int k = 0; k < n_sel && staged; ++k)
+        staged = mx[(size_t)refs[k]] <= 0 || P.stage_at[(size_t)refs[k]] >= 0;
+    if (staged) {
+        for (int k = 0; k < n_sel; ++k) {
+            const int r = refs[k];
+            const size_t rows = (size_t)std::min<int64_t>(P.cap, std::max(mx[(size_t)r], 0));
+            if (rows == 0) continue;
+            const size_t cap = (size_t)P.cap, ns = (size_t)P.stage_n, base = (size_t)r * cap;
+            const size_t at = (size_t)P.stage_at[(size_t)r] * cap;
+            std::memcpy(dense + 4 * base, P.stage + 16 * at, 16 * rows);
+            std::memcpy(nflag + base, P.stage + 16 * cap * ns + at, rows);
+            std::memcpy(dflag + base, P.stage + 17 * cap * ns + at, rows);
+        }
+        return 0;
+    }
     std::vector<FetchPart> parts;
     parts.reserve(3 * (size_t)n_sel);
     for (int k = 0; k < n_sel; ++k) {
         const int r = refs[k];
-        if (r < 0 || r >= P.n_refs) { set_error("mh_pileup_fetch_refs: ref %d out of range", r); return -3; }
         const int64_t rows = std::min<int64_t>(P.cap, std::max(mx[(size_t)r], 0));
         if (rows == 0) continue;
         const int64_t base = (int64_t)r * P.cap;
diff --git a/micall-lite_amd/csrc/mh_internal.h b/micall-lite_amd/csrc/mh_internal.h
--- a/micall-lite_amd/csrc/mh_internal.h
+++ b/micall-lite_amd/csrc/mh_internal.h
@@ -108,6 +108,8 @@
     const uint32_t u = (uint32_t)sid;
     return (int64_t)(u % MAXCAND) * plane + (int64_t)(u / MAXCAND);
 }
+
+constexpr size_t PASS_USED_AT = 256, PASS_STATS_AT = 512;
 
 struct MapState {
     int64_t n_reads = 0;
@@ -134,8 +136,8 @@
     int64_t last_rescue = 0;
     bool valid = false;
     std::vector<int64_t> stats_host;
-    int64_t *stats_pin = nullptr;
-    size_t stats_pin_cap = 0;
+    char *pass_pin = nullptr;
+    size_t pass_pin_cap = 0;
     bool stats_pin_ready = false;
     std::map<std::pair<const void *, int>, int> dp_occ;
     bool stats_host_valid = false;
@@ -169,9 +171,18 @@
     int64_t alloc_cells = 0;
     int alloc_refs = 0;
     int64_t gen = 0;
+    char *scal = nullptr;
+    char *pack = nullptr;
+    size_t pack_cap = 0;
     char *land = nullptr;
     size_t land_cap = 0;
     bool land_ok = false;
+    char *stage = nullptr;
+    int64_t stage_gen = -1;
+    int stage_n = 0;
+    std::vector<int32_t> stage_at;
+    int32_t *win_pin = nullptr;
+    int win_pin_cap = 0;
     std::vector<int32_t> ref_lens;
     std::vector<uint8_t> only;
     std::vector<int32_t> watch_ref, watch_pos, watch_order;
@@ -203,6 +214,23 @@
     } info;
 };
 
+struct Landing {
+    int64_t *read_counts, *first_unit;
+    int32_t *max_pos;
+    int64_t *ev_counters;
+    size_t bytes;
+};
+
+__host__ __device__ inline Landing landing_at(char *base, size_t nr)
+{
+    const size_t ev_at = (20 * nr + 7) & ~(size_t)7;
+    return Landing{(int64_t *)base, (int64_t *)(base + 8 * nr), (int32_t *)(base + 16 * nr),
+                   (int64_t *)(base + ev_at), 20 * nr + 64};
+}
+
+constexpr size_t PILE_STAGE_MAX = (size_t)8 << 20;
+constexpr size_t PILE_STAGE_RUNS = 16;
+
 hipError_t launch_pack_reads(DevReads &r, const uint8_t *d_seq, const uint8_t *d_qual,
                              const int64_t *d_src_off, hipStream_t s);
 int run_map(struct Ctx &c, const mh_params &par);
@@ -263,15 +291,20 @@
     int64_t pile_event_bytes = 0;
     int64_t token_bytes = 0;
     int64_t gotoh_wait_ticks = 0;
+    bool no_pile_stage = false;
 };
 
 enum { RETRY_CIGAR_POOL = 0, RETRY_PILE_EVENTS = 1, RETRY_TOKEN_BYTES = 2, RETRY_GOTOH_WAIT = 3,
        RETRY_KINDS = 4 };
+
+enum { WAIT_MAP = 0, WAIT_PILEUP = 1, WAIT_FETCH = 2, WAIT_INDEX = 3, WAIT_OTHER = 4, WAIT_KINDS = 5 };
 
 struct Ctx {
     int device = 0;
     TestCaps test_caps;
     int64_t retries[RETRY_KINDS] = {0, 0, 0, 0};
+    int64_t waits[WAIT_KINDS] = {0, 0, 0, 0, 0};
+    bool index_busy = false;
     int n_cu = 0;
     bool prof = false;
     std::map<std::string, ProfEntry> prof_acc;
@@ -307,6 +340,7 @@
 void prof_flush(Ctx &c);
 int hip_fail(hipError_t e, const char *what);
 hipError_t copy_sync(Ctx &c, void *dst, const void *src, size_t bytes, hipMemcpyKind kind);
+hipError_t wait_stream(Ctx &c, int kind);
 
 }
 
diff --git a/micall-lite_amd/csrc/mh_map.hip b/micall-lite_amd/csrc/mh_map.hip
--- a/micall-lite_amd/csrc/mh_map.hip
+++ b/micall-lite_amd/csrc/mh_map.hip
@@ -2280,14 +2280,18 @@
         MH_HIP(hipMalloc(&M.rec, sizeof(Rec) * cap));
         M.cap_reads = cap;
     }
-    if (M.counters == nullptr) MH_HIP(hipMalloc(&M.counters, sizeof(int32_t) * 8));
-    if (M.cap_refs < c.index.n_refs || M.ref_stats == nullptr) {
-        hipFree(M.ref_stats);
+    if (M.cap_refs < c.index.n_refs || M.counters == nullptr) {
+        hipFree(M.counters);
+        M.counters = nullptr;
+        M.pool_used = nullptr;
+        M.ref_stats = nullptr;
+        M.cap_refs = 0;
         const int cr = c.index.n_refs > 0 ? c.index.n_refs : 1;
-        MH_HIP(hipMalloc(&M.ref_stats, sizeof(int64_t) * (5 * cr + 3)));
+        MH_HIP(hipMalloc(&M.counters, PASS_STATS_AT + sizeof(int64_t) * (5 * (size_t)cr + 3)));
+        M.pool_used = (unsigned long long *)((char *)M.counters + PASS_USED_AT);
+        M.ref_stats = (int64_t *)((char *)M.counters + PASS_STATS_AT);
         M.cap_refs = cr;
     }
-    if (M.pool_used == nullptr) MH_HIP(hipMalloc(&M.pool_used, sizeof(unsigned long long)));
     const int64_t test_cap = c.test_caps.cigar_pool_words;
     const int64_t need = test_cap > 0 ? test_cap : pool_words_for(n);
     if (need > (int64_t)INT32_MAX) {
@@ -2305,10 +2309,13 @@
     return 0;
 }
 
-__global__ void k_init_stats(int64_t *s, int n_refs)
-{
-    for (int i = blockIdx.x * blockDim.x + threadIdx.x; i < 5 * n_refs + 3; i += gridDim.x * blockDim.x)
+__global__ void k_init_stats(int64_t *s, int n_refs, int32_t *counters, unsigned long long *pool_used)
+{
+    const int t = blockIdx.x * blockDim.x + threadIdx.x;
+    for (int i = t; i < 5 * n_refs + 3; i += gridDim.x * blockDim.x)
         s[i] = ((i >= 3 * n_refs && i < 5 * n_refs) || i == 5 * n_refs + 2) ? INT64_MAX : 0;
+    if (t < 8) counters[t] = 0;
+    if (t == 8) *pool_used = 0;
 }
 
 __global__ void k_fix_first(int64_t *s, int n_refs)
@@ -2325,14 +2332,8 @@
         M.stats_host.resize(5 * (size_t)M.n_refs + 3);
         const size_t bytes = sizeof(int64_t) * M.stats_host.size();
         if (M.stats_pin_ready) {
-            if (hipStreamSynchronize(c.stream) != hipSuccess) {
-                set_error("map_stats_host: copy failed");
-                return nullptr;
-            }
-            std::memcpy(M.stats_host.data(), M.stats_pin, bytes);
-        } else if (hipMemcpyAsync(M.stats_host.data(), M.ref_stats, bytes, hipMemcpyDeviceToHost,
-                                  c.stream) != hipSuccess ||
-                   hipStreamSynchronize(c.stream) != hipSuccess) {
+            std::memcpy(M.stats_host.data(), M.pass_pin + PASS_STATS_AT, bytes);
+        } else if (copy_sync(c, M.stats_host.data(), M.ref_stats, bytes, hipMemcpyDeviceToHost) != hipSuccess) {
             set_error("map_stats_host: copy failed");
             return nullptr;
         }
@@ -2403,6 +2404,7 @@
     if (lds > 160 * 1024) { set_error("mh_probe_extend: reads too long"); return -3; }
     hipStream_t s = c.stream;
     int32_t *d_items = nullptr, *d_out = nullptr;
+    c.index_busy = true;
     MH_HIP(hipMalloc(&d_items, sizeof(int32_t) * 4 * (size_t)n));
     MH_HIP(hipMalloc(&d_out, sizeof(int32_t) * 8 * (size_t)n));
     MH_HIP(hipMemcpyAsync(d_items, items, sizeof(int32_t) * 4 * (size_t)n, hipMemcpyHostToDevice, s));
@@ -2415,7 +2417,7 @@
     else hipLaunchKernelGGL((k_probe_ext<0>), dim3(n), dim3(64), lds, s, da, d_items, d_out, n);
     MH_HIP(hipGetLastError());
     MH_HIP(hipMemcpyAsync(out, d_out, sizeof(int32_t) * 8 * (size_t)n, hipMemcpyDeviceToHost, s));
-    MH_HIP(hipStreamSynchronize(s));
+    MH_HIP(wait_stream(c, WAIT_OTHER));
     hipFree(d_items);
     hipFree(d_out);
     return 0;
@@ -2447,7 +2449,27 @@
     M.par = par;
     hipStream_t s = c.stream;
     M.last_work = M.last_cigar = 0;
-    if (n == 0) hipLaunchKernelGGL(k_init_stats, dim3(64), dim3(256), 0, s, M.ref_stats, M.n_refs);
+    const size_t land_bytes = PASS_STATS_AT + sizeof(int64_t) * (5 * (size_t)M.n_refs + 3);
+    if (M.pass_pin_cap < land_bytes) {
+        if (M.pass_pin) hipHostFree(M.pass_pin);
+        M.pass_pin = nullptr;
+        M.pass_pin_cap = 0;
+        const size_t cap = land_bytes > 8192 ? land_bytes : 8192;
+        MH_HIP(hipHostMalloc((void **)&M.pass_pin, cap, hipHostMallocDefault));
+        M.pass_pin_cap = cap;
+    }
+    c.index_busy = true;
+    auto land_and_wait = [&]() -> int {
+        hipLaunchKernelGGL(k_fix_first, dim3(8), dim3(256), 0, s, M.ref_stats, M.n_refs);
+        MH_HIP(hipGetLastError());
+        MH_HIP(hipMemcpyAsync(M.pass_pin, M.counters, land_bytes, hipMemcpyDeviceToHost, s));
+        MH_HIP(wait_stream(c, WAIT_MAP));
+        return 0;
+    };
+    if (n == 0) {
+        hipLaunchKernelGGL(k_init_stats, dim3(64), dim3(256), 0, s, M.ref_stats, M.n_refs, M.counters, M.pool_used);
+        if (int st = land_and_wait()) return st;
+    }
     if (n > 0) {
         auto launch_seed = [&]() -> int {
             SeedArgs sa{c.reads, c.index, par.mode, c.len_tab, M.cand, M.n_cand, M.yf, M.work, M.counters, M.cap_reads};
@@ -2517,9 +2539,7 @@
         if (pblocks > 1 << 16) pblocks = 1 << 16;
         if (pblocks < 1) pblocks = 1;
         for (int attempt = 0; attempt < 2; ++attempt) {
-            hipLaunchKernelGGL(k_init_stats, dim3(64), dim3(256), 0, s, M.ref_stats, M.n_refs);
-            MH_HIP(hipMemsetAsync(M.counters, 0, sizeof(int32_t) * 8, s));
-            MH_HIP(hipMemsetAsync(M.pool_used, 0, sizeof(unsigned long long), s));
+            hipLaunchKernelGGL(k_init_stats, dim3(64), dim3(256), 0, s, M.ref_stats, M.n_refs, M.counters, M.pool_used);
             if (int st = launch_seed()) return st;
             if (int st = launch_dp(M.work, M.counters, M.counters + 5, n * 2, "k_dp")) return st;
             if (c.reads.paired && units > 0) {
@@ -2538,11 +2558,11 @@
             hipLaunchKernelGGL(k_pair, dim3((unsigned)pblocks), dim3(256), 0, s, pa);
             prof_end(c, pp);
             MH_HIP(hipGetLastError());
+            if (int st = land_and_wait()) return st;
             int32_t ctr[5];
             unsigned long long used = 0;
-            MH_HIP(hipMemcpyAsync(ctr, M.counters, sizeof(ctr), hipMemcpyDeviceToHost, s));
-            MH_HIP(hipMemcpyAsync(&used, M.pool_used, sizeof(used), hipMemcpyDeviceToHost, s));
-            MH_HIP(hipStreamSynchronize(s));
+            std::memcpy(ctr, M.pass_pin, sizeof(ctr));
+            std::memcpy(&used, M.pass_pin + PASS_USED_AT, sizeof(used));
             M.last_work = ctr[0] + ctr[4];
             M.last_rescue = ctr[4];
             M.last_cigar = (int64_t)used;
@@ -2564,22 +2584,7 @@
             M.pool_cap = grown;
         }
     }
-    hipLaunchKernelGGL(k_fix_first, dim3(8), dim3(256), 0, s, M.ref_stats, M.n_refs);
-    MH_HIP(hipGetLastError());
-    {
-        const size_t bytes = sizeof(int64_t) * (5 * (size_t)M.n_refs + 3);
-        if (M.stats_pin_cap < bytes) {
-            if (M.stats_pin) hipHostFree(M.stats_pin);
-            M.stats_pin = nullptr;
-            M.stats_pin_cap = 0;
-            if (hipHostMalloc(&M.stats_pin, bytes, hipHostMallocDefault) == hipSuccess)
-                M.stats_pin_cap = bytes;
-            else
-                M.stats_pin = nullptr;
-        }
-        if (M.stats_pin && hipMemcpyAsync(M.stats_pin, M.ref_stats, bytes, hipMemcpyDeviceToHost, s) == hipSuccess)
-            M.stats_pin_ready = true;
-    }
+    M.stats_pin_ready = true;
     M.valid = true;
     return 0;
 }
diff --git a/micall-lite_amd/csrc/mh_pileup.hip b/micall-lite_amd/csrc/mh_pileup.hip
--- a/micall-lite_amd/csrc/mh_pileup.hip
+++ b/micall-lite_amd/csrc/mh_pileup.hip
@@ -769,18 +769,73 @@
     }
 }
 
-__global__ void k_pile_init(long long *first_unit, int32_t *max_pos, int n)
-{
-    for (int i = blockIdx.x * blockDim.x + threadIdx.x; i < n; i += gridDim.x * blockDim.x) {
-        first_unit[i] = INT64_MAX;
-        max_pos[i] = 0;
-    }
-}
-
-__global__ void k_pile_fix(long long *first_unit, int n)
-{
-    for (int i = blockIdx.x * blockDim.x + threadIdx.x; i < n; i += gridDim.x * blockDim.x)
-        if (first_unit[i] == INT64_MAX) first_unit[i] = -1;
+struct PileReset {
+    uint4 *range[5];
+    int64_t words[5];
+    uint32_t fill[5];
+    unsigned long long *read_counts;
+    long long *first_unit;
+    int32_t *max_pos;
+    int64_t *ev_counters;
+    int n_refs;
+};
+
+__global__ void k_pile_init(PileReset a)
+{
+    const int64_t t = (int64_t)blockIdx.x * blockDim.x + threadIdx.x;
+    const int64_t stride = (int64_t)gridDim.x * blockDim.x;
+    for (int k = 0; k < 5; ++k) {
+        const uint4 v = make_uint4(a.fill[k], a.fill[k], a.fill[k], a.fill[k]);
+        for (int64_t i = t; i < a.words[k]; i += stride) a.range[k][i] = v;
+    }
+    for (int64_t i = t; i < a.n_refs; i += stride) {
+        a.read_counts[i] = 0;
+        a.first_unit[i] = INT64_MAX;
+        a.max_pos[i] = 0;
+    }
+    if (t < 4) a.ev_counters[t] = 0;
+}
+
+struct PileTail {
+    const unsigned long long *read_counts;
+    long long *first_unit;
+    const int32_t *max_pos;
+    const int64_t *ev_counters;
+    int n_refs;
+    char *out;
+    int64_t rows_at;
+    const int32_t *dense;
+    const uint8_t *nflag, *dflag;
+    int64_t cap;
+    int stage_n, n_runs;
+    int32_t run_first[PILE_STAGE_RUNS], run_slot[PILE_STAGE_RUNS], run_refs[PILE_STAGE_RUNS];
+};
+
+__global__ void k_pile_tail(PileTail a)
+{
+    const int64_t t = (int64_t)blockIdx.x * blockDim.x + threadIdx.x;
+    const int64_t stride = (int64_t)gridDim.x * blockDim.x;
+    const Landing L = landing_at(a.out, (size_t)a.n_refs);
+    for (int64_t i = t; i < a.n_refs; i += stride) {
+        long long fu = a.first_unit[i];
+        if (fu == INT64_MAX) a.first_unit[i] = fu = -1;
+        L.first_unit[i] = fu;
+        L.read_counts[i] = (int64_t)a.read_counts[i];
+        L.max_pos[i] = a.max_pos[i];
+    }
+    if (t < 4) L.ev_counters[t] = a.ev_counters[t];
+    uint4 *od = (uint4 *)(a.out + a.rows_at);
+    uint8_t *on = (uint8_t *)(od + a.cap * a.stage_n), *of = on + a.cap * a.stage_n;
+    for (int k = 0; k < a.n_runs; ++k) {
+        const int64_t from = (int64_t)a.run_first[k] * a.cap, to = (int64_t)a.run_slot[k] * a.cap;
+        const int64_t n = (int64_t)a.run_refs[k] * a.cap;
+        const uint4 *sd = (const uint4 *)a.dense + from;
+        for (int64_t i = t; i < n; i += stride) od[to + i] = sd[i];
+        for (int64_t i = t; i < n; i += stride) {
+            on[to + i] = a.nflag[from + i];
+            of[to + i] = a.dflag[from + i];
+        }
+    }
 }
 
 static int ensure_pile(Ctx &c)
@@ -789,20 +844,28 @@
     const int64_t cells = (int64_t)(P.n_refs > 0 ? P.n_refs : 1) * P.cap;
     if (P.alloc_cells < cells) {
         hipFree(P.dense); hipFree(P.nflag); hipFree(P.dflag);
+        P.dense = nullptr; P.nflag = nullptr; P.dflag = nullptr;
+        P.alloc_cells = 0;
         MH_HIP(hipMalloc(&P.dense, sizeof(int32_t) * 4 * cells));
-        MH_HIP(hipMalloc(&P.nflag, cells));
-        MH_HIP(hipMalloc(&P.dflag, cells));
+        MH_HIP(hipMalloc(&P.nflag, (cells + 15) & ~(int64_t)15));
+        MH_HIP(hipMalloc(&P.dflag, (cells + 15) & ~(int64_t)15));
         P.alloc_cells = cells;
     }
-    if (P.alloc_refs < (P.n_refs > 0 ? P.n_refs : 1)) {
-        hipFree(P.read_counts); hipFree(P.first_unit); hipFree(P.max_pos);
+    if (P.alloc_refs < (P.n_refs > 0 ? P.n_refs : 1) || !P.scal) {
+        hipFree(P.scal);
+        P.scal = nullptr;
+        P.alloc_refs = 0;
         const int nr = P.n_refs > 0 ? P.n_refs : 1;
-        MH_HIP(hipMalloc(&P.read_counts, sizeof(int64_t) * nr));
-        MH_HIP(hipMalloc(&P.first_unit, sizeof(int64_t) * nr));
-        MH_HIP(hipMalloc(&P.max_pos, sizeof(int32_t) * nr));
+        MH_HIP(hipMalloc(&P.scal, landing_at(nullptr, (size_t)nr).bytes));
         P.alloc_refs = nr;
     }
-    if (!P.ev_counters) MH_HIP(hipMalloc(&P.ev_counters, sizeof(int64_t) * 4));
+    {
+        const Landing D = landing_at(P.scal, (size_t)P.n_refs);
+        P.read_counts = D.read_counts;
+        P.first_unit = D.first_unit;
+        P.max_pos = D.max_pos;
+        P.ev_counters = D.ev_counters;
+    }
     const int64_t t_ev = c.test_caps.pile_events, t_pool = c.test_caps.pile_event_bytes;
     if (!P.ev || (t_ev > 0 && P.ev_cap != t_ev)) {
         hipFree(P.ev);
@@ -940,9 +1003,52 @@
         P.win_map_cap = 2 * (P.n_refs > 16 ? P.n_refs : 16);
         MH_HIP(hipMalloc(&P.win_map, sizeof(int32_t) * P.win_map_cap));
     }
-    if (P.n_refs > 0)
-        MH_HIP(hipMemcpyAsync(P.win_map, geo.win_map.data(), sizeof(int32_t) * 2 * P.n_refs,
-                              hipMemcpyHostToDevice, s));
+    if (P.n_refs > 0) {
+        if (P.win_pin_cap < 2 * P.n_refs) {
+            if (P.win_pin) hipHostFree(P.win_pin);
+            P.win_pin = nullptr;
+            P.win_pin_cap = 0;
+            MH_HIP(hipHostMalloc((void **)&P.win_pin, sizeof(int32_t) * P.win_map_cap, hipHostMallocDefault));
+            P.win_pin_cap = P.win_map_cap;
+        }
+        std::memcpy(P.win_pin, geo.win_map.data(), sizeof(int32_t) * 2 * P.n_refs);
+        MH_HIP(hipMemcpyAsync(P.win_map, P.win_pin, sizeof(int32_t) * 2 * P.n_refs, hipMemcpyHostToDevice, s));
+    }
+    P.land_ok = false;
+    P.stage_gen = -1;
+    const size_t land_bytes = landing_at(nullptr, (size_t)P.n_refs).bytes;
+    const size_t rows_at = (land_bytes + 255) & ~(size_t)255;
+    const bool some_only = P.only.size() == (size_t)P.n_refs && P.n_refs > 0;
+    P.stage_at.assign((size_t)P.n_refs, -1);
+    P.stage_n = 0;
+    std::vector<std::pair<int, int>> runs;
+    for (int r = 0; r < P.n_refs; ++r) {
+        if (some_only && !P.only[(size_t)r]) continue;
+        if (runs.empty() || runs.back().second != r) runs.push_back({r, r});
+        runs.back().second = r + 1;
+        P.stage_at[(size_t)r] = P.stage_n++;
+    }
+    const size_t stage_bytes = (size_t)18 * (size_t)P.cap * (size_t)P.stage_n;
+    const bool stage = stage_bytes > 0 && stage_bytes <= PILE_STAGE_MAX && runs.size() <= PILE_STAGE_RUNS &&
+                       !c.test_caps.no_pile_stage;
+    const size_t image_bytes = stage ? rows_at + stage_bytes : land_bytes;
+    if (P.land_cap < image_bytes) {
+        if (P.land) hipHostFree(P.land);
+        P.land = nullptr;
+        P.land_cap = 0;
+        const size_t cap = image_bytes > ((size_t)1 << 20) ? image_bytes : ((size_t)1 << 20);
+        MH_HIP(hipHostMalloc((void **)&P.land, cap, hipHostMallocDefault));
+        P.land_cap = cap;
+    }
+    if (P.pack_cap < image_bytes) {
+        hipFree(P.pack);
+        P.pack = nullptr;
+        P.pack_cap = 0;
+        const size_t cap = image_bytes > ((size_t)1 << 20) ? image_bytes : ((size_t)1 << 20);
+        MH_HIP(hipMalloc(&P.pack, cap));
+        P.pack_cap = cap;
+    }
+    P.stage = P.land + rows_at;
     const int n_watch = (int)P.watch_order.size();
     const size_t watch_cells = (size_t)n_watch * 4 * PW_QBINS;
     if (n_watch > 0) {
@@ -975,17 +1081,29 @@
     }
     const int64_t cells = (int64_t)P.n_refs * P.cap;
     for (int attempt = 0; attempt < 3; ++attempt) {
-        if (n_watch > 0) {
-            MH_HIP(hipMemsetAsync(P.watch_count, 0, sizeof(uint32_t) * watch_cells, s));
-            MH_HIP(hipMemsetAsync(P.watch_first, 0xff, sizeof(unsigned long long) * watch_cells, s));
-        }
-        MH_HIP(hipMemsetAsync(P.dense, 0, sizeof(int32_t) * 4 * (cells > 0 ? cells : 1), s));
-        MH_HIP(hipMemsetAsync(P.nflag, 0, cells > 0 ? cells : 1, s));
-        MH_HIP(hipMemsetAsync(P.dflag, 0, cells > 0 ? cells : 1, s));
-        MH_HIP(hipMemsetAsync(P.read_counts, 0, sizeof(int64_t) * (P.n_refs > 0 ? P.n_refs : 1), s));
-        MH_HIP(hipMemsetAsync(P.ev_counters, 0, sizeof(int64_t) * 4, s));
-        hipLaunchKernelGGL(k_pile_init, dim3(8), dim3(256), 0, s, (long long *)P.first_unit,
-                           P.max_pos, P.n_refs);
+        {
+            const int64_t cz = cells > 0 ? cells : 1;
+            PileReset Z{};
+            Z.range[0] = (uint4 *)P.dense; Z.words[0] = cz;
+            Z.range[1] = (uint4 *)P.nflag; Z.words[1] = (cz + 15) / 16;
+            Z.range[2] = (uint4 *)P.dflag; Z.words[2] = (cz + 15) / 16;
+            if (n_watch > 0) {
+                Z.range[3] = (uint4 *)P.watch_count; Z.words[3] = (int64_t)watch_cells / 4;
+                Z.range[4] = (uint4 *)P.watch_first; Z.words[4] = (int64_t)watch_cells / 2;
+                Z.fill[4] = 0xffffffffu;
+            }
+            Z.read_counts = (unsigned long long *)P.read_counts;
+            Z.first_unit = (long long *)P.first_unit;
+            Z.max_pos = P.max_pos;
+            Z.ev_counters = P.ev_counters;
+            Z.n_refs = P.n_refs;
+            int64_t words = 0;
+            for (int k = 0; k < 5; ++k) words += Z.words[k];
+            int64_t zb = (words + 1023) / 1024;
+            zb = zb < 1 ? 1 : zb > 2048 ? 2048 : zb;
+            hipLaunchKernelGGL(k_pile_init, dim3((unsigned)zb), dim3(256), 0, s, Z);
+            MH_HIP(hipGetLastError());
+        }
         PileArgs A{};
         A.rec = c.map.rec;
         A.pool = c.map.pool;
@@ -1026,10 +1144,33 @@
             prof_end(c, pk);
             MH_HIP(hipGetLastError());
         }
-        hipLaunchKernelGGL(k_pile_fix, dim3(8), dim3(256), 0, s, (long long *)P.first_unit, P.n_refs);
+        {
+            PileTail T{};
+            T.read_counts = (const unsigned long long *)P.read_counts;
+            T.first_unit = (long long *)P.first_unit;
+            T.max_pos = P.max_pos;
+            T.ev_counters = P.ev_counters;
+            T.n_refs = P.n_refs;
+            T.out = P.pack;
+            T.rows_at = (int64_t)rows_at;
+            T.dense = P.dense; T.nflag = P.nflag; T.dflag = P.dflag;
+            T.cap = P.cap;
+            T.stage_n = P.stage_n;
+            T.n_runs = stage ? (int)runs.size() : 0;
+            for (int k = 0; k < T.n_runs; ++k) {
+                T.run_first[k] = runs[(size_t)k].first;
+                T.run_slot[k] = P.stage_at[(size_t)runs[(size_t)k].first];
+                T.run_refs[k] = runs[(size_t)k].second - runs[(size_t)k].first;
+            }
+            int64_t tb = stage ? ((int64_t)P.cap * P.stage_n + 1023) / 1024 : 1;
+            tb = tb < 1 ? 1 : tb > 2048 ? 2048 : tb;
+            hipLaunchKernelGGL(k_pile_tail, dim3((unsigned)tb), dim3(256), 0, s, T);
+            MH_HIP(hipGetLastError());
+            MH_HIP(hipMemcpyAsync(P.land, P.pack, image_bytes, hipMemcpyDeviceToHost, s));
+        }
+        MH_HIP(wait_stream(c, WAIT_PILEUP));
         int64_t ctr[4];
-        MH_HIP(hipMemcpyAsync(ctr, P.ev_counters, sizeof(ctr), hipMemcpyDeviceToHost, s));
-        MH_HIP(hipStreamSynchronize(s));
+        std::memcpy(ctr, landing_at(P.land, (size_t)P.n_refs).ev_counters, sizeof(ctr));
         if (ctr[3] == (int64_t)PILE_ERR_INSBUF) {
             set_error("mh_pileup: the merged insertions of one read pair exceed PU_INSBUF (%d bytes)",
                       PU_INSBUF);
@@ -1039,7 +1180,11 @@
             set_error("mh_pileup: malformed alignment row (CIGAR/position)");
             return -3;
         }
-        if (!ctr[2]) return 0;
+        if (!ctr[2]) {
+            P.land_ok = true;
+            if (stage) P.stage_gen = P.gen;
+            return 0;
+        }
         ++c.retries[RETRY_PILE_EVENTS];
         hipFree(P.ev); hipFree(P.ev_pool);
         P.ev = nullptr; P.ev_pool = nullptr;
@@ -1188,6 +1333,19 @@
     }
 }
 
+__global__ void k_tok_reset(uint4 *slot, uint4 *cnt, int64_t words, int32_t *used, int32_t *overflow)
+{
+    const int64_t t = (int64_t)blockIdx.x * blockDim.x + threadIdx.x;
+    for (int64_t i = t; i < words; i += (int64_t)gridDim.x * blockDim.x) {
+        slot[i] = make_uint4(0, 0, 0, 0);
+        cnt[i] = make_uint4(0, 0, 0, 0);
+    }
+    if (t == 0) {
+        used[0] = 0;
+        *overflow = 0;
+    }
+}
+
 int run_token_aggregate(Ctx &c, int64_t ne, int64_t pool_used, std::vector<int32_t> &meta,
                         std::string &bytes)
 {
@@ -1224,9 +1382,12 @@
         P.tok_bytes_cap = want;
     }
     int32_t *slotid = P.tok_slot + cap, *eslot = P.tok_slot + 2 * cap;
-    MH_HIP(hipMemsetAsync(P.tok_slot, 0, sizeof(int32_t) * cap, s));
-    MH_HIP(hipMemsetAsync(P.tok_cnt, 0, sizeof(uint32_t) * cap, s));
-    MH_HIP(hipMemsetAsync(P.tok_used, 0, sizeof(int32_t), s));
+    {
+        int64_t zb = (cap / 4 + 255) / 256;
+        if (zb > 2048) zb = 2048;
+        hipLaunchKernelGGL(k_tok_reset, dim3((unsigned)zb), dim3(256), 0, s, (uint4 *)P.tok_slot,
+                           (uint4 *)P.tok_cnt, cap / 4, P.tok_used, ovf);
+    }
     int64_t blocks = (ne + 1023) / 1024;
     if (blocks > 256) blocks = 256;
     hipLaunchKernelGGL(k_tok_insert, dim3((unsigned)blocks), dim3(1024), 0, s, P.ev, P.ev_pool, ne,
@@ -1247,7 +1408,7 @@
         P.tok_pin_cap = pin_need;
     }
     for (int attempt = 0; attempt < 2; ++attempt) {
-        MH_HIP(hipMemsetAsync(ovf, 0, sizeof(int32_t), s));
+        if (attempt) MH_HIP(hipMemsetAsync(ovf, 0, sizeof(int32_t), s));
         hipLaunchKernelGGL(k_tok_gather, dim3(1), dim3(64), 0, s, P.ev, P.ev_pool, P.tok_slot,
                            P.tok_cnt, P.tok_used, P.tok_meta, P.tok_bytes, P.tok_bytes_cap, ovf);
         MH_HIP(hipGetLastError());
@@ -1255,7 +1416,7 @@
         MH_HIP(hipMemcpyAsync(P.tok_pin + 4, ovf, sizeof(int32_t), hipMemcpyDeviceToHost, s));
         MH_HIP(hipMemcpyAsync(P.tok_pin + 16, P.tok_meta, 20 * (size_t)K, hipMemcpyDeviceToHost, s));
         MH_HIP(hipMemcpyAsync(P.tok_pin + 16 + 20 * (size_t)K, P.tok_bytes, (size_t)B, hipMemcpyDeviceToHost, s));
-        MH_HIP(hipStreamSynchronize(s));
+        MH_HIP(wait_stream(c, WAIT_FETCH));
         int32_t nd = 0, of = 0;
         std::memcpy(&nd, P.tok_pin, 4);
         std::memcpy(&of, P.tok_pin + 4, 4);
@@ -1425,6 +1586,7 @@
     if (!P.dense) { set_error("no pileup to import into"); return -3; }
     MH_HIP(hipSetDevice(c.device));
     P.land_ok = false;
+    P.stage_gen = -1;
     int32_t *dsel = nullptr;
     if (int st = upload_sel(c, n_sel, sel, &dsel)) return st;
     hipLaunchKernelGGL(k_pile_import, dim3(64, n_sel > 0 ? n_sel : 1), dim3(256), 0, c.stream,
diff --git a/micall-lite_amd/micall_amd/_native.py b/micall-lite_amd/micall_amd/_native.py
--- a/micall-lite_amd/micall_amd/_native.py
+++ b/micall-lite_amd/micall_amd/_native.py
@@ -78,6 +78,10 @@
         'mh_test_pileup_info': ([_P, _P, ctypes.c_int, _P], ctypes.c_int),
         'mh_test_force_index_collision': ([_P, ctypes.c_int], ctypes.c_int),
         'mh_retry_counts': ([_P, _P], ctypes.c_int),
+        'mh_wait_counts': ([_P, _P, ctypes.c_int], ctypes.c_int),
+        'mh_test_pileup_staging': ([_P, ctypes.c_int], ctypes.c_int),
+        'mh_test_index_tables': ([ctypes.c_int, ctypes.POINTER(ctypes.c_char_p), ctypes.c_int,
+                                  ctypes.c_int, _I64P, _I64P, _P, _P], ctypes.c_int),
         'mh_test_set_gotoh_wait': ([_P, ctypes.c_int64], ctypes.c_int),
         'mh_format_rows': ([_P, ctypes.c_int, _P, ctypes.c_int64, ctypes.c_int64,
                             ctypes.POINTER(ctypes.c_char_p), _P, ctypes.c_size_t,
@@ -252,6 +256,21 @@
     return _lib
 
 
+INDEX_AUTO, INDEX_SORTED, INDEX_COUNTING = 0, 1, 2
+
+
+def index_tables(seqs, seedlen, method=INDEX_AUTO):
+    arr = (ctypes.c_char_p * max(len(seqs), 1))(*[s.encode() for s in seqs])
+    cap, n = ctypes.c_int64(), ctypes.c_int64()
+    check(lib().mh_test_index_tables(len(seqs), arr, seedlen, method, ctypes.byref(cap), ctypes.byref(n),
+                                     None, None), 'mh_test_index_tables')
+    hent = np.zeros((cap.value, 4), dtype=np.uint32)
+    hits = np.zeros((max(n.value, 1), 2), dtype=np.int32)
+    check(lib().mh_test_index_tables(len(seqs), arr, seedlen, method, ctypes.byref(cap), ctypes.byref(n),
+                                     _ptr(hent), _ptr(hits)), 'mh_test_index_tables')
+    return hent, hits[:n.value]
+
+
 def last_error():
     buf = ctypes.create_string_buffer(1024)
     lib().mh_last_error(buf, len(buf))
@@ -936,6 +955,14 @@
         out = np.zeros(5, dtype=np.float64)
         check(lib().mh_phase_times(self.h, _ptr(out), int(reset)), 'mh_phase_times')
         return dict(zip(('inflate', 'parse', 'upload', 'format', 'write'), (float(x) for x in out)))
+
+    def wait_counts(self, reset=False):
+        out = np.zeros(5, dtype=np.int64)
+        check(lib().mh_wait_counts(self.h, _ptr(out), int(reset)), 'mh_wait_counts')
+        return dict(zip(('map', 'pileup', 'fetch', 'index', 'other'), (int(x) for x in out)))
+
+    def test_pileup_staging(self, on):
+        check(lib().mh_test_pileup_staging(self.h, int(bool(on))), 'mh_test_pileup_staging')
 
     def _row_args(self, first, n, order):
         if order is not None:
```

Measured after the change: 65.82 million reads/s, median of 6. +1.5%, better.
